# bravesoftdz/soundchunks

Measured on AMD Instinct MI355X. Metric: encoded Msamples/s @44.1kHz stereo ChunkSize=8 ChunkCount=4096; bit-exact .gsc, higher is better.
Workload: dtype f32; 1 GPU; 44.1 kHz stereo, ChunkSize=8 ChunkCount=4096 8-bit, 1024 s synthetic; frames=256, parallelism=frame-sharded x1

## Files before the change

soundchunks_amd/csrc/gsc_device.h:

```cpp
#pragma once
#include <stdint.h>

namespace gsc {

constexpr int kMaxK = 4096;
constexpr int kMaxInternal = 4095;
constexpr int kScanThreads = 512;
constexpr int kScanSlots = 8;
constexpr int kMaxScanIters = 100;
constexpr int kMaxChunkSize = 16;

__host__ __device__ constexpr int feature_stride(int cs) { return 2 * cs <= 8 ? 8 : (2 * cs <= 16 ? 16 : 32); }

__device__ inline float sqrt_rn(float x) { return __builtin_sqrtf(x); }

struct ReduceFrame {
    int64_t x_off;
    int64_t c_off;
    int64_t n_off;
    int64_t k_off;
    int64_t ka_off;
    int64_t t_off;
    int32_t N, K;
    int32_t iters;
    int32_t slow;
    double err;
    int32_t done;
    int32_t generic;
    int32_t restarts;
    int32_t loop_iters;
    int32_t tree_exact;
    int32_t dcol;
    uint64_t t_done;
    int32_t* cl_host;
    int32_t* notify;
    uint64_t stamps[128];
    uint64_t ystamps[16];
    uint64_t acounts[64];
    uint64_t xcounts[16];
    uint64_t xcounts2[16];
};

struct DspFrame {
    int64_t s_off;
    int64_t x_off;
    int64_t c_off;
    int32_t sc;
    int32_t n;
    int32_t atten_div;
    int32_t pad_;
};

struct ReconFrame {
    int64_t chunk_off;
    int64_t red_off;
    int64_t out_off;
    int32_t n, sc;
    double law;
};

struct FitFrame {
    int64_t cand_off;
    int64_t q_off;
    int64_t out_off;
    int32_t R, N;
    float eps;
    int32_t overflow;
};

struct PackFrame {
    int64_t out_off;
    int64_t r_off;
    int64_t w_off;
    int32_t N, R;
    int32_t nbits;
    int32_t cp_off;
};

inline int64_t pack_word_capacity(int64_t n) { return (n * 17 + 31) / 32 + 1; }

struct AnnTree {
    const float* pts;
    int n, dd;
    int* pidx;
    int* cd;
    float* cv;
    float* lo;
    float* hi;
    float* bnd;
    float* val;
    int ncap;
};

struct KnnOvJob {
    int tree;
    int q_off;
    int out;
    float eps;
};

}
```

soundchunks_amd/csrc/gsc_runtime.cpp:

```cpp
#include <cstddef>
#include <hip/hip_runtime.h>

#include <algorithm>
#include <atomic>
#include <chrono>
#include <cmath>
#include <cstdio>
#include <cstdlib>
#include <cstring>
#include <functional>
#include <new>
#include <string>
#include <strings.h>
#include <mutex>
#include <thread>
#include <vector>

#include "../../include/soundchunks.h"
#include "fpc_math.h"
#include "gsc_decode.h"
#include "gsc_device.h"
#include "gsc_encoder.h"

extern "C" hipError_t gsc_launch_yakmo(int D, const gsc::ReduceFrame* frames, int nframes, const float* X, float* C,
                                       float* fs, int* is, float* gsum, uint32_t* gbits, int max_n, hipStream_t st);
extern "C" size_t gsc_yakmo_big_floats(int64_t total_points, int nframes);
extern "C" size_t gsc_yakmo_big_words(int64_t total_points, int nframes);
extern "C" int gsc_yakmo_max_lds_points(void);
extern "C" hipError_t gsc_launch_scan_pass(int D, gsc::ReduceFrame* frames, int nframes, int K, const float* X,
                                           float* C, int* is, float* fs, const float* rate_tab, double tol, int max_passes,
                                           int only_flagged, hipStream_t st);
extern "C" hipError_t gsc_launch_scan_batch(int D, int logk, gsc::ReduceFrame* frames, int nframes, const float* X,
                                            float* C, int* is, const float* rate_tab, double tol, int max_passes,
                                            int opts, float* tails, hipStream_t st);
extern "C" size_t gsc_scan_tail_floats_per_frame(int D, int logk);
extern "C" hipError_t gsc_launch_atten(int cs, gsc::DspFrame* frames, int nframes, const double* samp, int64_t span,
                                       int ch, int obd, hipStream_t st);
extern "C" hipError_t gsc_launch_features(int cs, const gsc::DspFrame* frames, int nframes, int max_n,
                                          const double* samp, int64_t span, int ch, const double* trig, double s0,
                                          double scale, float* X, uint8_t* nr, float* Q, hipStream_t st);
extern "C" hipError_t gsc_launch_pcm(const int16_t* pcm, int64_t span, int ch, double* samp, hipStream_t st);
extern "C" hipError_t gsc_launch_knnfit(int CS, gsc::FitFrame* frames, int nframes, int max_n, int max_r,
                                        const float* cand, const float* q, int* out, hipStream_t st);
extern "C" hipError_t gsc_launch_recon(const gsc::ReconFrame* frames, int nframes, int max_n, int cs, int ch, int bd,
                                       const uint32_t* chunk, const int16_t* rdst, const uint8_t* ratten, int16_t* out,
                                       hipStream_t st);
extern "C" hipError_t gsc_launch_sqdiff(const int16_t* a, const int16_t* b, int64_t n, unsigned long long* acc,
                                        hipStream_t st);
extern "C" hipError_t gsc_launch_usecount(const gsc::PackFrame* frames, int nframes, const int* best, int* counts,
                                          hipStream_t st);
extern "C" hipError_t gsc_launch_pack(gsc::PackFrame* frames, int nframes, const int* best, const int* remap,
                                      uint32_t* words, uint32_t* codes, uint64_t* cps, hipStream_t st);
extern "C" hipError_t gsc_launch_ann_build_many(const void* trees, int ntrees, hipStream_t st);
extern "C" hipError_t gsc_launch_knnfit_ann(const void* trees, const void* jobs, int njobs, const float* q, int* out,
                                            float* pq_key, void* pq_node, int pq_cap, hipStream_t st);

namespace gsc {

void parallel_for(int n, int threads, const std::function<void(int)>& fn) {
    if (threads <= 1 || n <= 1) {
        for (int i = 0; i < n; ++i) fn(i);
        return;
    }
    std::atomic<int> next{0};
    std::vector<std::thread> pool;
    const int t = std::min(threads, n);
    pool.reserve(size_t(t));
    for (int k = 0; k < t; ++k)
        pool.emplace_back([&] {
            for (;;) {
                const int i = next.fetch_add(1);
                if (i >= n) break;
                fn(i);
            }
        });
    for (auto& th : pool) th.join();
}

int host_threads() {
    static int n = [] {
        const char* e = std::getenv("GSC_HOST_THREADS");
        if (e && std::atoi(e) > 0) return std::atoi(e);
        const unsigned hc = std::thread::hardware_concurrency();
        return int(std::min(16u, std::max(1u, hc)));
    }();
    return n;
}

namespace {

thread_local std::string t_err;
thread_local gsc_timing t_tim;

int fail(const std::string& m) {
    t_err = m;
    return -1;
}

#define HIP_TRY(expr)                                                                     \
    do {                                                                                  \
        hipError_t e_ = (expr);                                                           \
        if (e_ != hipSuccess) return fail(std::string(#expr) + ": " + hipGetErrorString(e_)); \
    } while (0)

double now_ms() {
    return std::chrono::duration<double, std::milli>(std::chrono::steady_clock::now().time_since_epoch()).count();
}

int ensure_device() {
    static int state = 0;
    static std::string why;
    if (state == 0) {
        int n = 0;
        if (hipGetDeviceCount(&n) != hipSuccess || n <= 0) {
            why = "no HIP device visible (the MI355X hot path has no CPU fallback)";
            state = -1;
        } else {
            hipDeviceProp_t p;
            int dev = 0;
            if (hipGetDevice(&dev) != hipSuccess || hipGetDeviceProperties(&p, dev) != hipSuccess) {
                why = "cannot query the HIP device";
                state = -1;
            } else if (std::strncmp(p.gcnArchName, "gfx950", 6) != 0) {
                why = std::string("device is ") + p.gcnArchName + ", kernels are built for gfx950 only";
                state = -1;
            } else {
                state = 1;
            }
        }
    }
    if (state < 0) return fail(why);
    (void)hipGetLastError();
    return 0;
}

std::atomic<int64_t> g_devbuf_ns{0};

template <typename T>
struct DevBuf {
    T* p = nullptr;
    size_t n = 0;
    ~DevBuf() {
        if (p) {
            const double t = now_ms();
            (void)hipFree(p);
            g_devbuf_ns.fetch_add(int64_t((now_ms() - t) * 1e6));
        }
    }
    hipError_t alloc(size_t count) {
        n = count;
        const double t = now_ms();
        const hipError_t e = hipMalloc(&p, sizeof(T) * std::max<size_t>(count, 1));
        g_devbuf_ns.fetch_add(int64_t((now_ms() - t) * 1e6));
        return e;
    }
};

struct DevArena {
    char* p = nullptr;
    size_t cap = 0, used = 0;
    std::vector<char*> retired;
    ~DevArena() {
        if (p) (void)hipFree(p);
        for (char* r : retired) (void)hipFree(r);
    }
    static size_t round_up(size_t b) { return (std::max<size_t>(b, 1) + 255) & ~size_t(255); }
    hipError_t reset(size_t bytes) {
        used = 0;
        if (bytes <= cap) return hipSuccess;
        if (p) retired.push_back(p);
        p = nullptr;
        cap = 0;
        const size_t want = std::max<size_t>(bytes + bytes / 4, size_t(1) << 20);
        const double t = now_ms();
        const hipError_t e = hipMalloc(reinterpret_cast<void**>(&p), want);
        g_devbuf_ns.fetch_add(int64_t((now_ms() - t) * 1e6));
        if (e == hipSuccess) cap = want;
        return e;
    }
    template <typename T>
    T* take(size_t count) {
        const size_t b = round_up(sizeof(T) * count);
        if (used + b > cap) return nullptr;
        T* r = reinterpret_cast<T*>(p + used);
        used += b;
        return r;
    }
};

double scan_tolerance(int precision) {
    if (precision <= 0) return 1.0;
    double p = 1.0, base = 10.0;
    int i = precision;
    while (i > 0) {
        while ((i & 1) == 0) {
            i >>= 1;
            base = base * base;
        }
        --i;
        p = p * base;
    }
    return 1.0 / p;
}

int padded_k(int K) {
    int k = 256;
    while (k < K) k <<= 1;
    return k;
}

bool batched_scan_shape(int D, int K) {
    if (std::getenv("GSC_SCAN_GENERIC")) return false;
    return (D == 8 || D == 16 || D == 32) && K >= 2 && K <= 4096;
}

int64_t tail_offset(int i) { return int64_t(i) * 4096 * 16; }

std::atomic<int> g_scan_rounds{0};

hipError_t launch_scan_passes(int D, ReduceFrame* dfr, int nf, int K, const float* X, float* C, int* is, float* fs,
                              const float* rate, int precision) {
    const double tol = scan_tolerance(precision);
    const bool batched = batched_scan_shape(D, K);
    int logk = 0;
    while ((1 << logk) < padded_k(K)) ++logk;
    DevBuf<float> tails;
    if (batched && gsc_scan_tail_floats_per_frame(D, logk) > 0) {
        const hipError_t e = tails.alloc(size_t(tail_offset(nf)));
        if (e != hipSuccess) return e;
    }
    int max_passes = kMaxScanIters;
    if (const char* e = std::getenv("GSC_SCAN_MAX_PASSES")) max_passes = std::max(1, std::min(kMaxScanIters, std::atoi(e)));
    std::vector<int32_t> flags(2 * static_cast<size_t>(nf));
    static_assert(offsetof(ReduceFrame, generic) == offsetof(ReduceFrame, done) + sizeof(int32_t), "adjacent flags");
    for (int round = 0; round < max_passes; ++round) {
        if (batched) {
            const int opts = (std::getenv("GSC_SCAN_FULL_A1") ? 1 : 0) | (std::getenv("GSC_SCAN_NO_PRUNE") ? 2 : 0) |
                             ((std::getenv("GSC_SCAN_KB") ? (std::atoi(std::getenv("GSC_SCAN_KB")) & 255) : 0) << 8);
            hipError_t e =
                gsc_launch_scan_batch(D, logk, dfr, nf, X, C, is, rate, tol, max_passes, opts, tails.p, nullptr);
            if (e != hipSuccess) return e;
            e = hipMemcpy2D(flags.data(), 2 * sizeof(int32_t), &dfr[0].done, sizeof(ReduceFrame), 2 * sizeof(int32_t),
                            size_t(nf), hipMemcpyDeviceToHost);
            if (e != hipSuccess) return e;
            g_scan_rounds.fetch_add(1);
            bool any_generic = false, all_done = true;
            for (int i = 0; i < nf; ++i) {
                all_done = all_done && flags[2 * size_t(i)] != 0;
                any_generic = any_generic || flags[2 * size_t(i) + 1] != 0;
            }
            if (all_done) break;
            if (!any_generic) continue;
        }
        const hipError_t e = gsc_launch_scan_pass(D, dfr, nf, K, X, C, is, fs, rate, tol, max_passes, batched ? 1 : 0, nullptr);
        if (e != hipSuccess) return e;
        if (!batched) g_scan_rounds.fetch_add(1);
    }
    return hipSuccess;
}

std::vector<float> rate_table(int n) {
    std::vector<float> t(size_t(n) + 2);
    t[0] = 0.0f;
    for (int c = 1; c < int(t.size()); ++c) t[c] = float(1.0 / std::sqrt(double(c)));
    return t;
}


int run_reduce_batch_dev(int D, int K, int precision, const std::vector<int>& Ns, const std::vector<int64_t>& xoff,
                         const float* dX, std::vector<float>* C, std::vector<int>* clusters, std::vector<int>* iters,
                         std::vector<int>* slow, long long* restarts, double* yakmo_ms, double* scan_ms,
                         int* cl_host = nullptr, int* notify = nullptr, int dcol = 0) {
    const int nf = int(Ns.size());
    if (nf == 0) return 0;
    if (D != 8 && D != 16 && D != 32) return fail("KNNScanReduce kernels support D = 8, 16 or 32 (ChunkSize 4, 8, 16)");
    std::vector<ReduceFrame> fr(static_cast<size_t>(nf));
    int64_t no = 0, maxN = 0;
    for (int i = 0; i < nf; ++i) {
        fr[i] = ReduceFrame{};
        fr[i].x_off = xoff[i];
        fr[i].c_off = int64_t(i) * K * D;
        fr[i].n_off = no;
        fr[i].k_off = 0;
        fr[i].N = Ns[i];
        fr[i].K = K;
        fr[i].dcol = dcol;
        no += Ns[i];
        maxN = std::max<int64_t>(maxN, Ns[i]);
    }
    const int Kp = padded_k(K);
    for (int i = 0; i < nf; ++i) {
        fr[i].k_off = no + int64_t(i) * K;
        fr[i].ka_off = no + int64_t(nf) * K + int64_t(i) * Kp;
        fr[i].t_off = tail_offset(i);
        if (cl_host && notify) {
            fr[i].cl_host = cl_host + fr[i].n_off;
            fr[i].notify = notify + i;
        }
    }
    DevBuf<float> dC, dF, dRate, dYSum;
    DevBuf<int> dI;
    DevBuf<uint32_t> dBits;
    DevBuf<ReduceFrame> dFr;
    HIP_TRY(dC.alloc(size_t(nf) * K * D));
    HIP_TRY(dF.alloc(size_t(no) * 4));
    HIP_TRY(dI.alloc(size_t(no) + size_t(nf) * (size_t(K) + size_t(Kp))));
    if (maxN > gsc_yakmo_max_lds_points()) {
        HIP_TRY(dBits.alloc(gsc_yakmo_big_words(no, nf)));
        HIP_TRY(dYSum.alloc(gsc_yakmo_big_floats(no, nf)));
    }
    HIP_TRY(dFr.alloc(size_t(nf)));
    const std::vector<float> rt = rate_table(int(maxN));
    HIP_TRY(dRate.alloc(rt.size()));
    HIP_TRY(hipMemcpy(dRate.p, rt.data(), sizeof(float) * rt.size(), hipMemcpyHostToDevice));
    HIP_TRY(hipMemcpy(dFr.p, fr.data(), sizeof(ReduceFrame) * size_t(nf), hipMemcpyHostToDevice));
    hipEvent_t e0, e1, e2;
    HIP_TRY(hipEventCreate(&e0));
    HIP_TRY(hipEventCreate(&e1));
    HIP_TRY(hipEventCreate(&e2));
    HIP_TRY(hipEventRecord(e0, nullptr));
    HIP_TRY(gsc_launch_yakmo(D, dFr.p, nf, dX, dC.p, dF.p, dI.p, dYSum.p, dBits.p, int(maxN), nullptr));
    HIP_TRY(hipEventRecord(e1, nullptr));
    HIP_TRY(launch_scan_passes(D, dFr.p, nf, K, dX, dC.p, dI.p, dF.p, dRate.p, precision));
    HIP_TRY(hipEventRecord(e2, nullptr));
    HIP_TRY(hipEventSynchronize(e2));
    float t1 = 0, t2 = 0;
    (void)hipEventElapsedTime(&t1, e0, e1);
    (void)hipEventElapsedTime(&t2, e1, e2);
    if (yakmo_ms) *yakmo_ms += t1;
    if (scan_ms) *scan_ms += t2;
    (void)hipEventDestroy(e0);
    (void)hipEventDestroy(e1);
    (void)hipEventDestroy(e2);
    C->resize(size_t(nf) * K * D);
    clusters->resize(size_t(no));
    HIP_TRY(hipMemcpy(C->data(), dC.p, sizeof(float) * C->size(), hipMemcpyDeviceToHost));
    HIP_TRY(hipMemcpy(clusters->data(), dI.p, sizeof(int) * size_t(no), hipMemcpyDeviceToHost));
    HIP_TRY(hipMemcpy(fr.data(), dFr.p, sizeof(ReduceFrame) * size_t(nf), hipMemcpyDeviceToHost));
    if (std::getenv("GSC_HOST_TIMING")) {
        std::vector<uint64_t> t;
        for (int i = 0; i < nf; ++i)
            if (fr[i].t_done) t.push_back(fr[i].t_done);
        if (!t.empty()) {
            std::sort(t.begin(), t.end());
            const double last = double(t.back());
            auto at = [&](double q) { return (last - double(t[size_t(q * double(t.size() - 1))])) / 1e5; };
            std::fprintf(stderr, "scan tail: frames finished [ms before the last] min %.1f p10 %.1f p50 %.1f p90 %.1f\n",
                         at(0.0), at(0.1), at(0.5), at(0.9));
        }
    }
    if (std::getenv("GSC_FRAME_STATS")) {
        uint64_t t0 = ~0ull;
        for (int i = 0; i < nf; ++i)
            if (fr[i].t_done) t0 = std::min<uint64_t>(t0, fr[i].t_done);
        for (int i = 0; i < nf; ++i)
            std::fprintf(stderr, "frame %d: N %d passes %d slow %d restarts %d done +%.1f ms\n", i, fr[i].N, fr[i].iters,
                         fr[i].slow, fr[i].restarts, fr[i].t_done ? double(fr[i].t_done - t0) / 1e5 : -1.0);
    }
    if (std::getenv("GSC_HOST_TIMING") && nf > 0 && fr[0].ystamps[6] + fr[0].ystamps[1] + fr[0].ystamps[2] != 0) {
        double m[16] = {};
        for (int i = 0; i < nf; ++i)
            for (int k = 0; k < 16; ++k) m[k] += double(fr[i].ystamps[k]) / double(nf) / double(K);
        std::fprintf(stderr,
                     "yakmo stamps [clk/pick]: chain pick %.0f fast %.0f slow %.0f wait %.0f (fast calls %.1f"
                     " slow blocks %.1f) | dist pick+sdlo %.0f compute %.0f wait %.0f | negative deltas dropped"
                     " per pick: chain %.3g dist %.3g\n",
                     m[0], m[1], m[2], m[3], m[4], m[5], m[8], m[9], m[10], m[6], m[14]);
    }
    iters->resize(size_t(nf));
    slow->resize(size_t(nf));
    for (int i = 0; i < nf; ++i) {
        (*iters)[i] = fr[i].iters;
        (*slow)[i] = fr[i].slow;
        if (restarts) *restarts += fr[i].restarts;
        if (fr[i].loop_iters < 0) return fail("KNNScanReduce: batched pipeline made no progress (guard tripped)");
    }
    return 0;
}

int run_reduce_batch(int D, int K, int precision, const std::vector<int>& Ns, const std::vector<float>& X,
                     std::vector<float>* C, std::vector<int>* clusters, std::vector<int>* iters, std::vector<int>* slow,
                     long long* restarts, double* yakmo_ms, double* scan_ms) {
    std::vector<int64_t> xoff(Ns.size());
    int64_t xo = 0;
    for (size_t i = 0; i < Ns.size(); ++i) {
        xoff[i] = xo;
        xo += int64_t(Ns[i]) * D;
    }
    DevBuf<float> dX;
    HIP_TRY(dX.alloc(size_t(xo)));
    HIP_TRY(hipMemcpy(dX.p, X.data(), sizeof(float) * size_t(xo), hipMemcpyHostToDevice));
    return run_reduce_batch_dev(D, K, precision, Ns, xoff, dX.p, C, clusters, iters, slow, restarts, yakmo_ms,
                                scan_ms);
}

int run_knnfit_overflow(int CS, const std::vector<FitFrame>& fr, const std::vector<int>& ov_frames,
                        const std::vector<float>& eps, const std::vector<float>& cand, const std::vector<float>& q,
                        std::vector<int>* best, hipStream_t st, DevArena* arena) {
    const int nt = int(ov_frames.size());
    const double t_begin = now_ms();
    std::vector<float> pts;
    std::vector<int64_t> pt_off(static_cast<size_t>(nt)), nd_off(static_cast<size_t>(nt));
    std::vector<int> caps(static_cast<size_t>(nt));
    int64_t nodes = 0;
    int max_n = 0;
    for (int t = 0; t < nt; ++t) {
        const FitFrame& f = fr[size_t(ov_frames[t])];
        const int n = 4 * f.R;
        pt_off[t] = int64_t(pts.size());
        pts.resize(pts.size() + size_t(n) * CS);
        float* o = pts.data() + pt_off[t];
        const float* c = cand.data() + f.cand_off;
        for (int r = 0; r < f.R; ++r) {
            const float* v = c + size_t(r) * CS;
            for (int j = 0; j < CS; ++j) {
                const float fw = v[j], rv = v[CS - 1 - j];
                o[(size_t(4 * r) + 0) * CS + j] = fw;
                o[(size_t(4 * r) + 1) * CS + j] = rv;
                o[(size_t(4 * r) + 2) * CS + j] = fw == 0.0f ? 0.0f : -fw;
                o[(size_t(4 * r) + 3) * CS + j] = rv == 0.0f ? 0.0f : -rv;
            }
        }
        int p2 = 1;
        while (p2 < n) p2 <<= 1;
        caps[t] = 2 * p2;
        nd_off[t] = nodes;
        nodes += caps[t];
        max_n = std::max(max_n, n);
    }
    std::vector<KnnOvJob> jobs;
    std::vector<int64_t> job_q;
    for (int t = 0; t < nt; ++t) {
        const FitFrame& f = fr[size_t(ov_frames[t])];
        for (int i = 0; i < f.N; ++i)
            if ((*best)[size_t(f.out_off + i)] == -1) {
                jobs.push_back(KnnOvJob{t, int(f.q_off + int64_t(i) * CS), int(f.out_off + i), eps[size_t(ov_frames[t])]});
            }
    }
    if (jobs.empty()) return 0;
    if (q.size() > size_t(INT32_MAX)) return fail("KNNFit overflow: query slab exceeds 2^31 floats");
    const int pq_cap = max_n + 2;
    const size_t per_job = size_t(pq_cap) * (sizeof(float) + sizeof(int4));
    const int chunk = int(std::max<size_t>(64, std::min<size_t>(jobs.size(), (size_t(2) << 30) / per_job)));
    const size_t npts = pts.size() / size_t(CS);
    const size_t R = DevArena::round_up(sizeof(float) * pts.size()) + 2 * DevArena::round_up(sizeof(float) * npts) +
                     2 * DevArena::round_up(sizeof(int) * size_t(nodes)) + 2 * DevArena::round_up(sizeof(float) * size_t(nodes)) +
                     DevArena::round_up(sizeof(int) * npts) + DevArena::round_up(sizeof(float) * size_t(2 * CS * nt)) +
                     DevArena::round_up(sizeof(AnnTree) * size_t(nt)) + DevArena::round_up(sizeof(float) * q.size()) +
                     DevArena::round_up(sizeof(int) * best->size()) + DevArena::round_up(sizeof(KnnOvJob) * jobs.size()) +
                     DevArena::round_up(sizeof(float) * size_t(chunk) * pq_cap) +
                     DevArena::round_up(sizeof(int4) * size_t(chunk) * pq_cap);
    HIP_TRY(arena->reset(R));
    float* dPts = arena->take<float>(pts.size());
    int* dPidx = arena->take<int>(npts);
    float* dVal = arena->take<float>(npts);
    int* dCd = arena->take<int>(size_t(nodes));
    float* dCv = arena->take<float>(size_t(nodes));
    float* dLo = arena->take<float>(size_t(nodes));
    float* dHi = arena->take<float>(size_t(nodes));
    float* dBnd = arena->take<float>(size_t(2 * CS * nt));
    AnnTree* dTrees = arena->take<AnnTree>(size_t(nt));
    float* dQ = arena->take<float>(q.size());
    int* dOut = arena->take<int>(best->size());
    KnnOvJob* dJobs = arena->take<KnnOvJob>(jobs.size());
    float* dPqk = arena->take<float>(size_t(chunk) * pq_cap);
    int4* dPqn = arena->take<int4>(size_t(chunk) * pq_cap);
    (void)dVal;
    if (!dPqn) return fail("KNNFit overflow: replay arena too small");
    HIP_TRY(hipMemsetAsync(arena->p, 0xff, arena->used, st));
    HIP_TRY(hipMemcpyAsync(dPts, pts.data(), sizeof(float) * pts.size(), hipMemcpyHostToDevice, st));
    HIP_TRY(hipMemcpyAsync(dQ, q.data(), sizeof(float) * q.size(), hipMemcpyHostToDevice, st));
    HIP_TRY(hipMemcpyAsync(dOut, best->data(), sizeof(int) * best->size(), hipMemcpyHostToDevice, st));
    std::vector<AnnTree> trees(static_cast<size_t>(nt));
    for (int t = 0; t < nt; ++t) {
        AnnTree& a = trees[size_t(t)];
        a.pts = dPts + pt_off[t];
        a.n = 4 * fr[size_t(ov_frames[t])].R;
        a.dd = CS;
        a.pidx = dPidx + pt_off[t] / CS;
        a.cd = dCd + nd_off[t];
        a.cv = dCv + nd_off[t];
        a.lo = dLo + nd_off[t];
        a.hi = dHi + nd_off[t];
        a.bnd = dBnd + size_t(2 * CS) * size_t(t);
        a.val = dVal + pt_off[t] / CS;
        a.ncap = caps[t];
    }
    HIP_TRY(hipMemcpyAsync(dTrees, trees.data(), sizeof(AnnTree) * size_t(nt), hipMemcpyHostToDevice, st));
    const bool timing = std::getenv("GSC_HOST_TIMING") != nullptr;
    struct EvPair {
        hipEvent_t a = nullptr, b = nullptr;
        ~EvPair() {
            if (a) (void)hipEventDestroy(a);
            if (b) (void)hipEventDestroy(b);
        }
    } ev;
    hipEvent_t& eb0 = ev.a;
    hipEvent_t& eb1 = ev.b;
    if (timing) {
        HIP_TRY(hipEventCreate(&eb0));
        HIP_TRY(hipEventCreate(&eb1));
        HIP_TRY(hipEventRecord(eb0, st));
    }
    HIP_TRY(gsc_launch_ann_build_many(dTrees, nt, st));
    if (timing) HIP_TRY(hipEventRecord(eb1, st));
    HIP_TRY(hipMemcpyAsync(dJobs, jobs.data(), sizeof(KnnOvJob) * jobs.size(), hipMemcpyHostToDevice, st));
    for (size_t j0 = 0; j0 < jobs.size(); j0 += size_t(chunk)) {
        const int nj = int(std::min<size_t>(size_t(chunk), jobs.size() - j0));
        HIP_TRY(gsc_launch_knnfit_ann(dTrees, dJobs + j0, nj, dQ, dOut, dPqk, dPqn, pq_cap, st));
    }
    HIP_TRY(hipMemcpyAsync(best->data(), dOut, sizeof(int) * best->size(), hipMemcpyDeviceToHost, st));
    HIP_TRY(hipStreamSynchronize(st));
    if (timing) {
        float bms = 0.0f;
        (void)hipEventElapsedTime(&bms, eb0, eb1);
        std::fprintf(stderr, "KNNFit overflow: %d trees (largest %d candidates), %zu queries, %.2f ms (tree builds %.2f ms)\n",
                     nt, max_n, jobs.size(), now_ms() - t_begin, double(bms));
    }
    for (const KnnOvJob& j : jobs) {
        const int b = (*best)[size_t(j.out)];
        if (b == -4) return fail("KNNFit overflow: a tree index left its frame's arrays (device bounds check)");
        if (b < 0) return fail("KNNFit: ANN priority search emulation failed");
    }
    return 0;
}

int run_knnfit_batch(int CS, const std::vector<int>& Rs, const std::vector<int>& Ns, const std::vector<float>& eps,
                     const std::vector<float>& cand, const std::vector<float>& q, std::vector<int>* best,
                     double* knn_ms, const float* qdev = nullptr) {
    const int nf = int(Ns.size());
    if (nf == 0) return 0;
    std::vector<FitFrame> fr(static_cast<size_t>(nf));
    int64_t co = 0, qo = 0;
    int maxN = 0, maxR = 0;
    for (int i = 0; i < nf; ++i) {
        fr[i] = FitFrame{};
        fr[i].cand_off = co;
        fr[i].q_off = qo;
        fr[i].out_off = qo / CS;
        fr[i].R = Rs[i];
        fr[i].N = Ns[i];
        fr[i].eps = eps[i];
        co += int64_t(Rs[i]) * CS;
        qo += int64_t(Ns[i]) * CS;
        maxN = std::max(maxN, Ns[i]);
        maxR = std::max(maxR, Rs[i]);
    }
    DevBuf<float> dCand, dQ;
    DevBuf<int> dOut;
    DevBuf<FitFrame> dFr;
    HIP_TRY(dCand.alloc(size_t(co)));
    if (!qdev) {
        HIP_TRY(dQ.alloc(size_t(qo)));
        HIP_TRY(hipMemcpy(dQ.p, q.data(), sizeof(float) * size_t(qo), hipMemcpyHostToDevice));
        qdev = dQ.p;
    }
    HIP_TRY(dOut.alloc(size_t(qo / CS)));
    HIP_TRY(dFr.alloc(size_t(nf)));
    HIP_TRY(hipMemcpy(dCand.p, cand.data(), sizeof(float) * size_t(co), hipMemcpyHostToDevice));
    HIP_TRY(hipMemcpy(dFr.p, fr.data(), sizeof(FitFrame) * size_t(nf), hipMemcpyHostToDevice));
    hipEvent_t e0, e1;
    HIP_TRY(hipEventCreate(&e0));
    HIP_TRY(hipEventCreate(&e1));
    HIP_TRY(hipEventRecord(e0, nullptr));
    HIP_TRY(gsc_launch_knnfit(CS, dFr.p, nf, maxN, maxR, dCand.p, qdev, dOut.p, nullptr));
    HIP_TRY(hipEventRecord(e1, nullptr));
    HIP_TRY(hipEventSynchronize(e1));
    float t = 0;
    (void)hipEventElapsedTime(&t, e0, e1);
    if (knn_ms) *knn_ms += t;
    (void)hipEventDestroy(e0);
    (void)hipEventDestroy(e1);
    best->resize(size_t(qo / CS));
    HIP_TRY(hipMemcpy(best->data(), dOut.p, sizeof(int) * best->size(), hipMemcpyDeviceToHost));
    HIP_TRY(hipMemcpy(fr.data(), dFr.p, sizeof(FitFrame) * size_t(nf), hipMemcpyDeviceToHost));
    std::vector<int> ov_frames;
    for (int i = 0; i < nf; ++i)
        if (fr[i].overflow > 0) ov_frames.push_back(i);
    if (!ov_frames.empty()) {
        const double t0 = now_ms();
        std::vector<float> qh;
        if (q.empty()) {
            qh.resize(size_t(qo));
            HIP_TRY(hipMemcpy(qh.data(), qdev, sizeof(float) * size_t(qo), hipMemcpyDeviceToHost));
        }
        DevArena arena;
        if (run_knnfit_overflow(CS, fr, ov_frames, eps, cand, q.empty() ? qh : q, best, nullptr, &arena) != 0) return -1;
        if (knn_ms) *knn_ms += now_ms() - t0;
    }
    return 0;
}

struct PinnedBuf {
    unsigned flags = hipHostMallocDefault;
    void* p = nullptr;
    size_t cap = 0;
    hipError_t reserve(size_t bytes) {
        if (bytes <= cap) return hipSuccess;
        if (p) (void)hipHostFree(p);
        p = nullptr;
        cap = 0;
        const size_t want = std::max<size_t>(bytes + bytes / 4, 4096);
        const hipError_t e = hipHostMalloc(&p, want, flags);
        if (e == hipSuccess) cap = want;
        return e;
    }
    template <typename T>
    T* as() const {
        return static_cast<T*>(p);
    }
};

struct PinnedArena {
    std::mutex m;
    PinnedBuf cand, cnt, remap, words, codes;
    PinnedBuf cl{hipHostMallocMapped | hipHostMallocCoherent}, notify{hipHostMallocMapped | hipHostMallocCoherent};
};

PinnedArena& pinned_arena() {
    static PinnedArena* a = new PinnedArena;
    return *a;
}

}

struct PostCtx {
    hipStream_t st = nullptr;
    bool recon = false;
    std::vector<int64_t> coff, roff, woff, noff;
    DevBuf<float> dCand;
    DevBuf<int> dBest, dCnt, dRemap;
    DevBuf<uint32_t> dWords, dCodes;
    DevBuf<FitFrame> dFit;
    DevBuf<PackFrame> dPack;
    bool table = false;
    std::vector<int64_t> cpoff;
    DevBuf<uint64_t> dCps;
    std::vector<uint64_t> hCps;
    DevArena ov_arena;
    const float* dQry = nullptr;
    float* hCand = nullptr;
    int *hCnt = nullptr, *hRemap = nullptr;
    uint32_t *hWords = nullptr, *hCodes = nullptr;
    int slot = 0;
    double knn_ms = 0;
    int groups = 0;
    long long ov_queries = 0;
    ~PostCtx() {
        if (st) {
            (void)hipStreamSynchronize(st);
            (void)hipStreamDestroy(st);
        }
    }
};

static void compact_rows(std::vector<float>* v, int n, int dp, int d) {
    if (dp == d) return;
    for (int i = 0; i < n; ++i)
        for (int k = 0; k < d; ++k) (*v)[size_t(i) * d + k] = (*v)[size_t(i) * dp + k];
    v->resize(size_t(n) * d);
}

int Encoder::device_dsp(int b, std::vector<FrameState>& frames, void* dXv, std::vector<int64_t>* xoff, double* ms,
                        std::string* err, void* dQv) {
    auto& dX = *static_cast<DevBuf<float>*>(dXv);
    const int cs = opt_.chunk_size, ch = channels_, nfr = int(frames.size());
    const int obd = (1 << (opt_.chunk_bit_depth - 1)) - 1;
    const int e = b + nfr;
    const int64_t s_first = fr_start_[b], span = int64_t(fr_end_[e - 1]) - s_first + 1;
    std::vector<DspFrame> df(static_cast<size_t>(nfr));
    xoff->assign(size_t(nfr), 0);
    int64_t xo = 0, co = 0;
    int max_n = 0;
    for (int i = 0; i < nfr; ++i) {
        const FrameState& f = frames[i];
        df[i] = DspFrame{};
        df[i].s_off = int64_t(f.start) - s_first;
        df[i].x_off = xo;
        df[i].c_off = co;
        df[i].sc = f.sample_count;
        df[i].n = f.n;
        (*xoff)[i] = xo;
        xo += int64_t(f.n) * feature_stride(cs);
        co += f.n;
        max_n = std::max(max_n, f.n);
    }
    std::vector<double> trig;
    double s0 = 0, scale = 0;
    trig_pack(cs, &trig, &s0, &scale);
    DevBuf<double> dS, dT;
    DevBuf<DspFrame> dF;
    DevBuf<uint8_t> dNR;
    DevBuf<int16_t> dP;
    float* dQ = nullptr;
    const double t0 = now_ms();
    if (dS.alloc(size_t(ch) * size_t(span)) != hipSuccess || dT.alloc(trig.size()) != hipSuccess ||
        dF.alloc(size_t(nfr)) != hipSuccess || dNR.alloc(size_t(co)) != hipSuccess || dX.alloc(size_t(xo)) != hipSuccess ||
        dP.alloc(size_t(ch) * size_t(span)) != hipSuccess) {
        *err = "device DSP: out of device memory";
        return -1;
    }
    if (dQv) {
        auto& q = *static_cast<DevBuf<float>*>(dQv);
        if (q.alloc(size_t(co) * size_t(cs)) != hipSuccess) {
            *err = "device DSP: out of device memory";
            return -1;
        }
        dQ = q.p;
    }
    auto chk = [&](hipError_t r, const char* what) {
        if (r == hipSuccess) return true;
        *err = std::string("device DSP: ") + what + ": " + hipGetErrorString(r);
        return false;
    };
    if (!chk(hipMemcpy(dP.p, pcm_.data() + size_t(s_first - pcm_off_) * ch, sizeof(int16_t) * size_t(ch) * size_t(span),
                       hipMemcpyHostToDevice),
             "sample upload") ||
        !chk(gsc_launch_pcm(dP.p, span, ch, dS.p, nullptr), "sample conversion"))
        return -1;
    if (!chk(hipMemcpy(dT.p, trig.data(), sizeof(double) * trig.size(), hipMemcpyHostToDevice), "trig upload") ||
        !chk(hipMemcpy(dF.p, df.data(), sizeof(DspFrame) * size_t(nfr), hipMemcpyHostToDevice), "frame upload") ||
        !chk(gsc_launch_atten(cs, dF.p, nfr, dS.p, span, ch, obd, nullptr), "atten launch") ||
        !chk(gsc_launch_features(cs, dF.p, nfr, max_n, dS.p, span, ch, dT.p, s0, scale, dX.p, dNR.p, dQ, nullptr),
             "features launch"))
        return -1;
    std::vector<uint8_t> nr(static_cast<size_t>(co));
    if (!chk(hipMemcpy(df.data(), dF.p, sizeof(DspFrame) * size_t(nfr), hipMemcpyDeviceToHost), "frame download") ||
        !chk(hipMemcpy(nr.data(), dNR.p, size_t(co), hipMemcpyDeviceToHost), "flag download"))
        return -1;
    for (int i = 0; i < nfr; ++i) {
        FrameState& f = frames[i];
        f.atten_div = df[i].atten_div;
        const uint8_t* q = nr.data() + df[i].c_off;
        for (int c = 0; c < f.n; ++c) {
            f.neg[c] = q[c] & 1;
            f.rev[c] = (q[c] >> 1) & 1;
        }
    }
    if (ms) *ms += now_ms() - t0;
    return 0;
}

int Encoder::device_recon(int b, const std::vector<FrameState>& frames, ReconOut* ro, std::string* err) {
    const int cs = opt_.chunk_size, ch = channels_, nfr = int(frames.size());
    if (nfr == 0) return 0;
    const double t0 = now_ms();
    const int64_t s_first = fr_start_[b], span = int64_t(fr_end_[b + nfr - 1]) - s_first + 1;
    std::vector<ReconFrame> rf(static_cast<size_t>(nfr));
    int64_t nchunk = 0, nred = 0;
    int max_n = 0;
    for (int i = 0; i < nfr; ++i) {
        const FrameState& f = frames[i];
        rf[i] = ReconFrame{nchunk, nred, int64_t(f.start) - s_first, f.n, f.sample_count, 1.0 / double(f.atten_div)};
        nchunk += f.n;
        nred += f.r;
        max_n = std::max(max_n, f.n);
    }
    std::vector<uint32_t> words(static_cast<size_t>(nchunk));
    std::vector<int16_t> rdst(static_cast<size_t>(std::max<int64_t>(nred, 1) * cs));
    std::vector<uint8_t> ratten(static_cast<size_t>(std::max<int64_t>(nred, 1)));
    parallel_for(nfr, host_threads(), [&](int i) {
        const FrameState& f = frames[i];
        uint32_t* w = words.data() + rf[i].chunk_off;
        for (int c = 0; c < f.n; ++c) w[c] = uint32_t(f.red[c]) << 2 | uint32_t(f.neg[c] & 1) << 1 | uint32_t(f.rev[c] & 1);
        std::copy(f.rdst.begin(), f.rdst.begin() + long(size_t(f.r) * cs), rdst.begin() + long(rf[i].red_off * cs));
        std::copy(f.ratten.begin(), f.ratten.begin() + f.r, ratten.begin() + long(rf[i].red_off));
    });
    const int64_t psc = ro->wav_len >= 44 ? int64_t((ro->wav_len - 44) / (2 * size_t(ch))) : 0;
    std::vector<int16_t> src(static_cast<size_t>(span * ch), 0);
    const int64_t avail = std::max<int64_t>(0, std::min(span, psc - s_first));
    if (avail > 0) std::memcpy(src.data(), ro->wav + 44 + size_t(s_first) * ch * 2, size_t(avail) * ch * 2);
    DevBuf<ReconFrame> dF;
    DevBuf<uint32_t> dW;
    DevBuf<int16_t> dR, dOut, dSrc;
    DevBuf<uint8_t> dA;
    DevBuf<unsigned long long> dAcc;
    auto chk = [&](hipError_t r, const char* what) {
        if (r == hipSuccess) return true;
        *err = std::string("reconstruction: ") + what + ": " + hipGetErrorString(r);
        return false;
    };
    const size_t nout = size_t(span) * ch;
    if (!chk(dF.alloc(size_t(nfr)), "alloc") || !chk(dW.alloc(words.size()), "alloc") ||
        !chk(dR.alloc(rdst.size()), "alloc") || !chk(dA.alloc(ratten.size()), "alloc") ||
        !chk(dOut.alloc(nout), "alloc") || !chk(dSrc.alloc(nout), "alloc") || !chk(dAcc.alloc(1), "alloc"))
        return -1;
    if (!chk(hipMemcpy(dF.p, rf.data(), sizeof(ReconFrame) * rf.size(), hipMemcpyHostToDevice), "upload") ||
        !chk(hipMemcpy(dW.p, words.data(), sizeof(uint32_t) * words.size(), hipMemcpyHostToDevice), "upload") ||
        !chk(hipMemcpy(dR.p, rdst.data(), sizeof(int16_t) * rdst.size(), hipMemcpyHostToDevice), "upload") ||
        !chk(hipMemcpy(dA.p, ratten.data(), ratten.size(), hipMemcpyHostToDevice), "upload") ||
        !chk(hipMemcpy(dSrc.p, src.data(), sizeof(int16_t) * nout, hipMemcpyHostToDevice), "upload") ||
        !chk(hipMemset(dOut.p, 0, sizeof(int16_t) * nout), "memset") ||
        !chk(hipMemset(dAcc.p, 0, sizeof(unsigned long long)), "memset") ||
        !chk(gsc_launch_recon(dF.p, nfr, max_n, cs, ch, opt_.chunk_bit_depth, dW.p, dR.p, dA.p, dOut.p, nullptr),
             "recon launch") ||
        !chk(gsc_launch_sqdiff(dSrc.p, dOut.p, int64_t(nout), dAcc.p, nullptr), "PsyADelta launch"))
        return -1;
    unsigned long long sq = 0;
    if (!chk(hipMemcpy(ro->pcm + size_t(s_first) * ch, dOut.p, sizeof(int16_t) * nout, hipMemcpyDeviceToHost),
             "download") ||
        !chk(hipMemcpy(&sq, dAcc.p, sizeof(sq), hipMemcpyDeviceToHost), "download"))
        return -1;
    ro->sq += sq;
    ro->ms += now_ms() - t0;
    return 0;
}

static bool inject_post_failure() {
    static std::atomic<int> used{0};
    return std::getenv("GSC_TEST_FAIL_POST") != nullptr && used.exchange(1) == 0;
}

int Encoder::post_group(std::vector<FrameState>& frames, const std::vector<int>& ids,
                        const std::vector<char>& reduced, PostCtx& c, std::string* err) {
    const int cs = opt_.chunk_size, bd = opt_.chunk_bit_depth, obd = (1 << (bd - 1)) - 1;
    const int g = int(ids.size());
    if (g == 0) return 0;
    if (inject_post_failure()) {
        *err = "injected post_group failure (GSC_TEST_FAIL_POST)";
        return -1;
    }
    auto chk = [&](hipError_t r, const char* what) {
        if (r == hipSuccess) return true;
        *err = std::string("KNNFit/pack pipeline: ") + what + ": " + hipGetErrorString(r);
        return false;
    };
    std::vector<float> eps(static_cast<size_t>(g));
    parallel_for(g, host_threads(), [&](int k) {
        FrameState& f = frames[size_t(ids[k])];
        frame_reduce_post(f, reduced[size_t(ids[k])] != 0);
        const double law = 1.0 / double(f.atten_div);
        float acc = 1.0f;
        for (int j = 0; j <= 15; ++j) acc = float(double(acc) + double(j) * law);
        const float e1 = 1.0f / (float(1 << bd) * acc);
        const float e2 = float(1.0 / 32767.0);
        eps[size_t(k)] = e1 > e2 ? e1 : e2;
        float* cp = c.hCand + c.coff[size_t(ids[k])];
        for (int r = 0; r < f.r; ++r) {
            double coeff = 1.0;
            for (int a = 0; a <= f.ratten[r]; ++a) coeff += double(a) * law;
            for (int j = 0; j < cs; ++j) {
                double v = double(f.rdst[size_t(r) * cs + j]) / (double(obd) * coeff);
                v = std::min(1.0, std::max(-1.0, v));
                *cp++ = float(v);
            }
        }
    });
    const int gb = c.slot;
    c.slot += g;
    std::vector<FitFrame> fit(static_cast<size_t>(g));
    std::vector<PackFrame> pk(static_cast<size_t>(g));
    int maxN = 0, maxR = 0;
    for (int k = 0; k < g; ++k) {
        const size_t i = size_t(ids[k]);
        const FrameState& f = frames[i];
        fit[size_t(k)] = FitFrame{c.coff[i], c.noff[i] * cs, c.noff[i], f.r, f.n, eps[size_t(k)], 0};
        pk[size_t(k)] = PackFrame{c.noff[i], c.roff[i], c.woff[i], f.n, f.r, 0, c.table ? int32_t(c.cpoff[i]) : 0};
        maxN = std::max(maxN, f.n);
        maxR = std::max(maxR, f.r);
    }
    hipEvent_t e0 = nullptr, e1 = nullptr;
    if (!chk(hipEventCreate(&e0), "event") || !chk(hipEventCreate(&e1), "event")) return -1;
    struct EvGuard {
        hipEvent_t a, b;
        ~EvGuard() {
            (void)hipEventDestroy(a);
            (void)hipEventDestroy(b);
        }
    } evg{e0, e1};
    const hipStream_t st = c.st;
    bool ok = chk(hipMemcpyAsync(c.dFit.p + gb, fit.data(), sizeof(FitFrame) * size_t(g), hipMemcpyHostToDevice, st),
                  "upload") &&
              chk(hipMemcpyAsync(c.dPack.p + gb, pk.data(), sizeof(PackFrame) * size_t(g), hipMemcpyHostToDevice, st),
                  "upload");
    for (int k = 0; ok && k < g; ++k) {
        const size_t i = size_t(ids[k]);
        ok = chk(hipMemcpyAsync(c.dCand.p + c.coff[i], c.hCand + c.coff[i], sizeof(float) * size_t(frames[i].r) * cs,
                                hipMemcpyHostToDevice, st),
                 "candidate upload");
    }
    ok = ok && chk(hipEventRecord(e0, st), "event") &&
         chk(gsc_launch_knnfit(cs, c.dFit.p + gb, g, maxN, maxR, c.dCand.p, c.dQry, c.dBest.p, st), "KNNFit launch") &&
         chk(hipEventRecord(e1, st), "event") &&
         chk(gsc_launch_usecount(c.dPack.p + gb, g, c.dBest.p, c.dCnt.p, st), "use count launch") &&
         chk(hipMemcpyAsync(fit.data(), c.dFit.p + gb, sizeof(FitFrame) * size_t(g), hipMemcpyDeviceToHost, st),
             "download");
    for (int k = 0; ok && k < g; ++k) {
        const size_t i = size_t(ids[k]);
        ok = chk(hipMemcpyAsync(c.hCnt + c.roff[i], c.dCnt.p + c.roff[i], sizeof(int) * size_t(frames[i].r),
                                hipMemcpyDeviceToHost, st),
                 "use count download");
    }
    if (!ok || !chk(hipStreamSynchronize(st), "KNNFit")) return -1;
    float t = 0;
    if (hipEventElapsedTime(&t, e0, e1) == hipSuccess) c.knn_ms += t;
    std::vector<int> ovk;
    for (int k = 0; k < g; ++k)
        if (fit[size_t(k)].overflow > 0) ovk.push_back(k);
    if (!ovk.empty()) {
        const double t0 = now_ms();
        std::vector<FitFrame> lf;
        std::vector<float> lcand, lq, leps;
        std::vector<int> lbest, lidx;
        for (int k : ovk) {
            const FrameState& f = frames[size_t(ids[k])];
            FitFrame x = fit[size_t(k)];
            x.cand_off = int64_t(lcand.size());
            x.q_off = int64_t(lq.size());
            x.out_off = int64_t(lbest.size());
            lcand.insert(lcand.end(), c.hCand + fit[size_t(k)].cand_off,
                         c.hCand + fit[size_t(k)].cand_off + size_t(f.r) * cs);
            lq.resize(lq.size() + size_t(f.n) * cs);
            lbest.resize(lbest.size() + size_t(f.n));
            if (!chk(hipMemcpyAsync(lq.data() + x.q_off, c.dQry + fit[size_t(k)].q_off, sizeof(float) * size_t(f.n) * cs,
                                    hipMemcpyDeviceToHost, st),
                     "query download") ||
                !chk(hipMemcpyAsync(lbest.data() + x.out_off, c.dBest.p + fit[size_t(k)].out_off,
                                    sizeof(int) * size_t(f.n), hipMemcpyDeviceToHost, st),
                     "download"))
                return -1;
            lidx.push_back(int(lf.size()));
            leps.push_back(x.eps);
            lf.push_back(x);
        }
        if (!chk(hipStreamSynchronize(st), "download")) return -1;
        c.ov_queries += std::count(lbest.begin(), lbest.end(), -1);
        if (run_knnfit_overflow(cs, lf, lidx, leps, lcand, lq, &lbest, st, &c.ov_arena) != 0) {
            *err = t_err;
            return -1;
        }
        for (size_t j = 0; j < ovk.size(); ++j)
            if (!chk(hipMemcpyAsync(c.dBest.p + fit[size_t(ovk[j])].out_off, lbest.data() + lf[j].out_off,
                                    sizeof(int) * size_t(lf[j].N), hipMemcpyHostToDevice, st),
                     "upload"))
                return -1;
        ok = chk(gsc_launch_usecount(c.dPack.p + gb, g, c.dBest.p, c.dCnt.p, st), "use count launch");
        for (int k = 0; ok && k < g; ++k) {
            const size_t i = size_t(ids[k]);
            ok = chk(hipMemcpyAsync(c.hCnt + c.roff[i], c.dCnt.p + c.roff[i], sizeof(int) * size_t(frames[i].r),
                                    hipMemcpyDeviceToHost, st),
                     "use count download");
        }
        if (!ok || !chk(hipStreamSynchronize(st), "use counts")) return -1;
        c.knn_ms += now_ms() - t0;
    }
    parallel_for(g, host_threads(), [&](int k) {
        const size_t i = size_t(ids[k]);
        frame_prune(frames[i], c.hCnt + c.roff[i], c.hRemap + c.roff[i]);
    });
    for (int k = 0; k < g; ++k) {
        const FrameState& f = frames[size_t(ids[k])];
        if (f.r > kMaxK) {
            *err = "SaveStream: Assert(reducedChunks.Count <= CMaxChunksPerFrame) failed: frame " +
                   std::to_string(f.index) + " keeps " + std::to_string(f.r) + " reduced chunks";
            return -1;
        }
    }
    ok = true;
    for (int k = 0; ok && k < g; ++k) {
        const size_t i = size_t(ids[k]);
        ok = chk(hipMemcpyAsync(c.dRemap.p + c.roff[i], c.hRemap + c.roff[i],
                                sizeof(int) * size_t(frames[i].r_before_prune), hipMemcpyHostToDevice, st),
                 "remap upload");
    }
    ok = ok && chk(gsc_launch_pack(c.dPack.p + gb, g, c.dBest.p, c.dRemap.p, c.dWords.p, c.recon ? c.dCodes.p : nullptr,
                                   c.table ? c.dCps.p : nullptr, st),
                   "pack launch") &&
         chk(hipMemcpyAsync(pk.data(), c.dPack.p + gb, sizeof(PackFrame) * size_t(g), hipMemcpyDeviceToHost, st),
             "download") &&
         chk(hipStreamSynchronize(st), "pack");
    for (int k = 0; ok && k < g; ++k) {
        const size_t i = size_t(ids[k]);
        const int64_t nw = (int64_t(pk[size_t(k)].nbits) + 31) / 32;
        if (pk[size_t(k)].nbits < 0 || nw > pack_word_capacity(frames[i].n)) {
            *err = "index packer overran its word slab";
            return -1;
        }
        ok = chk(hipMemcpyAsync(c.hWords + c.woff[i], c.dWords.p + c.woff[i], sizeof(uint32_t) * size_t(nw),
                                hipMemcpyDeviceToHost, st),
                 "stream download");
        if (ok && c.recon)
            ok = chk(hipMemcpyAsync(c.hCodes + c.noff[i], c.dCodes.p + c.noff[i], sizeof(uint32_t) * size_t(frames[i].n),
                                    hipMemcpyDeviceToHost, st),
                     "code download");
        const size_t ncp = c.table ? (size_t(frames[i].n) + kDecodeS - 1) / kDecodeS : 0;
        if (ok && ncp)
            ok = chk(hipMemcpyAsync(c.hCps.data() + c.cpoff[i], c.dCps.p + c.cpoff[i], sizeof(uint64_t) * ncp,
                                    hipMemcpyDeviceToHost, st),
                     "checkpoint download");
        frames[i].nbits = pk[size_t(k)].nbits;
    }
    if (!ok || !chk(hipStreamSynchronize(st), "stream download")) return -1;
    parallel_for(g, host_threads(), [&](int k) {
        const size_t i = size_t(ids[k]);
        FrameState& f = frames[i];
        frame_save_head(f);
        const size_t nbytes = size_t((pk[size_t(k)].nbits + 15) / 16) * 2;
        const uint8_t* wb = reinterpret_cast<const uint8_t*>(c.hWords + c.woff[i]);
        f.stream.insert(f.stream.end(), wb, wb + nbytes);
        if (c.recon) {
            f.red.resize(size_t(f.n));
            f.neg.resize(size_t(f.n));
            f.rev.resize(size_t(f.n));
            const uint32_t* cw = c.hCodes + c.noff[i];
            for (int j = 0; j < f.n; ++j) {
                f.red[size_t(j)] = int(cw[j] >> 2);
                f.neg[size_t(j)] = uint8_t((cw[j] >> 1) & 1);
                f.rev[size_t(j)] = uint8_t(cw[j] & 1);
            }
        }
    });
    c.groups += 1;
    return 0;
}

int Encoder::dsp_frame(int fi, int* atten_div, std::vector<float>* feat, std::string* err) {
    if (ensure_device() != 0) {
        *err = t_err;
        return -1;
    }
    if (fi < 0 || fi >= frame_count()) {
        *err = "frame index out of range";
        return -1;
    }
    warm_trig_tables(opt_.chunk_size);
    std::vector<FrameState> frames(1);
    frames[0].index = fi;
    frames[0].start = fr_start_[fi];
    frames[0].sample_count = fr_end_[fi] - fr_start_[fi] + 1;
    frame_host_src(frames[0]);
    DevBuf<float> dX;
    std::vector<int64_t> xoff;
    if (device_dsp(fi, frames, &dX, &xoff, nullptr, err) != 0) return -1;
    *atten_div = frames[0].atten_div;
    const int dp = feature_stride(opt_.chunk_size);
    feat->resize(size_t(frames[0].n) * dp);
    if (hipMemcpy(feat->data(), dX.p, sizeof(float) * feat->size(), hipMemcpyDeviceToHost) != hipSuccess) {
        *err = "feature download failed";
        return -1;
    }
    compact_rows(feat, frames[0].n, dp, 2 * opt_.chunk_size);
    return 0;
}

int Encoder::encode_range(int b, int e, std::vector<uint8_t>* out, std::string* err, gsc_timing* tim,
                          ReconOut* recon, std::vector<size_t>* frame_bytes, std::vector<uint8_t>* table) {
    if (ensure_device() != 0) {
        *err = t_err;
        return -1;
    }
    const int cs = opt_.chunk_size, D = 2 * cs, K = opt_.chunks_per_frame;
    const int DP = feature_stride(cs);
    const int nfr = e - b;
    std::vector<FrameState> frames(static_cast<size_t>(std::max(nfr, 0)));
    double t0 = now_ms();
    warm_trig_tables(cs);
    parallel_for(nfr, host_threads(), [&](int i) {
        FrameState& f = frames[i];
        f.index = b + i;
        f.start = fr_start_[b + i];
        f.sample_count = fr_end_[b + i] - fr_start_[b + i] + 1;
        frame_host_src(f);
    });
    double dsp_ms = 0;
    DevBuf<float> dFeat, dQry;
    std::vector<int64_t> feat_off;
    if (nfr > 0 && device_dsp(b, frames, &dFeat, &feat_off, &dsp_ms, err, &dQry) != 0) return -1;
    double t1 = now_ms();
    std::vector<int> red_idx, Ns;
    std::vector<int64_t> red_xoff;
    std::vector<char> is_red(size_t(nfr), 0);
    for (int i = 0; i < nfr; ++i)
        if (opt_.precision > 0 && frames[i].n > K) {
            red_idx.push_back(i);
            Ns.push_back(frames[i].n);
            red_xoff.push_back(feat_off[i]);
            is_red[size_t(i)] = 1;
        }
    const int nred = int(red_idx.size());
    double yak_ms = 0, scan_ms = 0;
    long long passes = 0, slow = 0, restarts = 0;
    PinnedArena& pa = pinned_arena();
    std::lock_guard<std::mutex> arena_lock(pa.m);
    struct DeviceDrain {
        ~DeviceDrain() { (void)hipDeviceSynchronize(); }
    } drain_before_unlock;
    PostCtx pc;
    pc.recon = recon != nullptr;
    pc.dQry = dQry.p;
    pc.coff.resize(size_t(nfr));
    pc.roff.resize(size_t(nfr));
    pc.woff.resize(size_t(nfr));
    pc.noff.resize(size_t(nfr));
    pc.table = table != nullptr;
    pc.cpoff.resize(size_t(nfr));
    int64_t nc = 0, nr = 0, nw = 0, nn = 0, ncp = 0;
    for (int i = 0; i < nfr; ++i) {
        const int rmax = is_red[size_t(i)] ? K : frames[i].n;
        pc.coff[size_t(i)] = nc;
        pc.roff[size_t(i)] = nr;
        pc.woff[size_t(i)] = nw;
        pc.noff[size_t(i)] = nn;
        nc += int64_t(rmax) * cs;
        nr += rmax;
        nw += pack_word_capacity(frames[i].n);
        nn += frames[i].n;
        pc.cpoff[size_t(i)] = ncp;
        ncp += (int64_t(frames[i].n) + kDecodeS - 1) / kDecodeS;
    }
    if (pc.table && ncp >= (int64_t(1) << 31)) {
        *err = "seek table: too many checkpoints for one call";
        return -1;
    }
    if (pc.table) pc.hCps.resize(size_t(ncp));
    int64_t nred_pts = 0;
    for (int n : Ns) nred_pts += n;
    {
        auto chk = [&](hipError_t r, const char* what) {
            if (r == hipSuccess) return true;
            *err = std::string("KNNFit/pack pipeline setup: ") + what + ": " + hipGetErrorString(r);
            return false;
        };
        if (!chk(hipStreamCreateWithFlags(&pc.st, hipStreamNonBlocking), "stream") ||
            !chk(pc.dCand.alloc(size_t(nc)), "alloc") || !chk(pc.dBest.alloc(size_t(nn)), "alloc") ||
            !chk(pc.dCnt.alloc(size_t(nr)), "alloc") || !chk(pc.dRemap.alloc(size_t(nr)), "alloc") ||
            !chk(pc.dWords.alloc(size_t(nw)), "alloc") || !chk(pc.dFit.alloc(size_t(std::max(nfr, 1))), "alloc") ||
            !chk(pc.dPack.alloc(size_t(std::max(nfr, 1))), "alloc") ||
            (pc.recon && !chk(pc.dCodes.alloc(size_t(nn)), "alloc")) ||
            (pc.table && !chk(pc.dCps.alloc(size_t(std::max<int64_t>(ncp, 1))), "alloc")) ||
            !chk(pa.cand.reserve(sizeof(float) * size_t(nc)), "pinned alloc") ||
            !chk(pa.cnt.reserve(sizeof(int) * size_t(nr)), "pinned alloc") ||
            !chk(pa.remap.reserve(sizeof(int) * size_t(nr)), "pinned alloc") ||
            !chk(pa.words.reserve(sizeof(uint32_t) * size_t(nw)), "pinned alloc") ||
            (pc.recon && !chk(pa.codes.reserve(sizeof(uint32_t) * size_t(nn)), "pinned alloc")) ||
            !chk(pa.cl.reserve(sizeof(int) * size_t(std::max<int64_t>(nred_pts, 1))), "pinned alloc") ||
            !chk(pa.notify.reserve(sizeof(int) * size_t(std::max(nred, 1))), "pinned alloc") ||
            !chk(hipMemsetAsync(pc.dWords.p, 0, sizeof(uint32_t) * size_t(nw), pc.st), "memset"))
            return -1;
    }
    pc.hCand = pa.cand.as<float>();
    pc.hCnt = pa.cnt.as<int>();
    pc.hRemap = pa.remap.as<int>();
    pc.hWords = pa.words.as<uint32_t>();
    pc.hCodes = pa.codes.as<uint32_t>();
    int* notify = pa.notify.as<int>();
    int* cl_host = pa.cl.as<int>();
    std::memset(notify, 0, sizeof(int) * size_t(std::max(nred, 1)));
    std::vector<int64_t> red_noff(size_t(nred) + 1, 0);
    std::vector<int> red_pos(size_t(nfr), -1);
    for (int j = 0; j < nred; ++j) {
        red_noff[size_t(j) + 1] = red_noff[size_t(j)] + Ns[size_t(j)];
        red_pos[size_t(red_idx[size_t(j)])] = j;
    }
    std::atomic<int> scan_state{0};
    std::vector<int> cl_final;
    std::string post_err;
    double t_scan_end = 0, overlap_ms = 0;
    const bool batched_scan = nred > 0 && !opt_.python_reduce;
    auto post_loop = [&]() -> int {
        std::vector<char> done(size_t(nfr), 0);
        int remaining = nfr;
        while (remaining > 0) {
            const int st = scan_state.load(std::memory_order_acquire);
            if (st < 0) return 0;
            std::vector<int> ids;
            for (int i = 0; i < nfr; ++i) {
                if (done[size_t(i)]) continue;
                const int j = red_pos[size_t(i)];
                const bool notified = j >= 0 && batched_scan && __atomic_load_n(&notify[j], __ATOMIC_ACQUIRE) != 0;
                if (j < 0 || notified || st == 1) ids.push_back(i);
            }
            if (ids.empty() || (st == 0 && int(ids.size()) < std::min(remaining, 8))) {
                std::this_thread::sleep_for(std::chrono::microseconds(500));
                continue;
            }
            for (int i : ids) {
                const int j = red_pos[size_t(i)];
                if (j < 0 || !batched_scan) continue;
                FrameState& f = frames[size_t(i)];
                if (__atomic_load_n(&notify[j], __ATOMIC_ACQUIRE) != 0)
                    f.clusters.assign(cl_host + red_noff[size_t(j)], cl_host + red_noff[size_t(j) + 1]);
                else
                    f.clusters.assign(cl_final.begin() + long(red_noff[size_t(j)]),
                                      cl_final.begin() + long(red_noff[size_t(j) + 1]));
            }
            const double tg = now_ms();
            if (post_group(frames, ids, is_red, pc, &post_err) != 0) return -1;
            if (st == 0) overlap_ms += now_ms() - tg;
            for (int i : ids) done[size_t(i)] = 1;
            remaining -= int(ids.size());
        }
        return 0;
    };
    if (nred > 0 && opt_.python_reduce) {
        const double tb = now_ms();
        for (size_t j = 0; j < red_idx.size(); ++j) {
            FrameState& f = frames[red_idx[j]];
            std::vector<float> x(size_t(f.n) * DP);
            if (hipMemcpy(x.data(), dFeat.p + red_xoff[j], sizeof(float) * x.size(), hipMemcpyDeviceToHost) !=
                hipSuccess) {
                *err = "-py: feature download failed";
                return -1;
            }
            compact_rows(&x, f.n, DP, D);
            f.clusters.resize(size_t(f.n));
            if (birch_reduce_labels(f.n, D, x.data(), K, f.clusters.data(), err) != 0) return -1;
            f.scan_iters = 0;
            f.scan_slow = 0;
        }
        scan_ms += now_ms() - tb;
    }
    int post_rc = 0;
    if (batched_scan) {
        int dev = 0;
        (void)hipGetDevice(&dev);
        std::thread worker([&] {
            if (hipSetDevice(dev) != hipSuccess) {
                post_err = "KNNFit/pack pipeline: hipSetDevice failed";
                post_rc = -1;
                return;
            }
            post_rc = post_loop();
        });
        std::vector<float> C;
        std::vector<int> it, sl;
        g_scan_rounds.store(0);
        int* cl_dev = nullptr;
        int* nt_dev = nullptr;
        int rr = 0;
        if (hipHostGetDevicePointer(reinterpret_cast<void**>(&cl_dev), cl_host, 0) != hipSuccess ||
            hipHostGetDevicePointer(reinterpret_cast<void**>(&nt_dev), notify, 0) != hipSuccess) {
            rr = fail("KNNScanReduce: no device address for the host-mapped cluster buffers");
        } else {
            rr = run_reduce_batch_dev(DP, K, opt_.precision, Ns, red_xoff, dFeat.p, &C, &cl_final, &it, &sl, &restarts,
                                      &yak_ms, &scan_ms, cl_dev, nt_dev, D);
        }
        t_scan_end = now_ms();
        if (rr != 0) *err = t_err;
        scan_state.store(rr != 0 ? -1 : 1, std::memory_order_release);
        worker.join();
        if (rr != 0) return -1;
        for (int j = 0; j < nred; ++j) {
            FrameState& f = frames[size_t(red_idx[size_t(j)])];
            f.scan_iters = it[size_t(j)];
            f.scan_slow = sl[size_t(j)];
            passes += it[size_t(j)];
            slow += sl[size_t(j)];
        }
    } else {
        t_scan_end = now_ms();
        scan_state.store(1, std::memory_order_release);
        post_rc = post_loop();
    }
    if (post_rc != 0) {
        *err = post_err;
        return -1;
    }
    const double t2 = t_scan_end;
    const double t3 = now_ms();
    if (recon && device_recon(b, frames, recon, err) != 0) return -1;
    const double recon_ms = now_ms() - t3;
    out->clear();
    size_t bytes = 0;
    for (auto& f : frames) bytes += f.stream.size();
    out->reserve(bytes);
    for (auto& f : frames) out->insert(out->end(), f.stream.begin(), f.stream.end());
    if (frame_bytes) {
        frame_bytes->clear();
        for (auto& f : frames) frame_bytes->push_back(f.stream.size());
    }
    if (table) {
        Index ix;
        ix.frames.resize(frames.size());
        size_t off = 0;
        for (size_t i = 0; i < frames.size(); ++i) {
            ix.frames[i].off = off;
            ix.frames[i].nbits = uint64_t(frames[i].nbits);
            off += frames[i].stream.size();
        }
        ix.len = off;
        ix.cps = std::move(pc.hCps);
        index_table_write(ix, table);
    }
    double t4 = now_ms();
    if (std::getenv("GSC_HOST_TIMING"))
        std::fprintf(stderr,
                     "host timing [ms]: frames+dsp %.1f (dsp %.1f) | reduce (yakmo %.1f scan %.1f) %.1f |"
                     " post after the scan %.1f (in the scan tail %.1f, KNNFit kernels %.1f, %d groups) | concat %.1f"
                     " | hipMalloc/hipFree so far %.1f\n",
                     t1 - t0, dsp_ms, yak_ms, scan_ms, t2 - t1, t3 - t2, overlap_ms, pc.knn_ms, pc.groups, t4 - t3,
                     double(g_devbuf_ns.exchange(0)) / 1e6);
    if (std::getenv("GSC_HOST_TIMING") && !red_idx.empty()) {
        std::vector<int> h(kMaxScanIters + 1, 0);
        for (int i : red_idx) h[std::min(kMaxScanIters, std::max(0, frames[i].scan_iters))]++;
        std::fprintf(stderr, "scan passes histogram:");
        for (int v = 0; v <= kMaxScanIters; ++v)
            if (h[v]) std::fprintf(stderr, " %d:%d", v, h[v]);
        std::fprintf(stderr, "\n");
    }
    if (tim) {
        tim->host_frames_ms = t1 - t0 - dsp_ms;
        tim->gpu_dsp_ms = dsp_ms;
        tim->gpu_yakmo_ms = yak_ms;
        tim->gpu_scan_ms = scan_ms;
        tim->gpu_knnfit_ms = pc.knn_ms;
        tim->host_post_ms = t4 - t2 - recon_ms;
        tim->gpu_recon_ms = recon_ms;
        tim->post_overlap_ms = overlap_ms;
        tim->post_groups = pc.groups;
        tim->knnfit_overflow = pc.ov_queries;
        tim->frames = nfr;
        tim->reduce_frames = int(red_idx.size());
        long long pts = 0;
        for (auto& f : frames) pts += f.n;
        tim->points = pts;
        tim->scan_passes = passes;
        tim->scan_slow = slow;
        tim->scan_restarts = restarts;
        long long pp = 0;
        for (auto& f : frames) pp += (long long)f.scan_iters * f.n;
        tim->scan_point_passes = pp;
        tim->scan_launches = g_scan_rounds.exchange(0);
        tim->knnfit_launches = pc.groups;
        long long cand = 0;
        for (auto& f : frames) cand += (long long)f.n * 4 * f.r_before_prune;
        tim->knnfit_pairs = cand;
    }
    return 0;
}

int set_last_error(const std::string& m) { return fail(m); }
int require_device() { return ensure_device(); }

}

using namespace gsc;

extern "C" {

void gsc_default_options(gsc_options* o) {
    std::memset(o, 0, sizeof(*o));
    o->bit_rate = -1;
    o->precision = 3;
    o->low_cut = 0.0;
    o->high_cut = 24000.0;
    o->chunk_bit_depth = 8;
    o->chunk_size = 4;
    o->chunks_per_frame = 4096;
    o->reduce_bass_band = 1;
    o->vfr = 1.0;
    o->chunk_blend = 0;
    o->frame_length = 4000.0;
}

static int opt_start(int argc, const char* const* argv, const char* pfx) {
    const size_t l = std::strlen(pfx);
    for (int i = 0; i < argc; ++i)
        if (std::strncmp(argv[i], pfx, l) == 0) return i;
    return -1;
}
static double opt_value(int argc, const char* const* argv, const char* pfx, double def) {
    const int i = opt_start(argc, argv, pfx);
    if (i < 0) return def;
    const char* s = argv[i] + std::strlen(pfx);
    if (!*s) return def;
    char* end = nullptr;
    const double v = std::strtod(s, &end);
    return (end && !*end) ? v : def;
}
static bool opt_has(int argc, const char* const* argv, const char* p) {
    for (int i = 0; i < argc; ++i)
        if (strcasecmp(argv[i], p) == 0) return true;
    return false;
}

void gsc_parse_options(gsc_options* o, int argc, const char* const* argv) {
    auto clampi = [](int64_t v, int64_t lo, int64_t hi) { return int(std::min(hi, std::max(lo, v))); };
    o->bit_rate = int(fpc::round(opt_value(argc, argv, "-br", o->bit_rate)));
    o->precision = int(fpc::round(opt_value(argc, argv, "-pr", o->precision)));
    o->low_cut = opt_value(argc, argv, "-lc", o->low_cut);
    o->high_cut = opt_value(argc, argv, "-hc", o->high_cut);
    o->vfr = std::min(1.0, std::max(0.0, opt_value(argc, argv, "-vfr", o->vfr)));
    o->frame_length = std::max(opt_value(argc, argv, "-fl", o->frame_length), 1.0);
    o->chunk_bit_depth = clampi(fpc::round(opt_value(argc, argv, "-cbd", o->chunk_bit_depth)), 1, 16);
    o->chunk_size = int(fpc::round(opt_value(argc, argv, "-cs", o->chunk_size)));
    o->chunks_per_frame = clampi(fpc::round(opt_value(argc, argv, "-cpf", o->chunks_per_frame)), 256, 4096);
    o->verbose = opt_has(argc, argv, "-v");
    o->reduce_bass_band = !opt_has(argc, argv, "-pbb");
    o->chunk_blend = clampi(fpc::round(opt_value(argc, argv, "-cb", o->chunk_blend)), 0, o->chunk_size / 2);
    o->python_reduce = opt_has(argc, argv, "-py");
}

int gsc_count_frames(const uint8_t* wav, size_t wav_len, const gsc_options* o, int* frame_count) {
    Encoder enc(*o);
    std::string err;
    if (enc.prepare(wav, wav_len, &err) != 0) return fail(err);
    *frame_count = enc.frame_count();
    return 0;
}

static int encode_prepared(Encoder& enc, int frame_begin, int frame_end, uint8_t** out, size_t* out_len,
                           size_t* file_bytes = nullptr, size_t* frame_bytes = nullptr,
                           std::vector<uint8_t>* table = nullptr) {
    const double t0 = now_ms();
    const int fc = enc.frame_count();
    frame_begin = std::max(0, frame_begin);
    frame_end = std::min(fc, frame_end < 0 ? fc : frame_end);
    std::vector<uint8_t> bytes;
    std::vector<size_t> fb;
    std::string err;
    if (frame_end > frame_begin) {
        if (enc.encode_range(frame_begin, frame_end, &bytes, &err, &t_tim, nullptr, &fb, table) != 0) return fail(err);
    }
    if (file_bytes) {
        const std::vector<int>& ff = enc.file_first();
        for (size_t f = 0; f + 1 < ff.size(); ++f) {
            size_t n = 0;
            for (int i = std::max(ff[f], frame_begin); i < std::min(ff[f + 1], frame_end); ++i)
                n += fb[size_t(i - frame_begin)];
            file_bytes[f] = n;
        }
    }
    if (frame_bytes)
        for (int i = frame_begin; i < frame_end; ++i) frame_bytes[i - frame_begin] = fb[size_t(i - frame_begin)];
    *out = static_cast<uint8_t*>(std::malloc(std::max<size_t>(bytes.size(), 1)));
    if (!*out) return fail("out of host memory");
    if (!bytes.empty()) std::memcpy(*out, bytes.data(), bytes.size());
    *out_len = bytes.size();
    t_tim.total_ms = now_ms() - t0;
    return 0;
}

int gsc_encode_wav_frames(const uint8_t* wav, size_t wav_len, const gsc_options* o, int frame_begin, int frame_end,
                          uint8_t** out, size_t* out_len, int* frame_count) {
    const double t0 = now_ms();
    t_tim = gsc_timing{};
    Encoder enc(*o);
    std::string err;
    if (enc.prepare(wav, wav_len, &err) != 0) return fail(err);
    const double t1 = now_ms();
    if (frame_count) *frame_count = enc.frame_count();
    if (encode_prepared(enc, frame_begin, frame_end, out, out_len) != 0) return -1;
    t_tim.host_prepare_ms = t1 - t0;
    t_tim.total_ms = now_ms() - t0;
    return 0;
}

}

struct gsc_prepared {
    Encoder enc;
    double prepare_ms = 0;
    int loaded_begin = 0, loaded_end = -1;
    explicit gsc_prepared(const gsc_options& o) : enc(o) {}
};

extern "C" {

gsc_prepared* gsc_prepare(const uint8_t* wav, size_t wav_len, const gsc_options* o) {
    if (!wav || !o) {
        fail("gsc_prepare: null argument");
        return nullptr;
    }
    const double t0 = now_ms();
    gsc_prepared* p = new (std::nothrow) gsc_prepared(*o);
    if (!p) {
        fail("gsc_prepare: out of host memory");
        return nullptr;
    }
    std::string err;
    if (p->enc.prepare(wav, wav_len, &err) != 0) {
        delete p;
        fail(err);
        return nullptr;
    }
    p->prepare_ms = now_ms() - t0;
    return p;
}

int gsc_prepared_frame_count(const gsc_prepared* p) { return p ? p->enc.frame_count() : -1; }

int gsc_prepared_frame_chunks(const gsc_prepared* p, int* chunks) {
    if (!p || !chunks) return fail("gsc_prepared_frame_chunks: null argument");
    for (int i = 0; i < p->enc.frame_count(); ++i) chunks[i] = p->enc.frame_chunks(i);
    return 0;
}

int gsc_prepared_frame_bounds(const gsc_prepared* p, int* starts, int* ends) {
    if (!p || !starts || !ends) return fail("gsc_prepared_frame_bounds: null argument");
    const auto& s = p->enc.frame_starts();
    const auto& e = p->enc.frame_ends();
    std::copy(s.begin(), s.end(), starts);
    std::copy(e.begin(), e.end(), ends);
    return 0;
}

gsc_prepared* gsc_prepare_frames(const uint8_t* wav, size_t wav_len, const gsc_options* o, const int* starts,
                                 const int* ends, int frame_count, int frame_begin, int frame_end) {
    if (!wav || !o || !starts || !ends) {
        fail("gsc_prepare_frames: null argument");
        return nullptr;
    }
    const double t0 = now_ms();
    gsc_prepared* p = new (std::nothrow) gsc_prepared(*o);
    if (!p) {
        fail("gsc_prepare_frames: out of host memory");
        return nullptr;
    }
    std::string err;
    if (frame_end < 0) frame_end = frame_count;
    if (p->enc.prepare_bounds(wav, wav_len, starts, ends, frame_count, frame_begin, frame_end, &err) != 0) {
        delete p;
        fail(err);
        return nullptr;
    }
    p->loaded_begin = frame_begin;
    p->loaded_end = frame_end;
    p->prepare_ms = now_ms() - t0;
    return p;
}

static int check_loaded(const gsc_prepared* p, int frame_begin, int frame_end, const char* who) {
    if (p->loaded_end < 0) return 0;
    const int fe = frame_end < 0 ? p->enc.frame_count() : std::min(frame_end, p->enc.frame_count());
    const int fb = std::max(0, frame_begin);
    if (fe > fb && (fb < p->loaded_begin || fe > p->loaded_end))
        return fail(std::string(who) + ": frames outside the range gsc_prepare_frames loaded");
    return 0;
}

int gsc_encode_prepared(gsc_prepared* p, int frame_begin, int frame_end, uint8_t** out, size_t* out_len) {
    return gsc_encode_prepared_frames(p, frame_begin, frame_end, out, out_len, nullptr);
}

int gsc_encode_prepared_frames(gsc_prepared* p, int frame_begin, int frame_end, uint8_t** out, size_t* out_len,
                               size_t* frame_bytes) {
    if (!p || !out || !out_len) return fail("gsc_encode_prepared: null argument");
    if (check_loaded(p, frame_begin, frame_end, "gsc_encode_prepared") != 0) return -1;
    t_tim = gsc_timing{};
    if (encode_prepared(p->enc, frame_begin, frame_end, out, out_len, nullptr, frame_bytes) != 0) return -1;
    t_tim.host_prepare_ms = 0;
    return 0;
}

int gsc_encode_prepared_with_table(gsc_prepared* p, int frame_begin, int frame_end, uint8_t** out, size_t* out_len,
                                   uint8_t** table, size_t* table_len) {
    if (!p || !out || !out_len || !table || !table_len) return fail("gsc_encode_prepared_with_table: null argument");
    if (p->enc.file_first().size() != 2)
        return fail("gsc_encode_prepared_with_table: a batch of files has no single table; index each file's bytes");
    if (check_loaded(p, frame_begin, frame_end, "gsc_encode_prepared_with_table") != 0) return -1;
    t_tim = gsc_timing{};
    std::vector<uint8_t> t;
    *table = static_cast<uint8_t*>(std::malloc(1));
    if (!*table) return fail("out of host memory");
    if (encode_prepared(p->enc, frame_begin, frame_end, out, out_len, nullptr, nullptr, &t) != 0) {
        std::free(*table);
        *table = nullptr;
        return -1;
    }
    t_tim.host_prepare_ms = 0;
    if (!t.empty()) {
        uint8_t* q = static_cast<uint8_t*>(std::realloc(*table, t.size()));
        if (!q) {
            std::free(*table);
            std::free(*out);
            *table = *out = nullptr;
            return fail("out of host memory");
        }
        std::memcpy(q, t.data(), t.size());
        *table = q;
    }
    *table_len = t.size();
    return 0;
}

int gsc_encode_prepared_files_with_tables(gsc_prepared* p, int frame_begin, int frame_end, uint8_t** out,
                                          size_t* out_len, size_t* file_bytes, uint8_t** tables, size_t* tables_len,
                                          size_t* table_bytes) {
    if (!p || !out || !out_len || !file_bytes || !tables || !tables_len || !table_bytes)
        return fail("gsc_encode_prepared_files_with_tables: null argument");
    if (check_loaded(p, frame_begin, frame_end, "gsc_encode_prepared_files_with_tables") != 0) return -1;
    t_tim = gsc_timing{};
    std::vector<uint8_t> t;
    if (encode_prepared(p->enc, frame_begin, frame_end, out, out_len, file_bytes, nullptr, &t) != 0) return -1;
    t_tim.host_prepare_ms = 0;
    const int nfiles = int(p->enc.file_first().size()) - 1;
    std::vector<std::vector<uint8_t>> per;
    std::string err;
    size_t total = 0;
    if (t.empty()) {
        per.assign(size_t(nfiles), std::vector<uint8_t>());
    } else if (index_table_split(*out, *out_len, t.data(), t.size(), file_bytes, nfiles, &per, &err) != 0) {
        std::free(*out);
        *out = nullptr;
        return fail(err);
    }
    for (const auto& v : per) total += v.size();
    *tables = static_cast<uint8_t*>(std::malloc(std::max<size_t>(total, 1)));
    if (!*tables) {
        std::free(*out);
        *out = nullptr;
        return fail("out of host memory");
    }
    size_t at = 0;
    for (int f = 0; f < nfiles; ++f) {
        if (!per[size_t(f)].empty()) std::memcpy(*tables + at, per[size_t(f)].data(), per[size_t(f)].size());
        table_bytes[f] = per[size_t(f)].size();
        at += per[size_t(f)].size();
    }
    *tables_len = total;
    return 0;
}

double gsc_prepared_prepare_ms(const gsc_prepared* p) { return p ? p->prepare_ms : 0.0; }

gsc_prepared* gsc_prepare_many(const uint8_t* const* wavs, const size_t* lens, int nfiles, const gsc_options* o) {
    if (!wavs || !lens || !o || nfiles <= 0) {
        fail("gsc_prepare_many: invalid argument");
        return nullptr;
    }
    const double t0 = now_ms();
    gsc_prepared* p = new (std::nothrow) gsc_prepared(*o);
    if (!p) {
        fail("gsc_prepare_many: out of host memory");
        return nullptr;
    }
    std::string err;
    if (p->enc.prepare_many(wavs, lens, nfiles, &err) != 0) {
        delete p;
        fail(err);
        return nullptr;
    }
    p->prepare_ms = now_ms() - t0;
    return p;
}

int gsc_prepared_file_count(const gsc_prepared* p) { return p ? int(p->enc.file_first().size()) - 1 : -1; }

int gsc_prepared_file_frames(const gsc_prepared* p, int* first_frame) {
    if (!p || !first_frame) return fail("gsc_prepared_file_frames: null argument");
    const auto& ff = p->enc.file_first();
    std::copy(ff.begin(), ff.end(), first_frame);
    return 0;
}

int gsc_encode_prepared_files(gsc_prepared* p, int frame_begin, int frame_end, uint8_t** out, size_t* out_len,
                              size_t* file_bytes) {
    if (!p || !out || !out_len || !file_bytes) return fail("gsc_encode_prepared_files: null argument");
    if (check_loaded(p, frame_begin, frame_end, "gsc_encode_prepared_files") != 0) return -1;
    t_tim = gsc_timing{};
    if (encode_prepared(p->enc, frame_begin, frame_end, out, out_len, file_bytes) != 0) return -1;
    return 0;
}

void gsc_prepared_free(gsc_prepared* p) { delete p; }

int gsc_frame_dsp(const uint8_t* wav, size_t wav_len, const gsc_options* o, int frame, int* atten_div, float** feat,
                  int* n_chunks) {
    Encoder enc(*o);
    std::string err;
    if (enc.prepare(wav, wav_len, &err) != 0) return fail(err);
    std::vector<float> f;
    if (enc.dsp_frame(frame, atten_div, &f, &err) != 0) return fail(err);
    *n_chunks = int(f.size() / size_t(2 * o->chunk_size));
    *feat = static_cast<float*>(std::malloc(std::max<size_t>(f.size(), 1) * sizeof(float)));
    if (!f.empty()) std::memcpy(*feat, f.data(), f.size() * sizeof(float));
    return 0;
}

int gsc_encode_wav(const uint8_t* wav, size_t wav_len, const gsc_options* o, uint8_t** out, size_t* out_len) {
    return gsc_encode_wav_frames(wav, wav_len, o, 0, -1, out, out_len, nullptr);
}

int gsc_encode_wav_recon(const uint8_t* wav, size_t wav_len, const gsc_options* o, uint8_t** out, size_t* out_len,
                         int16_t** recon, size_t* recon_len, double* psy_a_delta) {
    if (!wav || !o || !out || !out_len || !recon || !recon_len || !psy_a_delta)
        return fail("gsc_encode_wav_recon: null argument");
    *out = nullptr;
    *recon = nullptr;
    t_tim = gsc_timing{};
    const double t0 = now_ms();
    Encoder enc(*o);
    std::string err;
    if (enc.prepare(wav, wav_len, &err) != 0) return fail(err);
    t_tim.host_prepare_ms = now_ms() - t0;
    const int ch = enc.channels();
    const size_t n = size_t(enc.sample_count()) * size_t(ch);
    ReconOut ro;
    ro.pcm = static_cast<int16_t*>(std::calloc(std::max<size_t>(n, 1), sizeof(int16_t)));
    if (!ro.pcm) return fail("out of host memory");
    ro.wav = wav;
    ro.wav_len = wav_len;
    std::vector<uint8_t> bytes;
    const int fc = enc.frame_count();
    if (fc > 0 && enc.encode_range(0, fc, &bytes, &err, &t_tim, &ro) != 0) {
        std::free(ro.pcm);
        return fail(err);
    }
    *out = static_cast<uint8_t*>(std::malloc(std::max<size_t>(bytes.size(), 1)));
    if (!*out) {
        std::free(ro.pcm);
        return fail("out of host memory");
    }
    if (!bytes.empty()) std::memcpy(*out, bytes.data(), bytes.size());
    *out_len = bytes.size();
    double acc = 0.0;
    if (ro.sq < (1ull << 53)) {
        acc = double(ro.sq);
    } else {
        const size_t psc = wav_len >= 44 ? (wav_len - 44) / (2 * size_t(ch)) : 0;
        for (int j = 0; j < ch; ++j)
            for (size_t i = 0; i < size_t(enc.sample_count()); ++i) {
                int16_t sv = 0;
                if (i < psc) std::memcpy(&sv, wav + 44 + (i * ch + j) * 2, 2);
                const double d = double(sv) - double(ro.pcm[i * ch + j]);
                acc += d * d;
            }
    }
    *psy_a_delta = n ? std::sqrt(acc / double(n)) : 0.0;
    *recon = ro.pcm;
    *recon_len = n;
    t_tim.total_ms = now_ms() - t0;
    return 0;
}

static std::vector<float> pad_rows(const float* x, int n, int d, int dp) {
    std::vector<float> v(size_t(n) * dp, 0.0f);
    for (int i = 0; i < n; ++i) std::memcpy(&v[size_t(i) * dp], x + size_t(i) * d, sizeof(float) * size_t(d));
    return v;
}

extern "C" hipError_t gsc_launch_yakmo_chain_test(int ppl, const float* pts, int nbk, float run, int* k_out,
                                                  float* out);

int gsc_yakmo_chain_test(int ppl, const float* pts, int nbk, float run, int* accepted, float* run_out, float* ck,
                         float* bmn, float* bmx) {
    if (ensure_device() != 0) return -1;
    if ((ppl != 8 && ppl != 16) || nbk < 1 || nbk > ppl) return fail("gsc_yakmo_chain_test: ppl 8 / 16, 1 <= nbk <= ppl");
    DevBuf<float> dP, dO;
    DevBuf<int> dK;
    HIP_TRY(dP.alloc(size_t(64) * nbk));
    HIP_TRY(dO.alloc(1 + 3 * 64));
    HIP_TRY(dK.alloc(1));
    HIP_TRY(hipMemcpy(dP.p, pts, sizeof(float) * 64 * size_t(nbk), hipMemcpyHostToDevice));
    HIP_TRY(gsc_launch_yakmo_chain_test(ppl, dP.p, nbk, run, dK.p, dO.p));
    HIP_TRY(hipDeviceSynchronize());
    float o[1 + 3 * 64];
    HIP_TRY(hipMemcpy(o, dO.p, sizeof(o), hipMemcpyDeviceToHost));
    HIP_TRY(hipMemcpy(accepted, dK.p, sizeof(int), hipMemcpyDeviceToHost));
    *run_out = o[0];
    for (int b = 0; b < nbk; ++b) {
        ck[b] = o[1 + b];
        bmn[b] = o[1 + 64 + b];
        bmx[b] = o[1 + 128 + b];
    }
    return 0;
}

int gsc_yakmo_seed_means(int n, int d0, const float* x, int k, float* centroids) {
    if (ensure_device() != 0) return -1;
    if (k >= n || k <= 0 || k > kMaxK) return fail("yakmo needs 0 < k < n, k <= 4096");
    if (d0 <= 0 || d0 > 32) return fail("yakmo: 1 <= d <= 32 features");
    const int d = feature_stride((d0 + 1) / 2);
    std::vector<float> X = pad_rows(x, n, d0, d), C;
    std::vector<int> cl, it, sl;
    const int nf = 1;
    std::vector<ReduceFrame> fr(1);
    fr[0] = ReduceFrame{};
    fr[0].N = n;
    fr[0].K = k;
    fr[0].k_off = n;
    DevBuf<float> dX, dC, dF, dYSum;
    DevBuf<int> dI;
    DevBuf<uint32_t> dBits;
    DevBuf<ReduceFrame> dFr;
    HIP_TRY(dX.alloc(X.size()));
    HIP_TRY(dC.alloc(size_t(k) * d));
    HIP_TRY(dF.alloc(size_t(n) * 4));
    HIP_TRY(dI.alloc(size_t(n) + size_t(k)));
    HIP_TRY(dBits.alloc(gsc_yakmo_big_words(n, 1)));
    HIP_TRY(dYSum.alloc(gsc_yakmo_big_floats(n, 1)));
    HIP_TRY(dFr.alloc(1));
    HIP_TRY(hipMemcpy(dX.p, X.data(), sizeof(float) * X.size(), hipMemcpyHostToDevice));
    HIP_TRY(hipMemcpy(dFr.p, fr.data(), sizeof(ReduceFrame), hipMemcpyHostToDevice));
    HIP_TRY(gsc_launch_yakmo(d, dFr.p, nf, dX.p, dC.p, dF.p, dI.p, dYSum.p, dBits.p, n, nullptr));
    HIP_TRY(hipDeviceSynchronize());
    C.resize(size_t(k) * d);
    HIP_TRY(hipMemcpy(C.data(), dC.p, sizeof(float) * size_t(k) * d, hipMemcpyDeviceToHost));
    compact_rows(&C, k, d, d0);
    std::memcpy(centroids, C.data(), sizeof(float) * size_t(k) * d0);
    (void)cl;
    (void)it;
    (void)sl;
    return 0;
}

int gsc_scan_reduce(int n, int d0, const float* x, int k, float* centroids, int* clusters, int precision, int* iters) {
    if (ensure_device() != 0) return -1;
    if (d0 <= 0 || d0 > 32) return fail("KNNScanReduce kernels support 1 <= d <= 32 features");
    const int d = feature_stride((d0 + 1) / 2);
    const std::vector<float> xp = pad_rows(x, n, d0, d);
    std::vector<float> cp = pad_rows(centroids, k, d0, d);
    x = xp.data();
    std::vector<ReduceFrame> fr(1);
    fr[0] = ReduceFrame{};
    fr[0].N = n;
    fr[0].K = k;
    fr[0].dcol = d0;
    fr[0].k_off = n;
    fr[0].ka_off = n + k;
    DevBuf<float> dX, dC, dRate, dF;
    DevBuf<int> dI;
    DevBuf<ReduceFrame> dFr;
    HIP_TRY(dF.alloc(size_t(n) * 4));
    HIP_TRY(dX.alloc(size_t(n) * d));
    HIP_TRY(dC.alloc(size_t(k) * d));
    HIP_TRY(dI.alloc(size_t(n) + size_t(k) + size_t(padded_k(k))));
    HIP_TRY(dFr.alloc(1));
    const std::vector<float> rt = rate_table(n);
    HIP_TRY(dRate.alloc(rt.size()));
    HIP_TRY(hipMemcpy(dX.p, x, sizeof(float) * size_t(n) * d, hipMemcpyHostToDevice));
    HIP_TRY(hipMemcpy(dC.p, cp.data(), sizeof(float) * size_t(k) * d, hipMemcpyHostToDevice));
    HIP_TRY(hipMemcpy(dRate.p, rt.data(), sizeof(float) * rt.size(), hipMemcpyHostToDevice));
    HIP_TRY(hipMemcpy(dFr.p, fr.data(), sizeof(ReduceFrame), hipMemcpyHostToDevice));
    HIP_TRY(launch_scan_passes(d, dFr.p, 1, k, dX.p, dC.p, dI.p, dF.p, dRate.p, precision));
    HIP_TRY(hipDeviceSynchronize());
    HIP_TRY(hipMemcpy(cp.data(), dC.p, sizeof(float) * size_t(k) * d, hipMemcpyDeviceToHost));
    compact_rows(&cp, k, d, d0);
    std::memcpy(centroids, cp.data(), sizeof(float) * size_t(k) * d0);
    HIP_TRY(hipMemcpy(clusters, dI.p, sizeof(int) * size_t(n), hipMemcpyDeviceToHost));
    HIP_TRY(hipMemcpy(fr.data(), dFr.p, sizeof(ReduceFrame), hipMemcpyDeviceToHost));
    if (iters) *iters = fr[0].iters;
    if (fr[0].loop_iters < 0) return fail("KNNScanReduce: batched pipeline made no progress (guard tripped)");
    if (std::getenv("GSC_SCAN_DEBUG"))
    {
        std::fprintf(stderr, "scan: passes %d slow %d restarts %d loop_iters(last pass) %d err %.9g tree_exact %d\n",
                     fr[0].iters, fr[0].slow, fr[0].restarts, fr[0].loop_iters, fr[0].err, fr[0].tree_exact);
        std::fprintf(stderr, "stamps [prep A1 A2 B2 part3 part4 B1 vcheck won setup soloA soloDFS a2win a2far a2box a2out]");
        for (int w = 0; w < 8; ++w) {
            std::fprintf(stderr, "\n  w%d:", w);
            for (int k = 0; k < 16; ++k) std::fprintf(stderr, " %.3g", double(fr[0].stamps[w * 16 + k]));
        }
        std::fprintf(stderr, "\nA1 queries [home pruned evaluated | iterations fixups pending | clk: box+home midbarrier]"
                             "\n  (one-CU frames: stamps slot 'vcheck' = A1 after the mid barrier + vp_end, slot 'A1' = the V check)");
        for (int w = 0; w < 8; ++w) {
            std::fprintf(stderr, "\n  w%d:", w);
            for (int k = 0; k < 8; ++k) std::fprintf(stderr, " %.4g", double(fr[0].acounts[w * 8 + k]));
        }
        const uint64_t* x = fr[0].xcounts;
        std::fprintf(stderr,
                     "\niterations [kind: count, cycles]: bubble %llu %.4g | with new queries %llu %.4g (new queries %llu)"
                     " | with fixups %llu %.4g | with a solo %llu %.4g | A2 queries on per-wave bounds %llu",
                     (unsigned long long)x[0], double(x[1]), (unsigned long long)x[2], double(x[3]),
                     (unsigned long long)x[8], (unsigned long long)x[4], double(x[5]), (unsigned long long)x[6],
                     double(x[7]), (unsigned long long)x[9]);
        std::fprintf(stderr, "\napproximate certificates failed: no unique minimum %llu, a far step not provable %llu",
                     (unsigned long long)x[10], (unsigned long long)x[11]);
        std::fprintf(stderr, "\nfailed queries by cause: snapshot uncertified %llu, c* moved past m2 %llu, V check %llu"
                     " (V check only %llu)", (unsigned long long)x[12], (unsigned long long)x[13],
                     (unsigned long long)x[14], (unsigned long long)x[15]);
        const uint64_t* x2 = fr[0].xcounts2;
        std::fprintf(stderr, "\nsolo answer = speculative c*: by cause uncertified %llu, m2 %llu, V %llu | solos with a remainder"
                             " %llu, of them same answer %llu (remainder queries valid to the next failure %llu, whole"
                             " remainder valid %llu)", (unsigned long long)x2[0], (unsigned long long)x2[1],
                     (unsigned long long)x2[2], (unsigned long long)x2[3], (unsigned long long)x2[4],
                     (unsigned long long)x2[5], (unsigned long long)x2[6]);
        std::fprintf(stderr, "\nin-batch DFS answers %llu, of them failing at commit %llu", (unsigned long long)x2[8],
                     (unsigned long long)x2[9]);
        std::fprintf(stderr, "\n");
    }
    return 0;
}

int gsc_birch_labels(int n, int d, const float* x, int k, int* labels) {
    if (!x || !labels || n <= 0 || d <= 0 || k <= 0) return fail("gsc_birch_labels: invalid argument");
    if (ensure_device() != 0) return -1;
    std::string err;
    if (birch_reduce_labels(n, d, x, k, labels, &err) != 0) return fail(err);
    return 0;
}

int gsc_knnfit_assign(int r, int cs, const float* cand_fwd, int n, const float* q, float eps, int* best) {
    if (ensure_device() != 0) return -1;
    std::vector<int> Rs{r}, Ns{n}, out;
    std::vector<float> E{eps}, C(cand_fwd, cand_fwd + size_t(r) * cs), Q(q, q + size_t(n) * cs);
    double ms = 0;
    if (run_knnfit_batch(cs, Rs, Ns, E, C, Q, &out, &ms) != 0) return -1;
    std::memcpy(best, out.data(), sizeof(int) * size_t(n));
    return 0;
}

void gsc_last_timing(gsc_timing* t) { *t = t_tim; }

int gsc_set_device(int device) {
    HIP_TRY(hipSetDevice(device));
    return 0;
}

int gsc_device_count(void) {
    int n = 0;
    if (hipGetDeviceCount(&n) != hipSuccess) return 0;
    return n;
}

const char* gsc_last_error(void) { return t_err.c_str(); }

void gsc_free(void* p) { std::free(p); }

}
```

soundchunks_amd/csrc/gsc_scan.hip:

```cpp
#include "gsc_tree.h"

namespace gsc {

#ifndef GSC_DFS_CALL_D
#define GSC_DFS_CALL_D 8
#endif
#ifndef GSC_VP_EARLY_D
#define GSC_VP_EARLY_D 32
#endif
#ifndef GSC_INBATCH_DFS_D
#define GSC_INBATCH_DFS_D 16
#endif
#ifndef GSC_EPSF8
#define GSC_EPSF8 0x1p-18f
#endif

template <int D_, int LOGK_, int SL_, int DR_ = D_>
struct ScanCfg {
    static constexpr int D = D_, LOGK = LOGK_, SL = SL_;
    static constexpr int DR = DR_, TL = D_ - DR_;
    static constexpr bool SPLIT = TL > 0;
    static constexpr int K = 1 << LOGK;
    static constexpr int LS = SL == 8 ? 3 : (SL == 4 ? 2 : (SL == 2 ? 1 : 0));
    static constexpr int LPW = 64 * SL;
    static constexpr bool FULL = K >= LPW;
    static constexpr int NWL = FULL ? K / LPW : 1;
    static constexpr int NWV = NWL;
    static constexpr int NT = 64 * NWL;
    static constexpr int KW = LOGK - 6 - LS >= 0 ? LOGK - 6 - LS : 0;
    static constexpr int KB = D > 16 ? 16 : 32;
    static constexpr int KVER = 64 + KB;
    static constexpr int QD = D < 16 ? 16 : D + 4;
    static constexpr int H = D / 2;
    static constexpr int ROW = D + 4;
    static constexpr float EPSF = D > 16 ? 0x1p-16f : (D > 8 ? 0x1p-17f : GSC_EPSF8);
    static_assert(NWV <= 16, "A2 evaluates up to 16 wave records per query (one per lane of a 16-lane group)");
    static_assert(KB <= 32 && 64 % KB == 0, "batch size");
    static_assert(!SPLIT || DR == H, "split layout: the DCT half in registers");
};

__device__ __forceinline__ uint32_t fminb(uint32_t a, uint32_t b) {
    return __float_as_uint(fminf(__uint_as_float(a), __uint_as_float(b)));
}
constexpr uint32_t kInfBits = 0x7F800000u;
__device__ __forceinline__ int ordkey(uint32_t b) { return (int)(b ^ ((uint32_t)((int32_t)b >> 31) >> 1)); }
__device__ __forceinline__ uint32_t keybits(int k) { return (uint32_t)ordkey((uint32_t)k); }

template <int SL>
struct WaveRecT {
    uint32_t minbits;
    int lanebits;
    uint32_t sl[6];
    uint32_t b[SL];
};

template <int SL>
__device__ __forceinline__ int rec_slot(const WaveRecT<SL>& r, bool* tie2) {
    int ls = SL - 1, lc = 0;
#pragma unroll
    for (int s = SL - 1; s >= 0; --s) {
        const bool e = r.b[s] == r.minbits;
        lc += e ? 1 : 0;
        ls = e ? s : ls;
    }
    *tie2 = lc > 1 || (r.lanebits >> 8) != 0;
    return ls;
}

template <int SL>
__device__ __forceinline__ uint32_t rec_sib(const WaveRecT<SL>& r, int ls, int idx) {
    if (idx < 6) return keybits((int)r.sl[idx]);
    if constexpr (SL >= 2) {
        if (idx == 6) return r.b[ls ^ 1];
    }
    if constexpr (SL >= 4) {
        if (SL == 4 || idx == 7) {
            const int pb = (ls & (SL - 4)) | ((ls & 2) ^ 2);
            return fminb(r.b[pb], r.b[pb + 1]);
        }
        const int qb = (ls & 4) ^ 4;
        return fminb(fminb(r.b[qb], r.b[qb + 1]), fminb(r.b[qb + 2], r.b[qb + 3]));
    }
    return kInfBits;
}

#ifndef GSC_MAX_IMP
#define GSC_MAX_IMP 8
#endif
constexpr int kMaxImp = GSC_MAX_IMP;

template <int D>
struct QRecT {
    int valid;
    int cstar;
    int id;
    float g;
    float m2;
    float rate;
    uint32_t farmask;
    int pad_;
    float B[16];
    float o[D];
    int nimp;
    int ir[kMaxImp];
};

template <class C>
struct Scan2Shared {
    KdTree t;
    union {
        float dist[kMaxK];
        WaveRecT<C::SL> wrec[C::NWV][C::KB + 1];
    };
    float rate[kMaxK];
    float dfs_inc[kMaxK];
    uint32_t dfs_near[kMaxK / 32];
    alignas(16) float q[2][C::KB][C::QD];
    alignas(16) float qm[2][C::KB][C::QD];
    float cnmax[C::NWV];
    float cnmax_h[C::NWV], cnmax_f[C::NWV];
    float ptlo[C::NWV][C::D], pthi[C::NWV][C::D];
    int xtlo[C::D], xthi[C::D];
    float wlo[C::NWV][C::D], whi[C::NWV][C::D];
    uint32_t ub[C::KB];
    int fxl[C::KB];
    alignas(16) float qslow[C::QD];
    alignas(16) QRecT<C::D> qrec[2][C::KB];
    QRecT<C::D> qsolo;
    alignas(16) float lg_c[64][C::ROW];
    int pub_pos[64];
    alignas(16) float solo_c[C::ROW];
    double err_out;
    int vcs[C::KB];
    alignas(16) int4 vmeta[C::KVER];
    alignas(16) float newc[2][C::KB][C::ROW];
    float gp[C::KB];
    int inval[C::KB];
    int nxt[2][C::KB];
    int ient[C::KB];
    int vie[C::KB];
    int freel[64];
    int asg[64];
    int slow_pos;
    float slow_key;
    int vc_next;
    int vp_ready;
    int any_nan;
    int nan_rows;
    uint32_t nanid[kMaxK / 32];
    int pass_done;
    uint32_t wkey[2][C::NWL];
    alignas(16) float a2s[C::NWL][C::D > 16 ? 2 : 1][64];
    alignas(16) float a2i[C::NWL][64];
};

#ifdef GSC_STAMPS
__device__ __forceinline__ uint64_t stamp() {
    uint64_t t;
    __builtin_amdgcn_sched_barrier(0);
    asm volatile("s_memtime %0\n\ts_waitcnt lgkmcnt(0)" : "=s"(t)::"memory");
    __builtin_amdgcn_sched_barrier(0);
    return t;
}
#define STAMP(k)                     \
    {                                \
        const uint64_t t_ = stamp(); \
        acc[k] += t_ - tlast;        \
        tlast = t_;                  \
    }
#else
#define STAMP(k)
#endif

template <int B>
__device__ __forceinline__ uint32_t partner(uint32_t v) {
    if constexpr (B == 0) return (uint32_t)__builtin_amdgcn_mov_dpp((int)v, 0xB1, 0xF, 0xF, true);
    if constexpr (B == 1) return (uint32_t)__builtin_amdgcn_mov_dpp((int)v, 0x4E, 0xF, 0xF, true);
    if constexpr (B == 2) return (uint32_t)__builtin_amdgcn_mov_dpp((int)v, 0x141, 0xF, 0xF, true);
    if constexpr (B == 3) return (uint32_t)__builtin_amdgcn_mov_dpp((int)v, 0x140, 0xF, 0xF, true);
    if constexpr (B == 4) return (uint32_t)__builtin_amdgcn_ds_swizzle((int)v, 0x401F);
    return 0u;
}
__device__ __forceinline__ uint32_t min16(uint32_t v) {
    v = min(v, partner<0>(v));
    v = min(v, partner<1>(v));
    v = min(v, partner<2>(v));
    return min(v, partner<3>(v));
}
__device__ __forceinline__ uint32_t fmin16(uint32_t v) {
    v = fminb(v, partner<0>(v));
    v = fminb(v, partner<1>(v));
    v = fminb(v, partner<2>(v));
    return fminb(v, partner<3>(v));
}
__device__ __forceinline__ uint32_t sum16(uint32_t v) {
    v += partner<0>(v);
    v += partner<1>(v);
    v += partner<2>(v);
    return v + partner<3>(v);
}

__device__ __forceinline__ int wave_of_lane() { return __builtin_amdgcn_readfirstlane(threadIdx.x >> 6); }

__device__ __forceinline__ int opaque_v(int v) {
    asm volatile("" : "+v"(v));
    return v;
}

__device__ __forceinline__ void wave_lds_sync() {
    __builtin_amdgcn_fence(__ATOMIC_SEQ_CST, "wavefront");
    __builtin_amdgcn_wave_barrier();
}

__device__ __forceinline__ void lds_barrier() {
    __builtin_amdgcn_fence(__ATOMIC_RELEASE, "workgroup", "local");
    __builtin_amdgcn_s_barrier();
    __builtin_amdgcn_fence(__ATOMIC_ACQUIRE, "workgroup", "local");
}

template <int D>
__device__ __forceinline__ float seqdist(const float* __restrict__ a, const float* __restrict__ b) {
    float s = 0.0f;
#pragma unroll
    for (int d = 0; d < D; ++d) {
        const float t = fsub(a[d], b[d]);
        s = fadd(s, fmul(t, t));
    }
    return s;
}

__device__ __forceinline__ int wave_min_i(int v) {
    v = min(v, (int)partner<0>((uint32_t)v));
    v = min(v, (int)partner<1>((uint32_t)v));
    v = min(v, (int)partner<2>((uint32_t)v));
    v = min(v, (int)partner<3>((uint32_t)v));
    v = min(v, (int)partner<4>((uint32_t)v));
    return min(__builtin_amdgcn_readlane(v, 0), __builtin_amdgcn_readlane(v, 32));
}
__device__ __forceinline__ int wave_max_i(int v) {
    v = max(v, (int)partner<0>((uint32_t)v));
    v = max(v, (int)partner<1>((uint32_t)v));
    v = max(v, (int)partner<2>((uint32_t)v));
    v = max(v, (int)partner<3>((uint32_t)v));
    v = max(v, (int)partner<4>((uint32_t)v));
    return max(__builtin_amdgcn_readlane(v, 0), __builtin_amdgcn_readlane(v, 32));
}

template <class C>
__device__ __forceinline__ void wave_box_init(Scan2Shared<C>& sh, const float (&creg)[C::SL][C::DR], int vwave, int lane,
                                              int p0, uint32_t dmask) {
    if constexpr (C::SPLIT) {
        if (lane == 0)
            for (int d = C::DR; d < C::D; ++d) {
                sh.wlo[vwave][d] = sh.ptlo[vwave][d];
                sh.whi[vwave][d] = sh.pthi[vwave][d];
            }
    }
#pragma unroll
    for (int d = 0; d < C::DR; ++d) {
        float lo = __builtin_inff(), hi = -__builtin_inff();
#pragma unroll
        for (int s = 0; s < C::SL; ++s)
            if (!((dmask >> s) & 1u)) {
                lo = fminf(lo, creg[s][d]);
                hi = fmaxf(hi, creg[s][d]);
            }
        const int klo = wave_min_i(ordkey(__float_as_uint(lo)));
        const int khi = wave_max_i(ordkey(__float_as_uint(hi)));
        if (lane == 0) {
            sh.wlo[vwave][d] = __uint_as_float(keybits(klo));
            sh.whi[vwave][d] = __uint_as_float(keybits(khi));
        }
    }
}

template <class C>
__device__ __forceinline__ float wave_box_lb(const Scan2Shared<C>& sh, const float* __restrict__ q, int w) {
    float lb = 0.0f;
#pragma unroll
    for (int d = 0; d < C::D; ++d) {
        const float qd = q[d], lo = sh.wlo[w][d], hi = sh.whi[w][d];
        const float t = fmaxf(fmaxf(fsub(lo, qd), fsub(qd, hi)), 0.0f);
        lb = fadd(lb, fmul(t, t));
    }
    return fmul(lb, 1.0f - 0x1p-17f);
}

template <int D, int SL>
__device__ __forceinline__ void a1_dist(const float (&creg)[SL][D], const float* __restrict__ qv, float (&dv)[SL]) {
#pragma unroll
    for (int s = 0; s < SL; ++s) dv[s] = 0.0f;
#pragma unroll
    for (int d = 0; d < D; ++d) {
        const float qd = qv[d];
#pragma unroll
        for (int s = 0; s < SL; ++s) {
            const float t = fsub(qd, creg[s][d]);
            dv[s] = fadd(dv[s], fmul(t, t));
        }
    }
}

template <int SL>
struct A1Tree {
    uint32_t b[SL];
    uint32_t lmin;
    int sl[6];
    uint64_t m;
};

template <class C>
__device__ __forceinline__ A1Tree<C::SL> a1_tree(const float (&dv)[C::SL], int vwave, int lane) {
    constexpr int SL = C::SL;
    const int p0 = (vwave * 64 + lane) * SL;
    A1Tree<SL> t;
    const bool has = C::FULL || p0 < C::K;
#pragma unroll
    for (int s = 0; s < SL; ++s) t.b[s] = has ? __float_as_uint(dv[s]) : kInfBits;
    if constexpr (SL == 1) {
        t.lmin = t.b[0];
    } else {
        uint32_t mm[SL / 2];
#pragma unroll
        for (int s = 0; s < SL / 2; ++s) mm[s] = fminb(t.b[2 * s], t.b[2 * s + 1]);
        if constexpr (SL == 8) {
            t.lmin = fminb(fminb(mm[0], mm[1]), fminb(mm[2], mm[3]));
        } else if constexpr (SL == 4) {
            t.lmin = fminb(mm[0], mm[1]);
        } else {
            t.lmin = mm[0];
        }
    }
    const int key = ordkey(t.lmin);
    int v = key;
    t.sl[0] = (int)partner<0>((uint32_t)v);
    v = min(v, t.sl[0]);
    t.sl[1] = (int)partner<1>((uint32_t)v);
    v = min(v, t.sl[1]);
    t.sl[2] = (int)partner<2>((uint32_t)v);
    v = min(v, t.sl[2]);
    t.sl[3] = (int)partner<3>((uint32_t)v);
    v = min(v, t.sl[3]);
    const auto p16 = __builtin_amdgcn_permlane16_swap((uint32_t)v, (uint32_t)v, false, false);
    t.sl[4] = (int)((lane & 16) ? p16[0] : p16[1]);
    v = min((int)p16[0], (int)p16[1]);
    const auto p32 = __builtin_amdgcn_permlane32_swap((uint32_t)v, (uint32_t)v, false, false);
    t.sl[5] = (int)((lane & 32) ? p32[0] : p32[1]);
    const int wmin = min((int)p32[0], (int)p32[1]);
    t.m = __ballot(key == wmin);
    return t;
}

template <int SL>
__device__ __forceinline__ void a1_store(const A1Tree<SL>& t, WaveRecT<SL>& rec, int lane) {
    const int L = __ffsll((long long)t.m) - 1;
    if (lane == L) {
        rec.minbits = t.lmin;
        rec.lanebits = L | (__popcll(t.m) > 1 ? 256 : 0);
#pragma unroll
        for (int i = 0; i < 6; ++i) rec.sl[i] = (uint32_t)t.sl[i];
#pragma unroll
        for (int s = 0; s < SL; ++s) rec.b[s] = t.b[s];
    }
}

template <class C>
__device__ __forceinline__ void a1_reduce(const float (&dv)[C::SL], WaveRecT<C::SL>& rec, int vwave, int lane) {
    a1_store<C::SL>(a1_tree<C>(dv, vwave, lane), rec, lane);
}

template <class C>
__device__ __forceinline__ void a1_reduce2(const float (&dv0)[C::SL], const float (&dv1)[C::SL], WaveRecT<C::SL>& rec0,
                                           WaveRecT<C::SL>& rec1, int vwave, int lane) {
    const A1Tree<C::SL> t0 = a1_tree<C>(dv0, vwave, lane);
    const A1Tree<C::SL> t1 = a1_tree<C>(dv1, vwave, lane);
    a1_store<C::SL>(t0, rec0, lane);
    a1_store<C::SL>(t1, rec1, lane);
}

__device__ __forceinline__ float wave_max_nonneg(float x) {
    uint32_t k = __float_as_uint(x);
    k = max(k, partner<0>(k));
    k = max(k, partner<1>(k));
    k = max(k, partner<2>(k));
    k = max(k, partner<3>(k));
    k = max(k, partner<4>(k));
    k = max((uint32_t)__builtin_amdgcn_readlane((int)k, 0), (uint32_t)__builtin_amdgcn_readlane((int)k, 32));
    return __uint_as_float(k);
}

__device__ __forceinline__ float wave_min_nonneg(float x) {
    uint32_t k = __float_as_uint(x);
    k = min(k, partner<0>(k));
    k = min(k, partner<1>(k));
    k = min(k, partner<2>(k));
    k = min(k, partner<3>(k));
    k = min(k, partner<4>(k));
    k = min((uint32_t)__builtin_amdgcn_readlane((int)k, 0), (uint32_t)__builtin_amdgcn_readlane((int)k, 32));
    return __uint_as_float(k);
}

template <class C>
__device__ __forceinline__ void a1_query(const float (&creg)[C::SL][C::DR], const float* __restrict__ qv,
                                         WaveRecT<C::SL>& rec, int vwave, int lane, uint32_t dmask,
                                         const float* __restrict__ trow = nullptr, int p0 = 0, float tw = 0.0f) {
    float dv[C::SL];
    a1_dist<C::DR, C::SL>(creg, qv, dv);
    if constexpr (C::SPLIT) {
        float ml = __builtin_inff();
#pragma unroll
        for (int s = 0; s < C::SL; ++s) ml = ((dmask >> s) & 1u) ? ml : fminf(ml, dv[s]);
        const float U = fmul(fadd(wave_min_nonneg(ml), tw), 1.0f + 0x1p-18f);
#pragma unroll
        for (int s = 0; s < C::SL; ++s)
            if (!((dmask >> s) & 1u) && dv[s] <= U) {
                const float* tr = trow + (int64_t)(p0 + s) * C::TL;
                float a = dv[s];
#pragma unroll
                for (int d = 0; d < C::TL; ++d) {
                    const float t = fsub(qv[C::DR + d], tr[d]);
                    a = fadd(a, fmul(t, t));
                }
                dv[s] = a;
            }
    }
#pragma unroll
    for (int s = 0; s < C::SL; ++s) dv[s] = ((dmask >> s) & 1u) ? __builtin_inff() : dv[s];
    a1_reduce<C>(dv, rec, vwave, lane);
}

template <int DD, int D, int SL>
__device__ __forceinline__ void a1_dist_x2(const float (&creg)[SL][D], const float (&cn)[SL],
                                           const float* __restrict__ qm0, const float* __restrict__ qm1,
                                           float (&dv0)[SL], float (&dv1)[SL]) {
#pragma unroll
    for (int s = 0; s < SL; ++s) {
        dv0[s] = cn[s];
        dv1[s] = cn[s];
    }
#pragma unroll
    for (int d = 0; d < DD; ++d) {
        const float m0 = qm0[d], m1 = qm1[d];
#pragma unroll
        for (int s = 0; s < SL; ++s) {
            dv0[s] = __builtin_fmaf(m0, creg[s][d], dv0[s]);
            dv1[s] = __builtin_fmaf(m1, creg[s][d], dv1[s]);
        }
    }
}

template <int D>
__device__ __forceinline__ float norm2_x(const float* __restrict__ v) {
    float n = 0.0f;
#pragma unroll
    for (int d = 0; d < D; ++d) n = __builtin_fmaf(v[d], v[d], n);
    return n;
}

__device__ __forceinline__ float fsum16(float v) {
    v = fadd(v, __uint_as_float(partner<0>(__float_as_uint(v))));
    v = fadd(v, __uint_as_float(partner<1>(__float_as_uint(v))));
    v = fadd(v, __uint_as_float(partner<2>(__float_as_uint(v))));
    return fadd(v, __uint_as_float(partner<3>(__float_as_uint(v))));
}

template <class C, bool APPROX>
__device__ __forceinline__ void a2_group(Scan2Shared<C>& sh, int j0, int nq, const float (*qrows)[C::QD],
                                         QRecT<C::D>* recs, int wcol0, const int* jlist, int lane,
                                         bool half = false, float twh = 0.0f, float te = 0.0f, bool nanpass = false
#ifdef GSC_STAMPS
                                         , uint64_t* acc = nullptr, uint64_t* tl = nullptr, uint64_t* xc = nullptr
#endif
) {
#ifdef GSC_STAMPS
#define ASTAMP(k)                          \
    if (acc) {                             \
        const uint64_t t_ = stamp();       \
        acc[k] += t_ - *tl;                \
        *tl = t_;                          \
    }
#else
#define ASTAMP(k)
#endif
    constexpr int D = C::D, LOGK = C::LOGK, NW = C::NWV, SL = C::SL, LS = C::LS;
    constexpr int KW = C::KW;
    const int l = lane & 15, gbase = lane & ~15;
    const int t = j0 + (lane >> 4);
    const bool qa = t < nq;
    const int tr = qa ? t : j0;
    const int jr = jlist ? jlist[tr] : tr;
    const int jj = jr;
    const int wc = wcol0 + jr;
    const uint32_t mw = (l < NW) ? sh.wrec[l][wc].minbits : kInfBits;
    const uint32_t gmin = fmin16(mw);
    const uint32_t nmin = sum16((mw == gmin && l < NW) ? 1u : 0u);
    const int W = (int)min16((mw == gmin && l < NW) ? (uint32_t)l : 99u);
    const int Wv = W < NW ? W : 0;
    const WaveRecT<SL>& r = sh.wrec[Wv][wc];
    bool tie2;
    const int ls = rec_slot<SL>(r, &tie2);
    const int cstar = (Wv * 64 + (r.lanebits & 255)) * SL + ls;
    const bool tie = nmin > 1 || tie2;
    const float* q = qrows[jr];
    ASTAMP(12)
    uint32_t sib = kInfBits;
    if (l < KW) {
        const int sh_ = KW - 1 - l;
        const int want = (W >> sh_) ^ 1;
#pragma unroll
        for (int w = 0; w < NW; ++w)
            if ((w >> sh_) == want) sib = fminb(sib, sh.wrec[w][wc].minbits);
    } else if (l < LOGK) {
        const int idx = l < LOGK - LS ? (LOGK - LS - 1 - l) : (6 + (LOGK - 1 - l));
        sib = rec_sib<SL>(r, ls, idx);
    }
    bool far = false;
    float inc = 0.0f;
    if (l < LOGK) {
        const int h = (1 << l) - 1 + (cstar >> (LOGK - l));
        const bool golo = ((cstar >> (LOGK - 1 - l)) & 1) == 0;
        const int cdim = sh.t.cd[h];
        const float qc = q[cdim];
        const float cut = fsub(qc, sh.t.cv[h]);
        const bool nearlo = cut < 0.0f;
        if (golo != nearlo) {
            float bd = nearlo ? fsub(sh.t.lo[h], qc) : fsub(qc, sh.t.hi[h]);
            if (bd < 0.0f) bd = 0.0f;
            far = true;
            inc = fsub(fmul(cut, cut), fmul(bd, bd));
        }
    }
    const uint32_t farmask = (uint32_t)(__ballot(far) >> gbase) & 0xFFFFu;
    ASTAMP(13)
    constexpr int NH = D > 16 ? 2 : 1;
    {
#pragma unroll
        for (int hh = 0; hh < NH; ++hh) {
            const int dd = l + 16 * hh;
            float term = -1.0f;
            if (dd < D) {
                const float qd = q[dd], blo = sh.t.bnd_lo[dd], bhi = sh.t.bnd_hi[dd];
                const bool below = blo > qd, above = qd > bhi;
                const float tt = below ? fsub(blo, qd) : fsub(qd, bhi);
                term = (below || above) ? fmul(tt, tt) : -1.0f;
            }
            sh.a2s[wave_of_lane()][hh][lane] = term;
        }
        sh.a2i[wave_of_lane()][lane] = inc;
    }
    wave_lds_sync();
    float box = 0.0f;
    {
#pragma unroll
        for (int d = 0; d < D; ++d) {
            const float v = sh.a2s[wave_of_lane()][d >> 4][gbase + (d & 15)];
            box = v >= 0.0f ? fadd(box, v) : box;
        }
    }
    float incs[LOGK];
#pragma unroll
    for (int k = 0; k < LOGK; ++k) incs[k] = sh.a2i[wave_of_lane()][gbase + k];
    wave_lds_sync();
    float bp[LOGK];
#pragma unroll
    for (int k = 0; k < LOGK; ++k) {
        bp[k] = -__builtin_inff();
        if ((farmask >> k) & 1u) {
            box = fadd(box, incs[k]);
            bp[k] = box;
        }
    }
    float Bv = -__builtin_inff(), run = -__builtin_inff();
#pragma unroll
    for (int k = LOGK - 1; k >= 0; --k) {
        run = fmaxf(run, bp[k]);
        Bv = (l == k) ? run : Bv;
    }
    ASTAMP(14)
    const uint32_t m2 = fmin16(sib);
    bool ok, unique;
    float m2lo;
    if constexpr (APPROX) {
        const int dn = half ? C::H : D;
        const float qs = l < dn ? q[l] : 0.0f;
        const float qs2 = (D > 16 && l + 16 < dn) ? q[l + 16] : 0.0f;
        const float qn0 = fsum16(__builtin_fmaf(qs2, qs2, __builtin_fmaf(qs, qs, 0.0f)));
        float M = 0.0f;
#pragma unroll
        for (int w = 0; w < NW; ++w) M = fmaxf(M, sh.cnmax[w]);
        const float eps = fadd(fadd(fmul(fadd(qn0, M), C::EPSF), 1e-37f), te);
        const float qn = fadd(qn0, twh);
#ifndef GSC_NO_LEAF_EPS
        const float eg = fmul(fadd(qn0, M), C::EPSF);
        auto epsv = [&](uint32_t vb) {
            const float v = __uint_as_float(vb);
            const float dq = fmaxf(fadd(fadd(qn0, v), fadd(eg, eg)), 0.0f);
            const float cb = fmul(fadd(fadd(qn0, qn0), fadd(dq, dq)), 1.0f + 0x1p-20f);
            return fadd(fadd(fmul(fadd(qn0, fminf(cb, M)), C::EPSF), 1e-37f), te);
        };
        const float es = epsv(gmin), e2 = epsv(m2), eb = epsv(sib);
        ok = !far || (fsub(fadd(qn, __uint_as_float(sib)), eb) > Bv);
        unique = fsub(__uint_as_float(m2), __uint_as_float(gmin)) > fadd(es, e2);
        m2lo = fsub(fadd(qn, __uint_as_float(m2)), e2);
#else
        ok = !far || (fsub(fadd(qn, __uint_as_float(sib)), eps) > Bv);
        unique = fsub(__uint_as_float(m2), __uint_as_float(gmin)) > fadd(eps, eps);
        m2lo = fsub(fadd(qn, __uint_as_float(m2)), eps);
#endif
        const bool gfail = !unique || ((__ballot(!ok) >> gbase) & 0xFFFFull) != 0;
#ifdef GSC_STAMPS
        if (xc) xc[9] += __popcll(__ballot(gfail && l == 0 && qa));
#endif
        if (__ballot(gfail) != 0) {
            auto epsw = [&](int w) { return fadd(fadd(fmul(fadd(qn0, sh.cnmax[w]), C::EPSF), 1e-37f), te); };
            const float eW = epsw(Wv);
            float eS = eW;
            if (l < KW) {
                const int sh_ = KW - 1 - l;
                const int want = (W >> sh_) ^ 1;
                eS = 0.0f;
#pragma unroll
                for (int w = 0; w < NW; ++w)
                    if ((w >> sh_) == want) eS = fmaxf(eS, epsw(w));
            }
            ok = !far || (fsub(fadd(qn, __uint_as_float(sib)), eS) > Bv);
            const float gm = __uint_as_float(gmin);
            const float m2W = __uint_as_float(fmin16((l >= KW && l < LOGK) ? sib : kInfBits));
            const bool ow = l < NW && l != Wv;
            const float el = ow ? epsw(l) : 0.0f;
            const bool uw = !ow || fsub(__uint_as_float(mw), gm) > fadd(eW, el);
            unique = fsub(m2W, gm) > fadd(eW, eW) && ((__ballot(!uw) >> gbase) & 0xFFFFull) == 0;
            const float lo_l = ow ? fsub(fadd(qn, __uint_as_float(mw)), el) : __builtin_inff();
            m2lo = fminf(fsub(fadd(qn, m2W), eW), __uint_as_float(fmin16(__float_as_uint(lo_l))));
        }
    } else {
        ok = !far || (__uint_as_float(sib) > Bv);
        unique = !tie;
        m2lo = __uint_as_float(m2);
    }
    if (far && inc != inc) ok = false;
    const bool gok = ((__ballot(!ok) >> gbase) & 0xFFFFull) == 0;
    const bool valid = unique && __uint_as_float(gmin) <= FLT_MAX && gok;
#ifdef GSC_STAMPS
    if (xc && APPROX) {
        xc[10] += __popcll(__ballot(qa && l == 0 && !unique));
        xc[11] += __popcll(__ballot(qa && l == 0 && unique && !gok));
    }
#endif
    int nanf = -1;
    if (APPROX && nanpass && qa && l == 0 && farmask != 0) {
        int h = 0, pos = 0;
#pragma unroll 1
        for (int lv = 0; lv < LOGK; ++lv) {
            const int bit = fsub(q[sh.t.cd[h]], sh.t.cv[h]) < 0.0f ? 0 : 1;
            pos = 2 * pos + bit;
            h = 2 * h + 1 + bit;
        }
        const int id = sh.t.pidx[pos];
        if (id != 0xFFFF && ((sh.nanid[id >> 5] >> (id & 31)) & 1u)) nanf = pos;
    }
    if (qa) {
        QRecT<D>& R = recs[jj];
        if (l < LOGK) R.B[l] = Bv;
        if (l == 0) {
            const int cs = nanf >= 0 ? nanf : cstar;
            R.valid = (valid || nanf >= 0) ? 1 : 0;
            R.cstar = cs;
            R.id = sh.t.pidx[cs];
            R.g = nanf >= 0 ? __builtin_nanf("") : __uint_as_float(gmin);
            R.m2 = m2lo;
            R.rate = sh.rate[cs];
            R.farmask = farmask;
            R.pad_ = nanf >= 0 ? 1 : 0;
        }
    }
    ASTAMP(15)
    (void)LS;
}
#undef ASTAMP

struct VPState {
    int cs, pred, nxt, first, ie;
};

template <class C>
__device__ __forceinline__ void vp_begin(Scan2Shared<C>& sh, int qb, int off, int pn, int a1, int lane, int& lg_pos,
                                         int lg_tag, VPState& st) {
    if (lg_pos >= 0 && lg_tag < a1) lg_pos = -1;
    st.cs = lane < pn ? (sh.qrec[qb][off + lane].pad_ ? -100 - lane : sh.qrec[qb][off + lane].cstar) : -2;
    sh.vmeta[lane].x = lg_pos;
    sh.vmeta[lane].y = 0;
    if (lane < C::KB) sh.vcs[lane] = st.cs;
    uint32_t* qm = reinterpret_cast<uint32_t*>(sh.dfs_inc);
    const int cs = st.cs;
    const bool qv = lane < C::KB && cs >= 0;
    if (qv) qm[cs] = 0u;
    if (lg_pos >= 0) qm[lg_pos] = 0u;
    if (lane < C::KB) sh.vie[lane] = 64;
    wave_lds_sync();
    if (qv) atomicOr(&qm[cs], 1u << lane);
    wave_lds_sync();
    const uint32_t mq = qv ? qm[cs] : 0u;
    const uint32_t me = lg_pos >= 0 ? qm[lg_pos] : 0u;
    const uint32_t below = lane < 32 ? (1u << lane) - 1u : ~0u;
    const uint32_t above = lane < 31 ? ~((2u << lane) - 1u) : 0u;
    const uint32_t mb = mq & below, ma = mq & above;
    st.pred = mb ? 64 + (31 - __clz(mb)) : -1;
    st.nxt = ma ? __ffs(ma) - 1 : C::KB;
    st.first = me ? __ffs(me) - 1 : C::KB;
    for (uint32_t m = me; m; m &= m - 1u) atomicMin(&sh.vie[__ffs(m) - 1], lane);
    wave_lds_sync();
    st.ie = lane < C::KB ? sh.vie[lane] : 64;
}

template <class C>
__device__ __forceinline__ void vp_end(Scan2Shared<C>& sh, int qb, int off, int pn, int lane, int lg_pos,
                                       const VPState& st, bool half, int par) {
    constexpr int D = C::D, KB = C::KB;
    const int j = lane;
    const bool act = j < pn;
    const QRecT<D>& R = sh.qrec[qb][off + (act ? j : 0)];
    const int cs = st.cs, nxt = st.nxt;
    const int ie = st.ie < 64 ? st.ie : -1;
    const int pred = st.pred >= 0 ? st.pred : ie;
    sh.vmeta[lane].z = lg_pos >= 0 ? st.first : -1;
    if (lane < KB) {
        sh.vmeta[64 + lane] = make_int4(act ? cs : -1, j + 1, act ? nxt : -1, 0);
        sh.nxt[par][lane] = nxt;
        sh.ient[lane] = ie;
        sh.inval[lane] = 0;
    }
    uint64_t done = ~__ballot(act);
    for (;;) {
        const bool ready = act && !((done >> j) & 1ull) && (pred < 64 || ((done >> (pred - 64)) & 1ull));
        const uint64_t rm = __ballot(ready);
        if (!rm) break;
        if (ready) {
            const float* qv = sh.q[qb][off + j];
            const float* o = pred < 0 ? R.o : (pred < 64 ? sh.lg_c[pred] : sh.newc[par][pred - 64]);
            float oc[D];
#pragma unroll
            for (int d = 0; d < D; ++d) oc[d] = o[d];
            const bool nanq = R.pad_ != 0;
            const float gpj = nanq ? __builtin_nanf("") : seqdist<D>(qv, oc);
            const bool okc = nanq || (R.valid != 0 && (pred < 0 || gpj < R.m2));
            const float rate = R.rate;
            float nrm = 0.0f;
#pragma unroll
            for (int d = 0; d < D; ++d) {
                const float nc = fadd(oc[d], fmul(fsub(qv[d], oc[d]), rate));
                sh.newc[par][j][d] = nc;
                if (d < C::H || !half) nrm = __builtin_fmaf(nc, nc, nrm);
            }
            sh.newc[par][j][C::ROW - 1] = nrm;
            sh.gp[j] = gpj;
#ifdef GSC_STAMPS
            if (!okc) sh.inval[j] = R.valid == 0 ? 1 : (R.valid == 2 ? 8 : 2);
#else
            if (!okc) sh.inval[j] = 1;
#endif
        }
        wave_lds_sync();
        done |= rm;
    }
}

template <int LOGK, int D>
__device__ __forceinline__ bool dfs_keeps(const QRecT<D>& R, float du, int vp, float g) {
    const int n = R.nimp;
#pragma unroll 1
    for (int i = n - 1; i >= 0; --i) {
        const int x = R.ir[i];
        const int pos = x & 4095, rk = x >> 12;
        if (vp == pos) return false;
        const int l = __clz((uint32_t)(vp ^ pos)) - (32 - LOGK);
        if (((rk >> (LOGK - 1 - l)) & 1) == 0) return !(du < (i == n - 1 ? g : R.B[i]));
    }
    return false;
}

template <class C>
__device__ __forceinline__ void v_check_grab(Scan2Shared<C>& sh, int qb, int off, int pn, int lane, int par) {
    constexpr int D = C::D, KB = C::KB, QPL = 64 / KB, LOGK = C::LOGK;
    constexpr int VPT = 2 * QPL;
    constexpr int NTRIP = (C::KVER + VPT - 1) / VPT;
    int t = 0;
    if (lane == 0) t = atomicAdd(&sh.vc_next, 1);
    t = __builtin_amdgcn_readfirstlane(t);
    if (t >= NTRIP) return;
    const int j = lane % KB, grp = lane / KB;
    const int jr = j < pn ? j : 0;
    const QRecT<D>& R = sh.qrec[qb][off + jr];
    const bool act = j < pn && R.pad_ == 0;
    const bool dfsa = R.valid == 2;
    const int cs = R.cstar;
    const uint32_t fm = R.farmask;
    const float g = sh.gp[jr];
    float q[D];
#pragma unroll
    for (int d = 0; d < D; ++d) q[d] = sh.q[qb][off + jr][d];
    bool bad = false;
#pragma unroll 1
    while (t < NTRIP) {
        int tn = 0;
        if (lane == 0) tn = atomicAdd(&sh.vc_next, 1);
        const int v0 = t * VPT + 2 * grp;
        const bool h0 = v0 < C::KVER, h1 = v0 + 1 < C::KVER;
        const int v0s = h0 ? v0 : 0, v1 = h1 ? v0 + 1 : v0s;
        const int4 m0 = sh.vmeta[v0s], m1 = sh.vmeta[v1];
        const int vp0 = h0 ? m0.x : -1, vp1 = h1 ? m1.x : -1;
        const bool u0 = (vp0 >= 0) & act & (j >= m0.y) & (j <= m0.z) & (vp0 != cs);
        const bool u1 = (vp1 >= 0) & act & (j >= m1.y) & (j <= m1.z) & (vp1 != cs);
        if (u0 || u1) {
            const float* c0 = v0s < 64 ? sh.lg_c[v0s] : sh.newc[par][v0s - 64];
            const float* c1 = v1 < 64 ? sh.lg_c[v1] : sh.newc[par][v1 - 64];
            const int lca0 = __clz(vp0 ^ cs) - (32 - LOGK), lca1 = __clz(vp1 ^ cs) - (32 - LOGK);
            const float b0 = R.B[lca0 & 15], b1 = R.B[lca1 & 15];
            float du0 = 0.0f, du1 = 0.0f;
#pragma unroll
            for (int d = 0; d < D; ++d) {
                const float t0 = fsub(q[d], c0[d]), t1 = fsub(q[d], c1[d]);
                du0 = fadd(du0, fmul(t0, t0));
                du1 = fadd(du1, fmul(t1, t1));
            }
            const bool far0 = (fm >> (lca0 & 31)) & 1u, far1 = (fm >> (lca1 & 31)) & 1u;
            if (!dfsa) {
                if (u0 && !(du0 > g && (!far0 || du0 > b0))) bad = true;
                if (u1 && !(du1 > g && (!far1 || du1 > b1))) bad = true;
            } else {
                if (u0 && !dfs_keeps<LOGK, D>(R, du0, vp0, g)) bad = true;
                if (u1 && !dfs_keeps<LOGK, D>(R, du1, vp1, g)) bad = true;
            }
        }
        t = __builtin_amdgcn_readfirstlane(tn);
    }
#ifdef GSC_STAMPS
    if (bad) atomicOr(&sh.inval[j], 4);
#else
    if (bad) sh.inval[j] = 1;
#endif
}

template <class C>
__device__ __forceinline__ void dfs_parallel(Scan2Shared<C>& sh, const float* __restrict__ q, int tid, int lane,
                                             int wave, int& out_pos, float& out_key, QRecT<C::D>* rec = nullptr) {
    constexpr int D = C::D, LOGK = C::LOGK, NW = C::NWL;
    constexpr int K = 1 << LOGK;
    constexpr int nthreads = 64 * NW;
    for (int h = tid; h < K - 1; h += nthreads) {
        const int cdim = sh.t.cd[h];
        const float qc = q[cdim];
        const float cut = fsub(qc, sh.t.cv[h]);
        const bool nearlo = cut < 0.0f;
        float bd = nearlo ? fsub(sh.t.lo[h], qc) : fsub(qc, sh.t.hi[h]);
        if (bd < 0.0f) bd = 0.0f;
        const float inc = fsub(fmul(cut, cut), fmul(bd, bd));
        sh.dfs_inc[h] = nearlo ? inc : -inc;
    }
    float rootbox = 0.0f;
#pragma unroll
    for (int d = 0; d < D; ++d) {
        const float qd = q[d];
        if (sh.t.bnd_lo[d] > qd) {
            const float t = fsub(sh.t.bnd_lo[d], qd);
            rootbox = fadd(rootbox, fmul(t, t));
        } else if (qd > sh.t.bnd_hi[d]) {
            const float t = fsub(qd, sh.t.bnd_hi[d]);
            rootbox = fadd(rootbox, fmul(t, t));
        }
    }
    lds_barrier();
    const int p0 = tid * 8;
    int rs[8];
    float bxs[8];
    {
        float box = rootbox, bF = 0.0f;
        int pref = 0, sF = -1, h = 0;
        for (int l = 0; l < LOGK - 3; ++l) {
            const int bit = (p0 >> (LOGK - 1 - l)) & 1;
            const float v = sh.dfs_inc[h];
            if (bit != (int)(__float_as_uint(v) >> 31)) {
                box = fadd(box, fabsf(v));
                sF = pref + (1 << (LOGK - 1 - l));
                bF = box;
                pref += 1 << (LOGK - 1 - l);
            }
            h = 2 * h + 1 + bit;
        }
#pragma unroll
        for (int s = 0; s < 8; ++s) {
            float box2 = box, bF2 = bF;
            int pref2 = pref, sF2 = sF, h2 = h;
#pragma unroll
            for (int l = LOGK - 3; l < LOGK; ++l) {
                const int bit = ((p0 + s) >> (LOGK - 1 - l)) & 1;
                const float v = sh.dfs_inc[h2];
                if (bit != (int)(__float_as_uint(v) >> 31)) {
                    box2 = fadd(box2, fabsf(v));
                    sF2 = pref2 + (1 << (LOGK - 1 - l));
                    bF2 = box2;
                    pref2 += 1 << (LOGK - 1 - l);
                }
                h2 = 2 * h2 + 1 + bit;
            }
            rs[s] = (pref2 << 13) | (sF2 + 1);
            bxs[s] = bF2;
        }
    }
    int pos = -1, bp = -1, par = 0, nimp = 0;
    float b = FLT_MAX;
    for (;;) {
        uint32_t key = 0xFFFFFFFFu;
#pragma unroll
        for (int s = 0; s < 8; ++s) {
            const int rk = rs[s] >> 13, st = (rs[s] & 8191) - 1;
            const bool reach = st <= pos || bxs[s] < b;
            if (p0 + s < K && rk > pos && reach && sh.dist[p0 + s] < b)
                key = min(key, ((uint32_t)rk << 12) | (uint32_t)(p0 + s));
        }
        key = min(key, partner<0>(key));
        key = min(key, partner<1>(key));
        key = min(key, partner<2>(key));
        key = min(key, partner<3>(key));
        key = min(key, partner<4>(key));
        key = min((uint32_t)__builtin_amdgcn_readlane((int)key, 0), (uint32_t)__builtin_amdgcn_readlane((int)key, 32));
        if (lane == 0) sh.wkey[par][wave] = key;
        lds_barrier();
        uint32_t g = 0xFFFFFFFFu;
#pragma unroll
        for (int w = 0; w < NW; ++w) g = min(g, sh.wkey[par][w]);
        par ^= 1;
        if (g == 0xFFFFFFFFu) break;
        pos = (int)(g >> 12);
        bp = (int)(g & 4095u);
        b = sh.dist[bp];
        if (rec && tid == 0 && nimp < kMaxImp) {
            rec->ir[nimp] = (int)g;
            rec->B[nimp] = b;
        }
        ++nimp;
    }
    if (rec && tid == 0) rec->nimp = nimp;
    out_pos = bp;
    out_key = b;
}

template <class C>
__device__ __noinline__ void dfs_parallel_call(Scan2Shared<C>& sh, const float* __restrict__ q, int tid, int lane,
                                               int wave, int& out_pos, float& out_key, QRecT<C::D>* rec) {
    dfs_parallel<C>(sh, q, tid, lane, wave, out_pos, out_key, rec);
}

template <class C>
__device__ __noinline__ void dfs_parallel_nan(Scan2Shared<C>& sh, const float* __restrict__ q, int tid, int lane,
                                                 int wave, int& out_pos, float& out_key, QRecT<C::D>* rec) {
    constexpr int D = C::D, LOGK = C::LOGK, NW = C::NWL;
    constexpr int K = 1 << LOGK;
    constexpr int nthreads = 64 * NW;
    for (int h0 = 0; h0 < K; h0 += nthreads) {
        const int h = h0 + tid;
        bool nearlo = false;
        if (h < K - 1) {
            const float qc = q[sh.t.cd[h]];
            const float cut = fsub(qc, sh.t.cv[h]);
            nearlo = cut < 0.0f;
            float bd = nearlo ? fsub(sh.t.lo[h], qc) : fsub(qc, sh.t.hi[h]);
            if (bd < 0.0f) bd = 0.0f;
            sh.dfs_inc[h] = fsub(fmul(cut, cut), fmul(bd, bd));
        }
        const uint64_t m = __ballot(nearlo);
        if (lane == 0) {
            sh.dfs_near[(h0 + wave * 64) >> 5] = (uint32_t)m;
            sh.dfs_near[((h0 + wave * 64) >> 5) + 1] = (uint32_t)(m >> 32);
        }
    }
    float rootbox = 0.0f;
#pragma unroll
    for (int d = 0; d < D; ++d) {
        const float qd = q[d];
        if (sh.t.bnd_lo[d] > qd) {
            const float t = fsub(sh.t.bnd_lo[d], qd);
            rootbox = fadd(rootbox, fmul(t, t));
        } else if (qd > sh.t.bnd_hi[d]) {
            const float t = fsub(qd, sh.t.bnd_hi[d]);
            rootbox = fadd(rootbox, fmul(t, t));
        }
    }
    lds_barrier();
    const int p0 = tid * 8;
    constexpr int LT = LOGK - 3;
    float smt[LT + 1];
    int preft = 0;
    float boxt = rootbox;
    int ht = 0;
    {
        float fb[LT];
#pragma unroll
        for (int l = 0; l < LT; ++l) {
            const int bit = (p0 >> (LOGK - 1 - l)) & 1;
            const int nearbit = ((sh.dfs_near[ht >> 5] >> (ht & 31)) & 1u) ? 0 : 1;
            fb[l] = -__builtin_inff();
            if (bit != nearbit) {
                boxt = fadd(boxt, sh.dfs_inc[ht]);
                preft += 1 << (LOGK - 1 - l);
                fb[l] = boxt != boxt ? __builtin_inff() : boxt;
            }
            ht = 2 * ht + 1 + bit;
        }
        smt[LT] = -__builtin_inff();
#pragma unroll
        for (int l = LT - 1; l >= 0; --l) smt[l] = fmaxf(fb[l], smt[l + 1]);
    }
    int rk[8];
    float sb[8][3];
#pragma unroll
    for (int s8 = 0; s8 < 8; ++s8) {
        float box = boxt, fb[3];
        int pref = preft, h = ht;
#pragma unroll
        for (int j = 0; j < 3; ++j) {
            const int l = LT + j;
            const int bit = ((p0 + s8) >> (LOGK - 1 - l)) & 1;
            const int nearbit = ((sh.dfs_near[h >> 5] >> (h & 31)) & 1u) ? 0 : 1;
            fb[j] = -__builtin_inff();
            if (bit != nearbit) {
                box = fadd(box, sh.dfs_inc[h]);
                pref += 1 << (LOGK - 1 - l);
                fb[j] = box != box ? __builtin_inff() : box;
            }
            h = 2 * h + 1 + bit;
        }
        rk[s8] = pref;
        sb[s8][2] = fb[2];
        sb[s8][1] = fmaxf(fb[1], fb[2]);
        sb[s8][0] = fmaxf(fb[0], sb[s8][1]);
    }
    int pos = -1, bp = -1, par = 0, nimp = 0;
    float b = FLT_MAX;
    for (;;) {
        uint32_t key = 0xFFFFFFFFu;
        const int gt = preft >> 3, gp = pos >> 3;
        if (gt > gp) {
            const int t = 31 - __builtin_clz((uint32_t)(preft ^ pos));
            const int lt = max(0, LOGK - 1 - t);
            float mt = smt[0];
#pragma unroll
            for (int l = 1; l < LT; ++l) mt = l == lt ? smt[l] : mt;
#pragma unroll
            for (int s8 = 0; s8 < 8; ++s8) {
                const float M = fmaxf(mt, sb[s8][0]);
                if (p0 + s8 < K && M < b && sh.dist[p0 + s8] < b)
                    key = min(key, ((uint32_t)rk[s8] << 12) | (uint32_t)(p0 + s8));
            }
        } else if (gt == gp) {
#pragma unroll
            for (int s8 = 0; s8 < 8; ++s8) {
                const int x = (rk[s8] ^ pos) & 7;
                if (rk[s8] > pos && x != 0) {
                    const int t = 31 - __builtin_clz((uint32_t)x);
                    const float M = t == 2 ? sb[s8][0] : (t == 1 ? sb[s8][1] : sb[s8][2]);
                    if (p0 + s8 < K && M < b && sh.dist[p0 + s8] < b)
                        key = min(key, ((uint32_t)rk[s8] << 12) | (uint32_t)(p0 + s8));
                }
            }
        }
        key = min(key, partner<0>(key));
        key = min(key, partner<1>(key));
        key = min(key, partner<2>(key));
        key = min(key, partner<3>(key));
        key = min(key, partner<4>(key));
        key = min((uint32_t)__builtin_amdgcn_readlane((int)key, 0), (uint32_t)__builtin_amdgcn_readlane((int)key, 32));
        if (lane == 0) sh.wkey[par][wave] = key;
        lds_barrier();
        uint32_t g = 0xFFFFFFFFu;
#pragma unroll
        for (int w = 0; w < NW; ++w) g = min(g, sh.wkey[par][w]);
        par ^= 1;
        if (g == 0xFFFFFFFFu) break;
        pos = (int)(g >> 12);
        bp = (int)(g & 4095u);
        b = sh.dist[bp];
        if (rec && tid == 0 && nimp < kMaxImp) {
            rec->ir[nimp] = (int)g;
            rec->B[nimp] = b;
        }
        ++nimp;
    }
    if (rec && tid == 0) rec->nimp = nimp;
    out_pos = bp;
    out_key = b;
}

template <class C>
__device__ __forceinline__ void refresh(Scan2Shared<C>& sh, float (&creg)[C::SL][C::DR], float (&cn)[C::SL],
                                        float& cnmax, int vwave, int lane, float* __restrict__ trow = nullptr) {
    constexpr int SL = C::SL, LS = C::LS, D = C::D, DR = C::DR;
    const int pp = sh.pub_pos[lane];
    uint64_t m = __ballot(pp >= 0 && (pp >> (6 + LS)) == vwave);
    if (!m) return;
    float blo = __builtin_inff(), bhi = -__builtin_inff();
    auto apply = [&](int e, int p, const float* r, float nv) {
        const int owner = (p >> LS) & 63, slot = p & (SL - 1);
#pragma unroll
        for (int s = 0; s < SL; ++s) {
            if (s == slot) {
#pragma unroll
                for (int d = 0; d < DR; ++d) creg[s][d] = lane == owner ? r[d] : creg[s][d];
                cn[s] = lane == owner ? nv : cn[s];
            }
        }
        if constexpr (C::SPLIT) {
            if (lane == owner)
                for (int d = DR; d < D; ++d) trow[(int64_t)p * C::TL + (d - DR)] = sh.lg_c[e][d];
        }
    };
    constexpr bool PAIR = DR <= 8;
    while (m) {
        const int e0 = __ffsll((long long)m) - 1;
        m &= m - 1;
        const bool two = PAIR && m != 0;
        const int e1 = two ? __ffsll((long long)m) - 1 : e0;
        if (two) m &= m - 1;
        const int p0 = __builtin_amdgcn_readlane(pp, e0), p1 = __builtin_amdgcn_readlane(pp, e1);
        float r0[DR], r1[PAIR ? DR : 1];
#pragma unroll
        for (int d = 0; d < DR; ++d) {
            r0[d] = sh.lg_c[e0][d];
            if constexpr (PAIR) r1[d] = sh.lg_c[e1][d];
        }
        const float nv0 = sh.lg_c[e0][C::ROW - 1], nv1 = sh.lg_c[e1][C::ROW - 1];
        if (lane < D) {
            const float v0 = sh.lg_c[e0][lane], v1 = sh.lg_c[e1][lane];
            blo = fminf(blo, fminf(v0, v1));
            bhi = fmaxf(bhi, fmaxf(v0, v1));
        }
        cnmax = fmaxf(cnmax, fmaxf(nv0, nv1));
        apply(e0, p0, r0, nv0);
        if constexpr (PAIR) {
            if (two) apply(e1, p1, r1, nv1);
        }
    }
    if (lane < D) {
        sh.wlo[vwave][lane] = fminf(sh.wlo[vwave][lane], blo);
        sh.whi[vwave][lane] = fmaxf(sh.whi[vwave][lane], bhi);
    }
    if (lane == 0) sh.cnmax[vwave] = cnmax;
}

template <class C>
__device__ __forceinline__ void fold_commits(Scan2Shared<C>& sh, float (&creg)[C::SL][C::DR], float (&cn)[C::SL],
                                             float& cnmax, int vwave, int lane, int qb, int off, int kc, int par,
                                             float* __restrict__ trow = nullptr) {
    constexpr int SL = C::SL, LS = C::LS, D = C::D, DR = C::DR;
    int pp = 0;
    bool mine = false;
    if (lane < kc) {
        const QRecT<D>& R = sh.qrec[qb][off + lane];
        pp = R.cstar;
        mine = sh.nxt[par][lane] >= kc && R.pad_ == 0 && (pp >> (6 + LS)) == vwave;
    }
    uint64_t m = __ballot(mine);
    if (!m) return;
    float blo = __builtin_inff(), bhi = -__builtin_inff();
    auto apply = [&](int e, int p, const float* r, float nv) {
        const int owner = (p >> LS) & 63, slot = p & (SL - 1);
#pragma unroll
        for (int s = 0; s < SL; ++s) {
            if (s == slot) {
#pragma unroll
                for (int d = 0; d < DR; ++d) creg[s][d] = lane == owner ? r[d] : creg[s][d];
                cn[s] = lane == owner ? nv : cn[s];
            }
        }
        if constexpr (C::SPLIT) {
            if (lane == owner)
                for (int d = DR; d < D; ++d) trow[(int64_t)p * C::TL + (d - DR)] = sh.newc[par][e][d];
        }
    };
    constexpr bool PAIR = DR <= 8;
    while (m) {
        const int e0 = __ffsll((long long)m) - 1;
        m &= m - 1;
        const bool two = PAIR && m != 0;
        const int e1 = two ? __ffsll((long long)m) - 1 : e0;
        if (two) m &= m - 1;
        const int p0 = __builtin_amdgcn_readlane(pp, e0), p1 = __builtin_amdgcn_readlane(pp, e1);
        float r0[DR], r1[PAIR ? DR : 1];
#pragma unroll
        for (int d = 0; d < DR; ++d) {
            r0[d] = sh.newc[par][e0][d];
            if constexpr (PAIR) r1[d] = sh.newc[par][e1][d];
        }
        const float nv0 = sh.newc[par][e0][C::ROW - 1], nv1 = sh.newc[par][e1][C::ROW - 1];
        if (lane < D) {
            const float v0 = sh.newc[par][e0][lane], v1 = sh.newc[par][e1][lane];
            blo = fminf(blo, fminf(v0, v1));
            bhi = fmaxf(bhi, fmaxf(v0, v1));
        }
        cnmax = fmaxf(cnmax, fmaxf(nv0, nv1));
        apply(e0, p0, r0, nv0);
        if constexpr (PAIR) {
            if (two) apply(e1, p1, r1, nv1);
        }
    }
    if (lane < D) {
        sh.wlo[vwave][lane] = fminf(sh.wlo[vwave][lane], blo);
        sh.whi[vwave][lane] = fmaxf(sh.whi[vwave][lane], bhi);
    }
    if (lane == 0) sh.cnmax[vwave] = cnmax;
}

template <class C>
__device__ __forceinline__ void write_cstar(Scan2Shared<C>& sh, const float (&creg)[C::SL][C::DR], QRecT<C::D>* recs,
                                            uint64_t qmask, int col0, int wave, int lane,
                                            const float* __restrict__ trow = nullptr) {
    constexpr int SL = C::SL, D = C::D, NWL = C::NWL;
    uint64_t won;
    int ol = 0;
    {
        const bool act = (qmask >> lane) & 1ull;
        const int jq = act ? lane : 0;
        float gm = __builtin_inff();
        int W = 0;
#pragma unroll
        for (int w = 0; w < NWL; ++w) {
            const float m = __uint_as_float(sh.wrec[w][col0 + jq].minbits);
            if (m < gm) {
                gm = m;
                W = w;
            }
        }
        won = __ballot(act && W == wave);
        if (act && W == wave) {
            const WaveRecT<SL>& r = sh.wrec[wave][col0 + jq];
            bool tie2;
            const int slot = rec_slot<SL>(r, &tie2);
            ol = ((r.lanebits & 255) << 8) | slot;
        }
    }
    while (won) {
        const int jj = __ffsll((long long)won) - 1;
        won &= won - 1;
        const int o = __builtin_amdgcn_readlane(ol, jj);
        const int owner = o >> 8, slot = o & 255;
        float* dst = recs[jj].o;
#pragma unroll
        for (int s = 0; s < SL; ++s)
            if (s == slot && lane == owner) {
#pragma unroll
                for (int d = 0; d < C::DR; ++d) dst[d] = creg[s][d];
                if constexpr (C::SPLIT) {
                    const float* tr = trow + (int64_t)((wave * 64 + owner) * SL + s) * C::TL;
                    for (int d = C::DR; d < D; ++d) dst[d] = tr[d - C::DR];
                }
            }
    }
}

template <class C>
__global__ __launch_bounds__(C::NT) void scan_batch_kernel(ReduceFrame* __restrict__ frames, int nframes,
                                                           const float* __restrict__ Xall, float* __restrict__ Call,
                                                           int* __restrict__ i_scratch,
                                                           const float* __restrict__ rate_tab, double tol,
                                                           int max_passes, int opts,
                                                           float* __restrict__ Tall) {
    constexpr int D = C::D, K = C::K, SL = C::SL, LS = C::LS, NWL = C::NWL, KB = C::KB;
    constexpr int kErrWave = NWL > 1 ? 1 : 0;
    constexpr bool PRUNE = true;
    constexpr bool kInBatchDfs = D <= GSC_INBATCH_DFS_D;
    const bool no_half = (opts & 1) != 0;
    const bool no_prune = (opts & 2) != 0;
    const int kbe = ((opts >> 8) & 255) > 0 && ((opts >> 8) & 255) < KB ? ((opts >> 8) & 255) : KB;
    extern __shared__ __attribute__((aligned(16))) unsigned char smem[];
    Scan2Shared<C>& sh = *reinterpret_cast<Scan2Shared<C>*>(smem);
    const int tid = threadIdx.x, lane = tid & 63, wave = tid >> 6;
    constexpr int nthreads = C::NT;
    const int vwave = wave;
    const int fi0 = blockIdx.x, fstep = nframes;
    for (int fi = fi0; fi < nframes; fi += fstep) {
    ReduceFrame* frp = frames + fi;
    if (uniform_int(frp->done) || uniform_int(frp->generic)) continue;
    const int N = uniform_int(frp->N);
    const int dcol_i = uniform_int(frp->dcol) > 0 ? uniform_int(frp->dcol) : D;
    auto per_col = [dcol_i](float v) { return dcol_i == D ? v / (float)D : v / (float)dcol_i; };
    const int Kr = uniform_int(frp->K);
    const bool padded = Kr != K;
    const float* __restrict__ X = Xall + uniform_i64(frp->x_off);
    float* C_ = Call + uniform_i64(frp->c_off);
    int* clusters = i_scratch + uniform_i64(frp->n_off);
    int* prev_cnt = i_scratch + uniform_i64(frp->k_off);
    int* cnta = i_scratch + uniform_i64(frp->ka_off);
    float* trow = C::SPLIT ? Tall + uniform_i64(frp->t_off) : nullptr;
    double prev_err = uniform_int(frp->iters) == 0 ? 3.4028234663852886e+38 : frp->err;
    if constexpr (PRUNE) {
        constexpr int NT_ = D - C::H;
        static_assert(nthreads % NT_ == 0, "each thread keeps one tail feature");
        __syncthreads();
        if (tid < D) {
            sh.xtlo[tid] = 0x7FFFFFFF;
            sh.xthi[tid] = (int)0x80000000;
        }
        __syncthreads();
        int klo = 0x7FFFFFFF, khi = (int)0x80000000;
        const int d = C::H + tid % NT_;
        for (int64_t r = tid / NT_; r < N; r += nthreads / NT_) {
            const int k = ordkey(__float_as_uint(X[r * D + d]));
            klo = min(klo, k);
            khi = max(khi, k);
        }
        atomicMin(&sh.xtlo[d], klo);
        atomicMax(&sh.xthi[d], khi);
        __syncthreads();
    }

    for (int pass = uniform_int(frp->iters); pass < max_passes; ++pass) {
#ifdef GSC_STAMPS
    const uint64_t t_kernel0 = stamp();
#endif
    if (pass == 0)
        for (int k = tid; k < Kr; k += nthreads) prev_cnt[k] = 1;
    if (tid == 0) sh.any_nan = 0;
    for (int w = tid; w < kMaxK / 32; w += nthreads) sh.nanid[w] = 0u;
    __syncthreads();
    int nan_rows = 0;
    for (int k = tid; k < Kr; k += nthreads) {
        bool nn = false;
#pragma unroll
        for (int d = 0; d < D; ++d) nn |= C_[(int64_t)k * D + d] != C_[(int64_t)k * D + d];
        if (nn) {
            atomicOr(&sh.nanid[k >> 5], 1u << (k & 31));
            nan_rows = 1;
        }
    }
    nan_rows = __syncthreads_or(nan_rows);
    if (padded) {
        build_tree<D>(sh.t, sh.dist, C_, Kr);
        pad_tree<C::LOGK>(sh.t, reinterpret_cast<int*>(sh.dist), Kr, tid, nthreads);
    } else if (nan_rows) {
        if constexpr (K / nthreads >= 4)
            build_tree_nan<D, C::LOGK, nthreads>(sh.t, sh.dist, sh.dfs_inc, C_);
        else
            build_tree<D>(sh.t, sh.dist, C_, K);
    } else if constexpr (K / nthreads < 4) {
        build_tree<D>(sh.t, sh.dist, C_, K);
    } else if (!build_tree_fast<D, C::LOGK, nthreads>(sh.t, sh.dist, sh.dfs_inc, C_, &sh.slow_pos)) {
        build_tree<D>(sh.t, sh.dist, C_, K);
        if (tid == 0) frp->tree_exact += 1;
    }

    float creg[SL][C::DR];
    float cn[SL];
    const int p0 = (vwave * 64 + lane) * SL;
    bool nan_here = false;
    uint32_t dmask = 0;
    constexpr int TLA = C::TL > 0 ? C::TL : 1;
    float tlo[TLA], thi[TLA];
#pragma unroll
    for (int d = 0; d < TLA; ++d) {
        tlo[d] = __builtin_inff();
        thi[d] = -__builtin_inff();
    }
#pragma unroll
    for (int s = 0; s < SL; ++s) {
        const int p = p0 + s;
        const int id = p < K ? (int)sh.t.pidx[p] : 0xFFFF;
        bool dead = false;
        if (nan_rows && p < K) {
#pragma unroll 1
            for (int l = 0, h = 0; l < C::LOGK; ++l) {
                const int bit = (p >> (C::LOGK - 1 - l)) & 1;
                dead |= bit == 0 && sh.t.cv[h] != sh.t.cv[h];
                h = 2 * h + 1 + bit;
            }
        }
        if (id != 0xFFFF && !dead && !((sh.nanid[id >> 5] >> (id & 31)) & 1u)) {
#pragma unroll
            for (int d = 0; d < C::DR; ++d) {
                creg[s][d] = C_[(int64_t)id * D + d];
                nan_here |= creg[s][d] != creg[s][d];
            }
            if constexpr (C::SPLIT) {
#pragma unroll
                for (int d = 0; d < C::TL; ++d) {
                    const float v = C_[(int64_t)id * D + C::DR + d];
                    trow[(int64_t)p * C::TL + d] = v;
                    nan_here |= v != v;
                    tlo[d] = fminf(tlo[d], v);
                    thi[d] = fmaxf(thi[d], v);
                }
            }
        } else {
            dmask |= 1u << s;
#pragma unroll
            for (int d = 0; d < C::DR; ++d) creg[s][d] = 0.0f;
        }
        cn[s] = (dmask >> s) & 1u ? __builtin_inff() : norm2_x<C::DR>(creg[s]);
    }
    if constexpr (PRUNE) {
        float mh = 0.0f;
#pragma unroll
        for (int s = 0; s < SL; ++s) mh = fmaxf(mh, (dmask >> s) & 1u ? 0.0f : norm2_x<C::H>(creg[s]));
        mh = wave_max_nonneg(nan_here ? 0.0f : mh);
        if (lane == 0) sh.cnmax_h[vwave] = mh;
#pragma unroll
        for (int d = C::H; d < D; ++d) {
            float lo = __builtin_inff(), hi = -__builtin_inff();
            if constexpr (C::SPLIT) {
                lo = tlo[d - C::H];
                hi = thi[d - C::H];
            } else {
#pragma unroll
                for (int s = 0; s < SL; ++s)
                    if (!((dmask >> s) & 1u)) {
                        lo = fminf(lo, creg[s][d < C::DR ? d : 0]);
                        hi = fmaxf(hi, creg[s][d < C::DR ? d : 0]);
                    }
            }
            const int klo = wave_min_i(ordkey(__float_as_uint(lo)));
            const int khi = wave_max_i(ordkey(__float_as_uint(hi)));
            if (lane == 0) {
                sh.ptlo[vwave][d] = __uint_as_float(keybits(klo));
                sh.pthi[vwave][d] = __uint_as_float(keybits(khi));
            }
        }
    }
    for (int p = tid; p < K; p += nthreads) {
        const int id = sh.t.pidx[p];
        sh.rate[p] = id != 0xFFFF ? rate_tab[prev_cnt[id]] : 0.0f;
        cnta[p] = 1;
    }
    if (nan_here) sh.any_nan = 1;
    float cnmax;
    {
        float mx = 0.0f;
#pragma unroll
        for (int s = 0; s < SL; ++s) mx = fmaxf(mx, (dmask >> s) & 1u ? 0.0f : cn[s]);
        cnmax = wave_max_nonneg(nan_here ? 0.0f : mx);
        if (lane == 0) {
            sh.cnmax[vwave] = cnmax;
            sh.cnmax_f[vwave] = cnmax;
        }
    }
    if constexpr (PRUNE) {
        wave_box_init<C>(sh, creg, vwave, lane, p0, dmask);
        if (tid < KB) sh.ub[tid] = kInfBits;
    }
    if (tid == 0) {
        sh.vc_next = 0;
        sh.vp_ready = 0;
    }
    const int n0 = min(kbe, N);
    for (int k = tid; k < n0 * D; k += nthreads) {
        const float x = X[k];
        sh.q[0][k / D][k % D] = x;
        sh.qm[0][k / D][k % D] = -2.0f * x;
    }
    __syncthreads();
    bool half = false;
    float twh = 0.0f, te = 0.0f, tw_pass = 0.0f;
    if constexpr (PRUNE) {
        float tw = 0.0f, tn = 0.0f;
#pragma unroll
        for (int d = C::H; d < D; ++d) {
            float lo = __uint_as_float(keybits(sh.xtlo[d])), hi = __uint_as_float(keybits(sh.xthi[d]));
#pragma unroll
            for (int w = 0; w < C::NWV; ++w) {
                lo = fminf(lo, sh.ptlo[w][d]);
                hi = fmaxf(hi, sh.pthi[w][d]);
            }
            const float mag = fmaxf(fabsf(lo), fabsf(hi));
            const float wd = fadd(fsub(hi, lo), fadd(fmul(mag, 0x1p-20f), 1e-30f));
            tw = fadd(tw, fmul(wd, wd));
            tn = fadd(tn, fmul(mag, mag));
        }
        tw = fmul(tw, 1.0f + 0x1p-10f);
        tw_pass = tw;
        float mh = 0.0f;
#pragma unroll
        for (int w = 0; w < C::NWV; ++w) mh = fmaxf(mh, sh.cnmax_h[w]);
        twh = fmul(tw, 0.5f);
        te = fadd(twh, fmul(fmul(fmul(tn, 2.0f), C::EPSF), 1.0f + 0x1p-10f));
        half = !(tw != tw) && te <= fmul(fmul(mh, C::EPSF), 0.25f) && !uniform_int(sh.any_nan) && !no_half;
    }
    if (uniform_int(sh.any_nan) || (C::SPLIT && !half)) {
        if (tid == 0) frp->generic = 1;
        break;
    }
    if (half) {
#pragma unroll
        for (int s = 0; s < SL; ++s) cn[s] = (dmask >> s) & 1u ? __builtin_inff() : norm2_x<C::H>(creg[s]);
        cnmax = sh.cnmax_h[vwave];
        __syncthreads();
        if (lane == 0) sh.cnmax[vwave] = cnmax;
        __syncthreads();
    }

    int lg_pos = -1, lg_tag = 0;
    double err = 0.0;
    int slow_total = 0, restarts = 0;
    int ib_try = 0, ib_fail = 0;
    bool guard = false;
#ifdef GSC_STAMPS
    uint64_t acc[16] = {0, 0, 0, 0, 0, 0, 0, 0, 0, 0, 0, 0, 0, 0, 0, 0};
    uint64_t acn[8] = {0, 0, 0, 0, 0, 0, 0, 0};
    uint64_t xc[16] = {0, 0, 0, 0, 0, 0, 0, 0, 0, 0, 0, 0, 0, 0, 0, 0};
    uint64_t xc2[16] = {0, 0, 0, 0, 0, 0, 0, 0, 0, 0, 0, 0, 0, 0, 0, 0};
    uint64_t tlast = stamp();
    acc[9] = tlast - t_kernel0;
#endif
    int vq_buf0 = 0, vq_s0 = 0, vq_off0 = 0, vq_n0 = 0, vq_a10 = 0;
    int vq_buf1 = 0, vq_s1 = 0, vq_off1 = 0, vq_n1 = 0, vq_a11 = 0;
    int nvq = 0;
    int cur_buf = 0, cur_s = 0, cur_n = n0;
    auto exact_dists = [&](const float* __restrict__ qe) {
        float dv[SL];
#pragma unroll
        for (int s = 0; s < SL; ++s) dv[s] = 0.0f;
#pragma unroll
        for (int d = 0; d < C::DR; ++d) {
            const float qd = qe[d];
#pragma unroll
            for (int s = 0; s < SL; ++s) {
                const float t = fsub(qd, creg[s][d]);
                dv[s] = fadd(dv[s], fmul(t, t));
            }
        }
        if constexpr (C::SPLIT) {
#pragma unroll
            for (int s = 0; s < SL; ++s) {
                const float* tr = trow + (int64_t)(p0 + s) * C::TL;
                if (!((dmask >> s) & 1u))
                    for (int d = 0; d < C::TL; ++d) {
                        const float t = fsub(qe[C::DR + d], tr[d]);
                        dv[s] = fadd(dv[s], fmul(t, t));
                    }
            }
        }
#pragma unroll
        for (int s = 0; s < SL; ++s)
            if (p0 + s < K) sh.dist[p0 + s] = ((dmask >> s) & 1u) ? __builtin_inff() : dv[s];
    };
    int next_load = n0;
    for (int it = 0;; ++it) {
        int ln = opaque_v(lane);
#ifdef GSC_STAMPS
        const uint64_t t_it0 = stamp();
        const bool it_bubble = cur_n == 0;
        bool it_fix = false;
#endif
        const bool has_p = nvq > 0;
        const int P_buf = vq_buf0, P_s = vq_s0, P_off = vq_off0, P_n = has_p ? vq_n0 : 0;
        VPState vst;
#ifdef GSC_STAMPS_PREP
        STAMP(14)
#endif
        if (wave == 0 && has_p) vp_begin<C>(sh, P_buf, P_off, P_n, vq_a10, ln, lg_pos, lg_tag, vst);
        constexpr bool kVpEarly = D <= GSC_VP_EARLY_D;
        if constexpr (kVpEarly) {
            if (wave == 0 && has_p) {
                vp_end<C>(sh, P_buf, P_off, P_n, ln, lg_pos, vst, half, it & 1);
                wave_lds_sync();
                if (ln == 0) __hip_atomic_store(&sh.vp_ready, it + 1, __ATOMIC_RELEASE, __HIP_MEMORY_SCOPE_WORKGROUP);
            }
        }
        constexpr int PE = (KB * D + nthreads - 1) / nthreads;
        float pre[PE];
#pragma unroll
        for (int e = 0; e < PE; ++e) {
            const int k = tid + e * nthreads;
            pre[e] = (k < KB * D && next_load + k / D < N) ? X[(int64_t)next_load * D + k] : 0.0f;
        }
        STAMP(0)
        auto a1_mask = [&](uint64_t m) {
#pragma unroll 1
            while (m) {
                const int j0 = __ffsll((long long)m) - 1;
                m &= m - 1;
                const int j1 = m ? __ffsll((long long)m) - 1 : j0;
                if (m) m &= m - 1;
                float dv0[SL], dv1[SL];
                if (C::SPLIT || half)
                    a1_dist_x2<C::H, C::DR, SL>(creg, cn, sh.qm[cur_buf][j0], sh.qm[cur_buf][j1], dv0, dv1);
                else if constexpr (!C::SPLIT)
                    a1_dist_x2<D, D, SL>(creg, cn, sh.qm[cur_buf][j0], sh.qm[cur_buf][j1], dv0, dv1);
                a1_reduce2<C>(dv0, dv1, sh.wrec[vwave][j0], sh.wrec[vwave][j1], vwave, ln);
            }
        };
        const uint64_t curm = cur_n > 0 ? (cur_n >= 64 ? ~0ull : (1ull << cur_n) - 1ull) : 0ull;
#ifdef GSC_STAMPS
        const int cur_n_it = cur_n;
#endif
        uint64_t prunedm = 0;
        float lbp = 0.0f, qn_j = 0.0f, eps_j = 0.0f;
        if constexpr (PRUNE) {
            if (no_prune) {
                a1_mask(curm);
            } else if (cur_n > 0) {
                const int jr = ln < cur_n ? ln : 0;
                const float* qv = sh.q[cur_buf][jr];
                lbp = wave_box_lb<C>(sh, qv, vwave);
                qn_j = half ? norm2_x<C::H>(qv) : norm2_x<D>(qv);
                float M = 0.0f;
#pragma unroll
                for (int w = 0; w < C::NWV; ++w) M = fmaxf(M, sh.cnmax[w]);
                eps_j = fadd(fadd(fmul(fadd(qn_j, M), C::EPSF), 1e-37f), te);
                qn_j = fadd(qn_j, twh);
                const uint64_t home = __ballot(lbp == 0.0f) & curm;
                a1_mask(home);
                wave_lds_sync();
                if ((home >> ln) & 1ull) {
                    const float m = __uint_as_float(sh.wrec[vwave][ln].minbits);
                    const float ubd = fmul(fadd(fadd(qn_j, m), eps_j), 1.0f + 0x1p-20f);
                    atomicMin(&sh.ub[ln], __float_as_uint(fmaxf(ubd, 0.0f)));
                }
#ifdef GSC_STAMPS
                const uint64_t tm0_ = stamp();
                acn[6] += tm0_ - tlast;
#endif
                lds_barrier();
#ifdef GSC_STAMPS
                {
                    const uint64_t tm1_ = stamp();
                    acn[7] += tm1_ - tm0_;
                    tlast = tm1_;
                }
#endif
                const float ubj = __uint_as_float(sh.ub[jr]);
                const float thr = fmul(fadd(ubj, fmul(4.0f, eps_j)), 1.0f + 0x1p-20f);
                prunedm = __ballot(lbp > thr) & curm & ~home;
#ifdef GSC_STAMPS
                acn[0] += __popcll(home);
                acn[1] += __popcll(prunedm);
                acn[2] += __popcll(curm & ~home & ~prunedm);
#endif
                if ((prunedm >> ln) & 1ull)
                    sh.wrec[vwave][ln].minbits = __float_as_uint(fsub(fsub(lbp, fmul(3.0f, eps_j)), qn_j));
                a1_mask(curm & ~home & ~prunedm);
            }
        } else {
            a1_mask(curm);
        }
        if constexpr (!kVpEarly) {
            if (wave == 0 && has_p) vp_end<C>(sh, P_buf, P_off, P_n, ln, lg_pos, vst, half, it & 1);
        }
        {
            STAMP(7)
            if (has_p) {
                if (wave == 0) {
                    if constexpr (!kVpEarly) {
                        wave_lds_sync();
                        if (ln == 0)
                            __hip_atomic_store(&sh.vp_ready, it + 1, __ATOMIC_RELEASE, __HIP_MEMORY_SCOPE_WORKGROUP);
                    }
                } else {
                    while (__hip_atomic_load(&sh.vp_ready, __ATOMIC_ACQUIRE, __HIP_MEMORY_SCOPE_WORKGROUP) != it + 1)
                        __builtin_amdgcn_s_sleep(1);
                }
                v_check_grab<C>(sh, P_buf, P_off, P_n, ln, it & 1);
            }
        }
#ifdef GSC_STAMPS
        acn[3] += 1;
        acn[5] += P_n;
#endif
        STAMP(1)
        lds_barrier();
        STAMP(6)
        ln = opaque_v(ln);
        int fj = -1;
        if (has_p) {
            const uint64_t bad = __ballot(ln < P_n && sh.inval[ln] != 0);
            fj = bad ? __ffsll((long long)bad) - 1 : -1;
        }
        const int kc = has_p ? (fj >= 0 ? fj : P_n) : 0;
        if (kInBatchDfs && fj >= 0) ib_fail += uniform_int(sh.qrec[P_buf][P_off + fj].valid) == 2 ? 1 : 0;
#ifdef GSC_STAMPS
        int fj_cause = 0;
        if (fj >= 0) {
            const int cause = sh.inval[fj];
            fj_cause = cause;
            xc2[9] += sh.qrec[P_buf][P_off + fj].valid == 2 ? 1 : 0;
            xc[12] += (cause & 1) ? 1 : 0;
            xc[13] += (cause & 2) ? 1 : 0;
            xc[14] += (cause & 4) ? 1 : 0;
            xc[15] += (cause & 4) && (cause & 3) == 0 ? 1 : 0;
        }
#endif
        if (wave == 0 && fj >= 0 && ln < D) sh.qslow[ln] = sh.q[P_buf][P_off + fj][ln];
        const int A_buf = cur_buf, A_n = cur_n;
        const int solo_j = fj >= 0 ? P_s + P_off + fj : -1;
        if (has_p) {
            if (fj >= 0 && fj + 1 < P_n) {
                vq_off0 = P_off + fj + 1;
                vq_n0 = P_n - fj - 1;
            } else {
                vq_buf0 = vq_buf1;
                vq_s0 = vq_s1;
                vq_off0 = vq_off1;
                vq_n0 = vq_n1;
                vq_a10 = vq_a11;
                --nvq;
            }
        }
        if (cur_n > 0) {
            if (nvq == 0) {
                vq_buf0 = cur_buf;
                vq_s0 = cur_s;
                vq_off0 = 0;
                vq_n0 = cur_n;
                vq_a10 = it;
            } else {
                vq_buf1 = cur_buf;
                vq_s1 = cur_s;
                vq_off1 = 0;
                vq_n1 = cur_n;
                vq_a11 = it;
            }
            ++nvq;
        }
        cur_n = 0;
        const int freeb = nvq == 0 ? (fj >= 0 ? P_buf ^ 1 : 0) : (nvq == 1 ? vq_buf0 ^ 1 : -1);
        if (freeb >= 0 && !(fj >= 0 && freeb == P_buf) && !(A_n > 0 && freeb == A_buf) && next_load < N) {
            cur_buf = freeb;
            cur_s = next_load;
            cur_n = min(kbe, N - next_load);
            next_load += cur_n;
#pragma unroll
            for (int e = 0; e < PE; ++e) {
                const int k = tid + e * nthreads;
                if (k < cur_n * D) {
                    sh.q[cur_buf][k / D][k % D] = pre[e];
                    sh.qm[cur_buf][k / D][k % D] = -2.0f * pre[e];
                }
            }
        }
        if (tid == 0) sh.vc_next = 0;
        if (PRUNE && wave == 0 && ln < KB) sh.ub[ln] = kInfBits;
        STAMP(4)
        if (A_n > 0) {
            write_cstar<C>(sh, creg, sh.qrec[A_buf], (1ull << A_n) - 1ull, 0, wave, ln, trow);
            STAMP(8)
#pragma unroll 1
            for (int j0 = wave * 4; j0 < A_n; j0 += 4 * NWL)
                a2_group<C, true>(sh, j0, A_n, sh.q[A_buf], sh.qrec[A_buf], 0, nullptr, ln, half, twh, te,
                                  nan_rows != 0
#ifdef GSC_STAMPS
                                  , acc, &tlast, xc
#endif
                );
        }
        float err_sq = 0.0f;
        if (wave == kErrWave && ln < kc) err_sq = sqrt_rn(per_col(sh.gp[ln]));
        STAMP(2)
        lds_barrier();
        if (A_n > 0) {
            const uint64_t fx = __ballot(ln < A_n && sh.qrec[A_buf][ln].valid == 0);
            if (fx) {
                const int nfx = __popcll(fx);
#ifdef GSC_STAMPS
                it_fix = true;
                acn[4] += nfx;
#endif
                if (wave == 0 && ((fx >> ln) & 1ull)) sh.fxl[__popcll(fx & ((1ull << ln) - 1ull))] = ln;
                uint64_t m = fx;
                while (m) {
                    const int jj = __ffsll((long long)m) - 1;
                    m &= m - 1;
                    if ((prunedm >> jj) & 1ull) {
                        const float lb = __int_as_float(__builtin_amdgcn_readlane(__float_as_int(lbp), jj));
                        if (ln == 0) sh.wrec[vwave][jj].minbits = __float_as_uint(lb);
                    } else {
                        a1_query<C>(creg, sh.q[A_buf][jj], sh.wrec[vwave][jj], vwave, ln, dmask, trow, p0,
                                    tw_pass);
                    }
                }
                lds_barrier();
                write_cstar<C>(sh, creg, sh.qrec[A_buf], fx, 0, wave, ln, trow);
#pragma unroll 1
                for (int j0 = wave * 4; j0 < nfx; j0 += 4 * NWL)
                    a2_group<C, false>(sh, j0, nfx, sh.q[A_buf], sh.qrec[A_buf], 0, sh.fxl, ln);
                lds_barrier();
                if (kInBatchDfs && 3 * ib_fail <= ib_try + 8) {
                    uint64_t ux = __ballot(((fx >> ln) & 1ull) && sh.qrec[A_buf][ln].valid == 0);
                    const bool any_ux = ux != 0;
                    ib_try += __popcll(ux);
#pragma unroll 1
                    while (ux) {
                        const int jj = __ffsll((long long)ux) - 1;
                        ux &= ux - 1;
                        QRecT<D>& R = sh.qrec[A_buf][jj];
                        exact_dists(sh.q[A_buf][jj]);
                        lds_barrier();
                        int bpos;
                        float key;
                        if (nan_rows)
                            dfs_parallel_nan<C>(sh, sh.q[A_buf][jj], tid, ln, wave, bpos, key, &R);
                        else
                            dfs_parallel_call<C>(sh, sh.q[A_buf][jj], tid, ln, wave, bpos, key, &R);
                        bpos = uniform_int(bpos);
                        const int owner_t = bpos >> LS, slot = bpos & (SL - 1);
#pragma unroll
                        for (int s = 0; s < SL; ++s)
                            if (s == slot && tid == owner_t) {
#pragma unroll
                                for (int d = 0; d < C::DR; ++d) R.o[d] = creg[s][d];
                                if constexpr (C::SPLIT)
                                    for (int d = C::DR; d < D; ++d) R.o[d] = trow[(int64_t)bpos * C::TL + (d - C::DR)];
                            }
                        if (tid == 0) {
                            R.cstar = bpos;
                            R.id = sh.t.pidx[bpos];
                            R.g = key;
                            R.m2 = __uint_as_float(__float_as_uint(key) + 1u);
                            R.rate = sh.rate[bpos];
                            R.valid = (R.nimp <= kMaxImp && key <= FLT_MAX) ? 2 : 0;
                        }
#ifdef GSC_STAMPS
                        xc2[8] += 1;
#endif
                    }
                    if (any_ux) lds_barrier();
                }
            }
        }
        if (kc > 0) fold_commits<C>(sh, creg, cn, cnmax, vwave, ln, P_buf, P_off, kc, it & 1, trow);
#ifdef GSC_BOX_SHRINK
        if constexpr (!C::SPLIT) {
            if ((it % GSC_BOX_SHRINK) == GSC_BOX_SHRINK - 1) wave_box_init<C>(sh, creg, vwave, ln, p0, dmask);
        }
#endif
        STAMP(3)
        ln = opaque_v(ln);
        if (wave == kErrWave && has_p) {
            const int j = ln;
            const bool cj = j < kc;
            const QRecT<D>& R = sh.qrec[P_buf][P_off + (cj ? j : 0)];
            if (cj) {
                clusters[P_s + P_off + j] = R.id;
                atomicAdd(&cnta[R.cstar], 1);
            }
#pragma unroll
            for (int jj = 0; jj < KB; ++jj) {
                const double t = (double)__int_as_float(__builtin_amdgcn_readlane(__float_as_int(err_sq), jj));
                err = jj < kc ? err + t : err;
            }
        }
        if (wave == 0 && has_p) {
            const int j = ln;
            const bool cj = j < kc;
            const QRecT<D>& R = sh.qrec[P_buf][P_off + (cj ? j : 0)];
            const bool lastc = cj && sh.nxt[it & 1][j] >= kc && R.pad_ == 0;
            int tgt = lastc ? sh.ient[j] : -1;
            const uint64_t need = __ballot(lastc && tgt < 0);
            const uint64_t freem = __ballot(lg_pos < 0);
            const uint64_t below = (1ull << ln) - 1ull;
            sh.asg[ln] = -1;
            if (lg_pos < 0) sh.freel[__popcll(freem & below)] = ln;
            wave_lds_sync();
            if (lastc && tgt < 0) tgt = sh.freel[__popcll(need & below)];
            if (lastc) {
#pragma unroll
                for (int d = 0; d < D; ++d) sh.lg_c[tgt][d] = sh.newc[it & 1][j][d];
                sh.lg_c[tgt][C::ROW - 1] = sh.newc[it & 1][j][C::ROW - 1];
                sh.asg[tgt] = R.cstar;
            }
            wave_lds_sync();
            const int a = sh.asg[ln];
            if (a >= 0) {
                lg_pos = a;
                lg_tag = it;
            }
        }
        if (solo_j >= 0) {
            ++restarts;
            const bool snap_failed = uniform_int(sh.qrec[P_buf][P_off + fj].valid) != 1;
            if (!snap_failed) {
                a1_query<C>(creg, sh.qslow, sh.wrec[vwave][KB], vwave, ln, dmask, trow, p0, tw_pass);
                lds_barrier();
                if (wave == 0)
                    a2_group<C, false>(sh, 0, 1, reinterpret_cast<const float(*)[C::QD]>(sh.qslow), &sh.qsolo, KB,
                                       nullptr, ln);
                lds_barrier();
            }
            int bpos;
            float key;
            STAMP(10)
            if (!snap_failed && uniform_int(sh.qsolo.valid)) {
                bpos = uniform_int(sh.qsolo.cstar);
                key = sh.qsolo.g;
            } else {
                exact_dists(sh.qslow);
                lds_barrier();
                if (nan_rows) {
                    dfs_parallel_nan<C>(sh, sh.qslow, tid, ln, wave, bpos, key, nullptr);
                } else if constexpr (D <= GSC_DFS_CALL_D) {
                    dfs_parallel_call<C>(sh, sh.qslow, tid, ln, wave, bpos, key, nullptr);
                } else {
                    dfs_parallel<C>(sh, sh.qslow, tid, ln, wave, bpos, key);
                }
                bpos = uniform_int(bpos);
                ++slow_total;
                STAMP(11)
            }
#ifdef GSC_STAMPS
            {
                const bool same = bpos == sh.vcs[fj];
                const bool rem = fj + 1 < P_n;
                const uint64_t badm = __ballot(ln > fj && ln < P_n && sh.inval[ln] != 0);
                const int nb = badm ? __ffsll((long long)badm) - 1 : P_n;
                if (same) {
                    xc2[(fj_cause & 1) ? 0 : ((fj_cause & 2) ? 1 : 2)] += 1;
                    if (rem) {
                        xc2[4] += 1;
                        xc2[5] += (uint64_t)(nb - fj - 1);
                        xc2[6] += nb == P_n ? 1 : 0;
                    }
                }
                xc2[3] += rem ? 1 : 0;
            }
#endif
            const int owner_t = bpos >> LS, slot = bpos & (SL - 1);
#pragma unroll
            for (int s = 0; s < SL; ++s)
                if (s == slot && tid == owner_t) {
#pragma unroll
                    for (int d = 0; d < C::DR; ++d) sh.solo_c[d] = creg[s][d];
                    if constexpr (C::SPLIT)
                        for (int d = C::DR; d < D; ++d) sh.solo_c[d] = trow[(int64_t)bpos * C::TL + (d - C::DR)];
                }
            lds_barrier();
            if (wave == kErrWave && ln == 0) err += (double)sqrt_rn(per_col(key));
            if (wave == 0) {
                if (ln == 0) {
                    const float rate = sh.rate[bpos];
                    for (int d = 0; d < D; ++d) {
                        const float o = sh.solo_c[d];
                        sh.solo_c[d] = fadd(o, fmul(fsub(sh.qslow[d], o), rate));
                    }
                    atomicAdd(&cnta[bpos], 1);
                    clusters[solo_j] = sh.t.pidx[bpos];
                }
                wave_lds_sync();
                const uint64_t hit = __ballot(lg_pos == bpos);
                const int e = hit ? __ffsll((long long)hit) - 1 : __ffsll((long long)__ballot(lg_pos < 0)) - 1;
                if (ln == e) {
                    lg_pos = bpos;
                    lg_tag = it;
#pragma unroll
                    for (int d = 0; d < D; ++d) sh.lg_c[e][d] = sh.solo_c[d];
                    sh.lg_c[e][C::ROW - 1] = half ? norm2_x<C::H>(sh.solo_c) : norm2_x<D>(sh.solo_c);
                }
                sh.pub_pos[ln] = ln == e ? bpos : -1;
            }
            lds_barrier();
            refresh<C>(sh, creg, cn, cnmax, vwave, ln, trow);
        }
        STAMP(5)
#ifdef GSC_STAMPS
        {
            const uint64_t dt_ = stamp() - t_it0;
            xc[it_bubble ? 0 : 2] += 1;
            xc[it_bubble ? 1 : 3] += dt_;
            if (it_fix) {
                xc[4] += 1;
                xc[5] += dt_;
            }
            if (solo_j >= 0) {
                xc[6] += 1;
                xc[7] += dt_;
            }
            xc[8] += (uint64_t)cur_n_it;
        }
#endif
        if (nvq == 0 && cur_n == 0) {
            if (tid == 0) frp->loop_iters = it + 1;
            break;
        }
        if (it > 4 * N + 64) {
            if (tid == 0) frp->loop_iters = -1;
            guard = true;
            break;
        }
    }
    if (wave == kErrWave && lane == 0) sh.err_out = err;
    __syncthreads();
    err = sh.err_out;
#pragma unroll
    for (int s = 0; s < SL; ++s) {
        const int p = p0 + s;
        if (!((dmask >> s) & 1u)) {
            const int id = sh.t.pidx[p];
#pragma unroll
            for (int d = 0; d < C::DR; ++d) C_[(int64_t)id * D + d] = creg[s][d];
            if constexpr (C::SPLIT)
                for (int d = C::DR; d < D; ++d) C_[(int64_t)id * D + d] = trow[(int64_t)p * C::TL + (d - C::DR)];
        }
    }
    for (int p = tid; p < K; p += nthreads) {
        const int id = sh.t.pidx[p];
        if (id != 0xFFFF) prev_cnt[id] = __hip_atomic_load(&cnta[p], __ATOMIC_RELAXED, __HIP_MEMORY_SCOPE_AGENT);
    }
#ifdef GSC_STAMPS
    if (lane == 0)
        for (int k = 0; k < 16; ++k) frp->stamps[wave * 16 + k] += acc[k];
    if (lane == 0)
        for (int k = 0; k < 8; ++k) frp->acounts[wave * 8 + k] += acn[k];
    if (tid == 0)
        for (int k = 0; k < 16; ++k) frp->xcounts[k] += xc[k];
    if (tid == 0)
        for (int k = 0; k < 16; ++k) frp->xcounts2[k] += xc2[k];
#endif
    const double diff = err > prev_err ? err - prev_err : prev_err - err;
    const bool done = diff <= tol || pass + 1 >= kMaxScanIters || guard;
    prev_err = err;
    if (tid == 0) {
        frp->iters = pass + 1;
        frp->slow += slow_total;
        frp->restarts += restarts;
        frp->err = err;
        frp->done = done ? 1 : 0;
        if (done) frp->t_done = __builtin_amdgcn_s_memrealtime();
    }
    __threadfence();
    __syncthreads();
    if (done) {
        int* clh = uniform_ptr(frp->cl_host);
        if (clh) {
            for (int j = tid; j < N; j += nthreads)
                clh[j] = __hip_atomic_load(&clusters[j], __ATOMIC_RELAXED, __HIP_MEMORY_SCOPE_AGENT);
            __threadfence_system();
            __syncthreads();
            if (tid == 0) __hip_atomic_store(uniform_ptr(frp->notify), 1, __ATOMIC_RELEASE, __HIP_MEMORY_SCOPE_SYSTEM);
        }
        break;
    }
    }
    }
}

}

using namespace gsc;

template <class C>
static hipError_t launch_scan(ReduceFrame* frames, int nframes, const float* X, float* Cc, int* is,
                              const float* rate_tab, double tol, int max_passes, int opts, float* tails,
                              hipStream_t st) {
    const size_t shm = sizeof(Scan2Shared<C>);
    static_assert(sizeof(Scan2Shared<C>) <= 160 * 1024, "LDS budget (160 KB per CU)");
    hipError_t e = hipFuncSetAttribute((const void*)scan_batch_kernel<C>, hipFuncAttributeMaxDynamicSharedMemorySize,
                                       (int)shm);
    if (e != hipSuccess) return e;
    hipLaunchKernelGGL(scan_batch_kernel<C>, dim3(nframes), dim3(C::NT), shm, st, frames, nframes, X, Cc, is, rate_tab,
                       tol, max_passes, opts, tails);
    return hipGetLastError();
}

extern "C" hipError_t gsc_launch_scan_batch(int D, int logk, ReduceFrame* frames, int nframes, const float* X,
                                            float* Cc, int* is, const float* rate_tab, double tol, int max_passes,
                                            int opts, float* tails, hipStream_t st) {
#define SB(DV, LK, SLV)                                                                                           \
    if (D == DV && logk == LK)                                                                                    \
        return launch_scan<ScanCfg<DV, LK, SLV>>(frames, nframes, X, Cc, is, rate_tab, tol, max_passes, opts, tails, \
                                                 st);
    SB(8, 8, 1) SB(8, 9, 1) SB(8, 10, 2) SB(8, 11, 4) SB(8, 12, 8)
    SB(16, 8, 1) SB(16, 9, 1) SB(16, 10, 2) SB(16, 11, 4) SB(16, 12, 8)
    SB(32, 8, 1) SB(32, 9, 1) SB(32, 10, 2) SB(32, 11, 4)
    if (D == 32 && logk == 12)
        return launch_scan<ScanCfg<32, 12, 8, 16>>(frames, nframes, X, Cc, is, rate_tab, tol, max_passes, opts, tails,
                                                   st);
#undef SB
    return hipErrorInvalidValue;
}

extern "C" size_t gsc_scan_tail_floats_per_frame(int D, int logk) {
    return logk == 12 && D == 32 ? 4096 * size_t(D / 2) : 0;
}
```

Measured before the change: 23.93 Msamples/s.

## Specialize scan kernel for NaN-free frames and run general variant on side stream

```diff
diff --git a/soundchunks_amd/csrc/gsc_device.h b/soundchunks_amd/csrc/gsc_device.h
--- a/soundchunks_amd/csrc/gsc_device.h
+++ b/soundchunks_amd/csrc/gsc_device.h
@@ -31,6 +31,8 @@
     int32_t loop_iters;
     int32_t tree_exact;
     int32_t dcol;
+    int32_t plain;
+    int32_t plain_passes;
     uint64_t t_done;
     int32_t* cl_host;
     int32_t* notify;
diff --git a/soundchunks_amd/csrc/gsc_runtime.cpp b/soundchunks_amd/csrc/gsc_runtime.cpp
--- a/soundchunks_amd/csrc/gsc_runtime.cpp
+++ b/soundchunks_amd/csrc/gsc_runtime.cpp
@@ -32,7 +32,12 @@
                                            int only_flagged, hipStream_t st);
 extern "C" hipError_t gsc_launch_scan_batch(int D, int logk, gsc::ReduceFrame* frames, int nframes, const float* X,
                                             float* C, int* is, const float* rate_tab, double tol, int max_passes,
-                                            int opts, float* tails, hipStream_t st);
+                                            int opts, float* tails, int kinds, hipStream_t st,
+                                            hipStream_t st_general, hipEvent_t fork, hipEvent_t join);
+extern "C" int gsc_scan_has_experiments(void);
+extern "C" int gsc_scan_has_plain(int D, int logk);
+extern "C" hipError_t gsc_launch_scan_classify(int D, int logk, gsc::ReduceFrame* frames, int nframes, const float* C,
+                                               hipStream_t st);
 extern "C" size_t gsc_scan_tail_floats_per_frame(int D, int logk);
 extern "C" hipError_t gsc_launch_atten(int cs, gsc::DspFrame* frames, int nframes, const double* samp, int64_t span,
                                        int ch, int obd, hipStream_t st);
@@ -218,6 +223,48 @@
 
 std::atomic<int> g_scan_rounds{0};
 
+int scan_experiment_opts() {
+    const char* full = std::getenv("GSC_SCAN_FULL_A1");
+    const char* nopr = std::getenv("GSC_SCAN_NO_PRUNE");
+    const char* kb = std::getenv("GSC_SCAN_KB");
+    if (!full && !nopr && !kb) return 0;
+    if (!gsc_scan_has_experiments()) {
+        static std::atomic<bool> said{false};
+        if (!said.exchange(true))
+            std::fprintf(stderr,
+                         "soundchunks:%s%s%s set, but the scan experiments are not compiled into this build "
+                         "(tools/build_variant.sh NAME -DGSC_SCAN_EXPERIMENTS): ignored\n",
+                         full ? " GSC_SCAN_FULL_A1" : "", nopr ? " GSC_SCAN_NO_PRUNE" : "", kb ? " GSC_SCAN_KB" : "");
+        return 0;
+    }
+    return (full ? 1 : 0) | (nopr ? 2 : 0) | ((kb ? (std::atoi(kb) & 255) : 0) << 8);
+}
+
+struct ScanFork {
+    hipStream_t side = nullptr;
+    hipEvent_t fork = nullptr, join = nullptr;
+    std::mutex mu;
+    hipError_t err = hipSuccess;
+    bool made = false;
+};
+
+ScanFork* scan_fork() {
+    constexpr int kMaxDev = 64;
+    static ScanFork forks[kMaxDev];
+    static std::mutex mu;
+    int dev = 0;
+    if (hipGetDevice(&dev) != hipSuccess || dev < 0 || dev >= kMaxDev) return nullptr;
+    std::lock_guard<std::mutex> lk(mu);
+    ScanFork& f = forks[dev];
+    if (!f.made) {
+        f.made = true;
+        f.err = hipStreamCreateWithFlags(&f.side, hipStreamNonBlocking);
+        if (f.err == hipSuccess) f.err = hipEventCreateWithFlags(&f.fork, hipEventDisableTiming);
+        if (f.err == hipSuccess) f.err = hipEventCreateWithFlags(&f.join, hipEventDisableTiming);
+    }
+    return f.err == hipSuccess ? &f : nullptr;
+}
+
 hipError_t launch_scan_passes(int D, ReduceFrame* dfr, int nf, int K, const float* X, float* C, int* is, float* fs,
                               const float* rate, int precision) {
     const double tol = scan_tolerance(precision);
@@ -229,16 +276,29 @@
         const hipError_t e = tails.alloc(size_t(tail_offset(nf)));
         if (e != hipSuccess) return e;
     }
+    const int kinds = batched && K == (1 << logk) && gsc_scan_has_plain(D, logk) ? 3 : 2;
+    ScanFork* sf = kinds == 3 ? scan_fork() : nullptr;
+    if (kinds == 3) {
+        if (!sf) return hipErrorUnknown;
+        const hipError_t e = gsc_launch_scan_classify(D, logk, dfr, nf, C, nullptr);
+        if (e != hipSuccess) return e;
+    }
+    const int opts = batched ? scan_experiment_opts() : 0;
     int max_passes = kMaxScanIters;
     if (const char* e = std::getenv("GSC_SCAN_MAX_PASSES")) max_passes = std::max(1, std::min(kMaxScanIters, std::atoi(e)));
     std::vector<int32_t> flags(2 * static_cast<size_t>(nf));
     static_assert(offsetof(ReduceFrame, generic) == offsetof(ReduceFrame, done) + sizeof(int32_t), "adjacent flags");
     for (int round = 0; round < max_passes; ++round) {
         if (batched) {
-            const int opts = (std::getenv("GSC_SCAN_FULL_A1") ? 1 : 0) | (std::getenv("GSC_SCAN_NO_PRUNE") ? 2 : 0) |
-                             ((std::getenv("GSC_SCAN_KB") ? (std::atoi(std::getenv("GSC_SCAN_KB")) & 255) : 0) << 8);
-            hipError_t e =
-                gsc_launch_scan_batch(D, logk, dfr, nf, X, C, is, rate, tol, max_passes, opts, tails.p, nullptr);
+            hipError_t e;
+            if (sf) {
+                std::lock_guard<std::mutex> lk(sf->mu);
+                e = gsc_launch_scan_batch(D, logk, dfr, nf, X, C, is, rate, tol, max_passes, opts, tails.p, kinds, nullptr,
+                                          sf->side, sf->fork, sf->join);
+            } else {
+                e = gsc_launch_scan_batch(D, logk, dfr, nf, X, C, is, rate, tol, max_passes, opts, tails.p, kinds, nullptr,
+                                          nullptr, nullptr, nullptr);
+            }
             if (e != hipSuccess) return e;
             e = hipMemcpy2D(flags.data(), 2 * sizeof(int32_t), &dfr[0].done, sizeof(ReduceFrame), 2 * sizeof(int32_t),
                             size_t(nf), hipMemcpyDeviceToHost);
@@ -354,8 +414,10 @@
         for (int i = 0; i < nf; ++i)
             if (fr[i].t_done) t0 = std::min<uint64_t>(t0, fr[i].t_done);
         for (int i = 0; i < nf; ++i)
-            std::fprintf(stderr, "frame %d: N %d passes %d slow %d restarts %d done +%.1f ms\n", i, fr[i].N, fr[i].iters,
-                         fr[i].slow, fr[i].restarts, fr[i].t_done ? double(fr[i].t_done - t0) / 1e5 : -1.0);
+            std::fprintf(stderr, "frame %d: N %d passes %d slow %d restarts %d done +%.1f ms kind %s plain_passes %d\n", i,
+                         fr[i].N, fr[i].iters, fr[i].slow, fr[i].restarts,
+                         fr[i].t_done ? double(fr[i].t_done - t0) / 1e5 : -1.0, fr[i].plain ? "plain" : "general",
+                         fr[i].plain_passes);
     }
     if (std::getenv("GSC_HOST_TIMING") && nf > 0 && fr[0].ystamps[6] + fr[0].ystamps[1] + fr[0].ystamps[2] != 0) {
         double m[16] = {};
@@ -1834,8 +1896,10 @@
     if (fr[0].loop_iters < 0) return fail("KNNScanReduce: batched pipeline made no progress (guard tripped)");
     if (std::getenv("GSC_SCAN_DEBUG"))
     {
-        std::fprintf(stderr, "scan: passes %d slow %d restarts %d loop_iters(last pass) %d err %.9g tree_exact %d\n",
-                     fr[0].iters, fr[0].slow, fr[0].restarts, fr[0].loop_iters, fr[0].err, fr[0].tree_exact);
+        std::fprintf(stderr, "scan: passes %d slow %d restarts %d loop_iters(last pass) %d err %.9g tree_exact %d"
+                             " kind %s plain_passes %d\n",
+                     fr[0].iters, fr[0].slow, fr[0].restarts, fr[0].loop_iters, fr[0].err, fr[0].tree_exact,
+                     fr[0].plain ? "plain" : "general", fr[0].plain_passes);
         std::fprintf(stderr, "stamps [prep A1 A2 B2 part3 part4 B1 vcheck won setup soloA soloDFS a2win a2far a2box a2out]");
         for (int w = 0; w < 8; ++w) {
             std::fprintf(stderr, "\n  w%d:", w);
@@ -1872,6 +1936,72 @@
     return 0;
 }
 
+extern "C" int gsc_scan_reduce_frames(int nf, int d0, const int* ns, const float* x, const int* ks, float* centroids,
+                                      int* clusters, int precision, int* iters, int* plain, int* plain_passes,
+                                      double* err) {
+    if (ensure_device() != 0) return -1;
+    if (nf <= 0 || !ns || !ks || !x || !centroids || !clusters) return fail("gsc_scan_reduce_frames: invalid argument");
+    if (d0 <= 0 || d0 > 32) return fail("KNNScanReduce kernels support 1 <= d <= 32 features");
+    const int d = feature_stride((d0 + 1) / 2);
+    int kmax = 0, nmax = 0;
+    int64_t nsum = 0, ksum = 0;
+    for (int i = 0; i < nf; ++i) {
+        if (ns[i] <= 0 || ks[i] < 2 || ks[i] > kMaxK) return fail("gsc_scan_reduce_frames: invalid frame shape");
+        kmax = std::max(kmax, ks[i]);
+        nmax = std::max(nmax, ns[i]);
+        nsum += ns[i];
+        ksum += ks[i];
+    }
+    const int Kp = padded_k(kmax);
+    const std::vector<float> xp = pad_rows(x, int(nsum), d0, d);
+    std::vector<float> cp = pad_rows(centroids, int(ksum), d0, d);
+    std::vector<ReduceFrame> fr(static_cast<size_t>(nf));
+    int64_t no = 0, ko = 0;
+    for (int i = 0; i < nf; ++i) {
+        fr[i] = ReduceFrame{};
+        fr[i].x_off = no * d;
+        fr[i].c_off = ko * d;
+        fr[i].n_off = no;
+        fr[i].k_off = nsum + ko;
+        fr[i].ka_off = nsum + ksum + int64_t(i) * Kp;
+        fr[i].t_off = tail_offset(i);
+        fr[i].N = ns[i];
+        fr[i].K = ks[i];
+        fr[i].dcol = d0;
+        no += ns[i];
+        ko += ks[i];
+    }
+    DevBuf<float> dX, dC, dRate, dF;
+    DevBuf<int> dI;
+    DevBuf<ReduceFrame> dFr;
+    HIP_TRY(dF.alloc(size_t(nsum) * 4));
+    HIP_TRY(dX.alloc(xp.size()));
+    HIP_TRY(dC.alloc(cp.size()));
+    HIP_TRY(dI.alloc(size_t(nsum) + size_t(ksum) + size_t(nf) * size_t(Kp)));
+    HIP_TRY(dFr.alloc(size_t(nf)));
+    const std::vector<float> rt = rate_table(nmax);
+    HIP_TRY(dRate.alloc(rt.size()));
+    HIP_TRY(hipMemcpy(dX.p, xp.data(), sizeof(float) * xp.size(), hipMemcpyHostToDevice));
+    HIP_TRY(hipMemcpy(dC.p, cp.data(), sizeof(float) * cp.size(), hipMemcpyHostToDevice));
+    HIP_TRY(hipMemcpy(dRate.p, rt.data(), sizeof(float) * rt.size(), hipMemcpyHostToDevice));
+    HIP_TRY(hipMemcpy(dFr.p, fr.data(), sizeof(ReduceFrame) * size_t(nf), hipMemcpyHostToDevice));
+    HIP_TRY(launch_scan_passes(d, dFr.p, nf, kmax, dX.p, dC.p, dI.p, dF.p, dRate.p, precision));
+    HIP_TRY(hipDeviceSynchronize());
+    HIP_TRY(hipMemcpy(cp.data(), dC.p, sizeof(float) * cp.size(), hipMemcpyDeviceToHost));
+    compact_rows(&cp, int(ksum), d, d0);
+    std::memcpy(centroids, cp.data(), sizeof(float) * size_t(ksum) * d0);
+    HIP_TRY(hipMemcpy(clusters, dI.p, sizeof(int) * size_t(nsum), hipMemcpyDeviceToHost));
+    HIP_TRY(hipMemcpy(fr.data(), dFr.p, sizeof(ReduceFrame) * size_t(nf), hipMemcpyDeviceToHost));
+    for (int i = 0; i < nf; ++i) {
+        if (fr[i].loop_iters < 0) return fail("KNNScanReduce: batched pipeline made no progress (guard tripped)");
+        if (iters) iters[i] = fr[i].iters;
+        if (plain) plain[i] = fr[i].plain;
+        if (plain_passes) plain_passes[i] = fr[i].plain_passes;
+        if (err) err[i] = fr[i].err;
+    }
+    return 0;
+}
+
 int gsc_birch_labels(int n, int d, const float* x, int k, int* labels) {
     if (!x || !labels || n <= 0 || d <= 0 || k <= 0) return fail("gsc_birch_labels: invalid argument");
     if (ensure_device() != 0) return -1;
diff --git a/soundchunks_amd/csrc/gsc_scan.hip b/soundchunks_amd/csrc/gsc_scan.hip
--- a/soundchunks_amd/csrc/gsc_scan.hip
+++ b/soundchunks_amd/csrc/gsc_scan.hip
@@ -84,10 +84,14 @@
     return kInfBits;
 }
 
+#if !defined(GSC_SCAN_EXPERIMENTS) && (defined(GSC_BOX_SHRINK) || defined(GSC_MAX_IMP))
+#error "GSC_BOX_SHRINK and GSC_MAX_IMP are experiment switches: add -DGSC_SCAN_EXPERIMENTS"
+#endif
 #ifndef GSC_MAX_IMP
 #define GSC_MAX_IMP 8
 #endif
 constexpr int kMaxImp = GSC_MAX_IMP;
+static_assert(kMaxImp >= 1 && kMaxImp <= 16, "QRecT::B holds the improvement distances: 16 entries");
 
 template <int D>
 struct QRecT {
@@ -467,7 +471,8 @@
 template <class C, bool APPROX>
 __device__ __forceinline__ void a2_group(Scan2Shared<C>& sh, int j0, int nq, const float (*qrows)[C::QD],
                                          QRecT<C::D>* recs, int wcol0, const int* jlist, int lane,
-                                         bool half = false, float twh = 0.0f, float te = 0.0f, bool nanpass = false
+                                         bool half = false, float twh = 0.0f, float te = 0.0f, bool nanpass = false,
+                                         bool nans = true
 #ifdef GSC_STAMPS
                                          , uint64_t* acc = nullptr, uint64_t* tl = nullptr, uint64_t* xc = nullptr
 #endif
@@ -671,7 +676,7 @@
             R.m2 = m2lo;
             R.rate = sh.rate[cs];
             R.farmask = farmask;
-            R.pad_ = nanf >= 0 ? 1 : 0;
+            if (nans) R.pad_ = nanf >= 0 ? 1 : 0;
         }
     }
     ASTAMP(15)
@@ -685,9 +690,9 @@
 
 template <class C>
 __device__ __forceinline__ void vp_begin(Scan2Shared<C>& sh, int qb, int off, int pn, int a1, int lane, int& lg_pos,
-                                         int lg_tag, VPState& st) {
+                                         int lg_tag, VPState& st, bool nans) {
     if (lg_pos >= 0 && lg_tag < a1) lg_pos = -1;
-    st.cs = lane < pn ? (sh.qrec[qb][off + lane].pad_ ? -100 - lane : sh.qrec[qb][off + lane].cstar) : -2;
+    st.cs = lane < pn ? (nans && sh.qrec[qb][off + lane].pad_ ? -100 - lane : sh.qrec[qb][off + lane].cstar) : -2;
     sh.vmeta[lane].x = lg_pos;
     sh.vmeta[lane].y = 0;
     if (lane < C::KB) sh.vcs[lane] = st.cs;
@@ -715,7 +720,7 @@
 
 template <class C>
 __device__ __forceinline__ void vp_end(Scan2Shared<C>& sh, int qb, int off, int pn, int lane, int lg_pos,
-                                       const VPState& st, bool half, int par) {
+                                       const VPState& st, bool half, int par, bool nans) {
     constexpr int D = C::D, KB = C::KB;
     const int j = lane;
     const bool act = j < pn;
@@ -741,7 +746,7 @@
             float oc[D];
 #pragma unroll
             for (int d = 0; d < D; ++d) oc[d] = o[d];
-            const bool nanq = R.pad_ != 0;
+            const bool nanq = nans && R.pad_ != 0;
             const float gpj = nanq ? __builtin_nanf("") : seqdist<D>(qv, oc);
             const bool okc = nanq || (R.valid != 0 && (pred < 0 || gpj < R.m2));
             const float rate = R.rate;
@@ -780,7 +785,8 @@
 }
 
 template <class C>
-__device__ __forceinline__ void v_check_grab(Scan2Shared<C>& sh, int qb, int off, int pn, int lane, int par) {
+__device__ __forceinline__ void v_check_grab(Scan2Shared<C>& sh, int qb, int off, int pn, int lane, int par,
+                                             bool nans) {
     constexpr int D = C::D, KB = C::KB, QPL = 64 / KB, LOGK = C::LOGK;
     constexpr int VPT = 2 * QPL;
     constexpr int NTRIP = (C::KVER + VPT - 1) / VPT;
@@ -791,7 +797,7 @@
     const int j = lane % KB, grp = lane / KB;
     const int jr = j < pn ? j : 0;
     const QRecT<D>& R = sh.qrec[qb][off + jr];
-    const bool act = j < pn && R.pad_ == 0;
+    const bool act = j < pn && !(nans && R.pad_ != 0);
     const bool dfsa = R.valid == 2;
     const int cs = R.cstar;
     const uint32_t fm = R.farmask;
@@ -1150,14 +1156,14 @@
 template <class C>
 __device__ __forceinline__ void fold_commits(Scan2Shared<C>& sh, float (&creg)[C::SL][C::DR], float (&cn)[C::SL],
                                              float& cnmax, int vwave, int lane, int qb, int off, int kc, int par,
-                                             float* __restrict__ trow = nullptr) {
+                                             bool nans, float* __restrict__ trow = nullptr) {
     constexpr int SL = C::SL, LS = C::LS, D = C::D, DR = C::DR;
     int pp = 0;
     bool mine = false;
     if (lane < kc) {
         const QRecT<D>& R = sh.qrec[qb][off + lane];
         pp = R.cstar;
-        mine = sh.nxt[par][lane] >= kc && R.pad_ == 0 && (pp >> (6 + LS)) == vwave;
+        mine = sh.nxt[par][lane] >= kc && !(nans && R.pad_ != 0) && (pp >> (6 + LS)) == vwave;
     }
     uint64_t m = __ballot(mine);
     if (!m) return;
@@ -1257,20 +1263,29 @@
     }
 }
 
-template <class C>
+template <class C, bool PLAIN>
 __global__ __launch_bounds__(C::NT) void scan_batch_kernel(ReduceFrame* __restrict__ frames, int nframes,
                                                            const float* __restrict__ Xall, float* __restrict__ Call,
                                                            int* __restrict__ i_scratch,
                                                            const float* __restrict__ rate_tab, double tol,
-                                                           int max_passes, int opts,
+                                                           int max_passes,
+#ifdef GSC_SCAN_EXPERIMENTS
+                                                           int opts,
+#endif
                                                            float* __restrict__ Tall) {
     constexpr int D = C::D, K = C::K, SL = C::SL, LS = C::LS, NWL = C::NWL, KB = C::KB;
     constexpr int kErrWave = NWL > 1 ? 1 : 0;
     constexpr bool PRUNE = true;
+    constexpr bool NANS = !PLAIN;
     constexpr bool kInBatchDfs = D <= GSC_INBATCH_DFS_D;
+#ifdef GSC_SCAN_EXPERIMENTS
     const bool no_half = (opts & 1) != 0;
     const bool no_prune = (opts & 2) != 0;
     const int kbe = ((opts >> 8) & 255) > 0 && ((opts >> 8) & 255) < KB ? ((opts >> 8) & 255) : KB;
+#else
+    constexpr bool no_half = false, no_prune = false;
+    constexpr int kbe = KB;
+#endif
     extern __shared__ __attribute__((aligned(16))) unsigned char smem[];
     Scan2Shared<C>& sh = *reinterpret_cast<Scan2Shared<C>*>(smem);
     const int tid = threadIdx.x, lane = tid & 63, wave = tid >> 6;
@@ -1279,12 +1294,12 @@
     const int fi0 = blockIdx.x, fstep = nframes;
     for (int fi = fi0; fi < nframes; fi += fstep) {
     ReduceFrame* frp = frames + fi;
-    if (uniform_int(frp->done) || uniform_int(frp->generic)) continue;
+    if (uniform_int(frp->done) || uniform_int(frp->generic) || (uniform_int(frp->plain) != 0) != PLAIN) continue;
     const int N = uniform_int(frp->N);
-    const int dcol_i = uniform_int(frp->dcol) > 0 ? uniform_int(frp->dcol) : D;
-    auto per_col = [dcol_i](float v) { return dcol_i == D ? v / (float)D : v / (float)dcol_i; };
-    const int Kr = uniform_int(frp->K);
-    const bool padded = Kr != K;
+    const int dcol_i = PLAIN ? D : (uniform_int(frp->dcol) > 0 ? uniform_int(frp->dcol) : D);
+    auto per_col = [=](float v) { return (PLAIN || dcol_i == D) ? v / (float)D : v / (float)dcol_i; };
+    const int Kr = PLAIN ? K : uniform_int(frp->K);
+    const bool padded = !PLAIN && Kr != K;
     const float* __restrict__ X = Xall + uniform_i64(frp->x_off);
     float* C_ = Call + uniform_i64(frp->c_off);
     int* clusters = i_scratch + uniform_i64(frp->n_off);
@@ -1320,27 +1335,35 @@
     if (pass == 0)
         for (int k = tid; k < Kr; k += nthreads) prev_cnt[k] = 1;
     if (tid == 0) sh.any_nan = 0;
-    for (int w = tid; w < kMaxK / 32; w += nthreads) sh.nanid[w] = 0u;
-    __syncthreads();
     int nan_rows = 0;
-    for (int k = tid; k < Kr; k += nthreads) {
-        bool nn = false;
-#pragma unroll
-        for (int d = 0; d < D; ++d) nn |= C_[(int64_t)k * D + d] != C_[(int64_t)k * D + d];
-        if (nn) {
-            atomicOr(&sh.nanid[k >> 5], 1u << (k & 31));
-            nan_rows = 1;
-        }
-    }
-    nan_rows = __syncthreads_or(nan_rows);
+    if constexpr (!PLAIN) {
+        for (int w = tid; w < kMaxK / 32; w += nthreads) sh.nanid[w] = 0u;
+        __syncthreads();
+        for (int k = tid; k < Kr; k += nthreads) {
+            bool nn = false;
+#pragma unroll
+            for (int d = 0; d < D; ++d) nn |= C_[(int64_t)k * D + d] != C_[(int64_t)k * D + d];
+            if (nn) {
+                atomicOr(&sh.nanid[k >> 5], 1u << (k & 31));
+                nan_rows = 1;
+            }
+        }
+        nan_rows = __syncthreads_or(nan_rows);
+    } else {
+        __syncthreads();
+    }
     if (padded) {
-        build_tree<D>(sh.t, sh.dist, C_, Kr);
-        pad_tree<C::LOGK>(sh.t, reinterpret_cast<int*>(sh.dist), Kr, tid, nthreads);
+        if constexpr (!PLAIN) {
+            build_tree<D>(sh.t, sh.dist, C_, Kr);
+            pad_tree<C::LOGK>(sh.t, reinterpret_cast<int*>(sh.dist), Kr, tid, nthreads);
+        }
     } else if (nan_rows) {
-        if constexpr (K / nthreads >= 4)
-            build_tree_nan<D, C::LOGK, nthreads>(sh.t, sh.dist, sh.dfs_inc, C_);
-        else
-            build_tree<D>(sh.t, sh.dist, C_, K);
+        if constexpr (!PLAIN) {
+            if constexpr (K / nthreads >= 4)
+                build_tree_nan<D, C::LOGK, nthreads>(sh.t, sh.dist, sh.dfs_inc, C_);
+            else
+                build_tree<D>(sh.t, sh.dist, C_, K);
+        }
     } else if constexpr (K / nthreads < 4) {
         build_tree<D>(sh.t, sh.dist, C_, K);
     } else if (!build_tree_fast<D, C::LOGK, nthreads>(sh.t, sh.dist, sh.dfs_inc, C_, &sh.slow_pos)) {
@@ -1365,15 +1388,22 @@
         const int p = p0 + s;
         const int id = p < K ? (int)sh.t.pidx[p] : 0xFFFF;
         bool dead = false;
-        if (nan_rows && p < K) {
+        if constexpr (!PLAIN) {
+            if (nan_rows && p < K) {
 #pragma unroll 1
-            for (int l = 0, h = 0; l < C::LOGK; ++l) {
-                const int bit = (p >> (C::LOGK - 1 - l)) & 1;
-                dead |= bit == 0 && sh.t.cv[h] != sh.t.cv[h];
-                h = 2 * h + 1 + bit;
-            }
-        }
-        if (id != 0xFFFF && !dead && !((sh.nanid[id >> 5] >> (id & 31)) & 1u)) {
+                for (int l = 0, h = 0; l < C::LOGK; ++l) {
+                    const int bit = (p >> (C::LOGK - 1 - l)) & 1;
+                    dead |= bit == 0 && sh.t.cv[h] != sh.t.cv[h];
+                    h = 2 * h + 1 + bit;
+                }
+            }
+        }
+        bool live = true;
+        if constexpr (!PLAIN)
+            live = id != 0xFFFF && !dead && !((sh.nanid[id >> 5] >> (id & 31)) & 1u);
+        else if constexpr (!C::FULL)
+            live = id != 0xFFFF;
+        if (live) {
 #pragma unroll
             for (int d = 0; d < C::DR; ++d) {
                 creg[s][d] = C_[(int64_t)id * D + d];
@@ -1554,11 +1584,11 @@
 #ifdef GSC_STAMPS_PREP
         STAMP(14)
 #endif
-        if (wave == 0 && has_p) vp_begin<C>(sh, P_buf, P_off, P_n, vq_a10, ln, lg_pos, lg_tag, vst);
+        if (wave == 0 && has_p) vp_begin<C>(sh, P_buf, P_off, P_n, vq_a10, ln, lg_pos, lg_tag, vst, NANS);
         constexpr bool kVpEarly = D <= GSC_VP_EARLY_D;
         if constexpr (kVpEarly) {
             if (wave == 0 && has_p) {
-                vp_end<C>(sh, P_buf, P_off, P_n, ln, lg_pos, vst, half, it & 1);
+                vp_end<C>(sh, P_buf, P_off, P_n, ln, lg_pos, vst, half, it & 1, NANS);
                 wave_lds_sync();
                 if (ln == 0) __hip_atomic_store(&sh.vp_ready, it + 1, __ATOMIC_RELEASE, __HIP_MEMORY_SCOPE_WORKGROUP);
             }
@@ -1641,7 +1671,7 @@
             a1_mask(curm);
         }
         if constexpr (!kVpEarly) {
-            if (wave == 0 && has_p) vp_end<C>(sh, P_buf, P_off, P_n, ln, lg_pos, vst, half, it & 1);
+            if (wave == 0 && has_p) vp_end<C>(sh, P_buf, P_off, P_n, ln, lg_pos, vst, half, it & 1, NANS);
         }
         {
             STAMP(7)
@@ -1656,7 +1686,7 @@
                     while (__hip_atomic_load(&sh.vp_ready, __ATOMIC_ACQUIRE, __HIP_MEMORY_SCOPE_WORKGROUP) != it + 1)
                         __builtin_amdgcn_s_sleep(1);
                 }
-                v_check_grab<C>(sh, P_buf, P_off, P_n, ln, it & 1);
+                v_check_grab<C>(sh, P_buf, P_off, P_n, ln, it & 1, NANS);
             }
         }
 #ifdef GSC_STAMPS
@@ -1743,7 +1773,7 @@
 #pragma unroll 1
             for (int j0 = wave * 4; j0 < A_n; j0 += 4 * NWL)
                 a2_group<C, true>(sh, j0, A_n, sh.q[A_buf], sh.qrec[A_buf], 0, nullptr, ln, half, twh, te,
-                                  nan_rows != 0
+                                  NANS && nan_rows != 0, NANS
 #ifdef GSC_STAMPS
                                   , acc, &tlast, xc
 #endif
@@ -1778,7 +1808,7 @@
                 write_cstar<C>(sh, creg, sh.qrec[A_buf], fx, 0, wave, ln, trow);
 #pragma unroll 1
                 for (int j0 = wave * 4; j0 < nfx; j0 += 4 * NWL)
-                    a2_group<C, false>(sh, j0, nfx, sh.q[A_buf], sh.qrec[A_buf], 0, sh.fxl, ln);
+                    a2_group<C, false>(sh, j0, nfx, sh.q[A_buf], sh.qrec[A_buf], 0, sh.fxl, ln, false, 0.0f, 0.0f, false, NANS);
                 lds_barrier();
                 if (kInBatchDfs && 3 * ib_fail <= ib_try + 8) {
                     uint64_t ux = __ballot(((fx >> ln) & 1ull) && sh.qrec[A_buf][ln].valid == 0);
@@ -1793,7 +1823,7 @@
                         lds_barrier();
                         int bpos;
                         float key;
-                        if (nan_rows)
+                        if (NANS && nan_rows)
                             dfs_parallel_nan<C>(sh, sh.q[A_buf][jj], tid, ln, wave, bpos, key, &R);
                         else
                             dfs_parallel_call<C>(sh, sh.q[A_buf][jj], tid, ln, wave, bpos, key, &R);
@@ -1823,7 +1853,7 @@
                 }
             }
         }
-        if (kc > 0) fold_commits<C>(sh, creg, cn, cnmax, vwave, ln, P_buf, P_off, kc, it & 1, trow);
+        if (kc > 0) fold_commits<C>(sh, creg, cn, cnmax, vwave, ln, P_buf, P_off, kc, it & 1, NANS, trow);
 #ifdef GSC_BOX_SHRINK
         if constexpr (!C::SPLIT) {
             if ((it % GSC_BOX_SHRINK) == GSC_BOX_SHRINK - 1) wave_box_init<C>(sh, creg, vwave, ln, p0, dmask);
@@ -1849,7 +1879,7 @@
             const int j = ln;
             const bool cj = j < kc;
             const QRecT<D>& R = sh.qrec[P_buf][P_off + (cj ? j : 0)];
-            const bool lastc = cj && sh.nxt[it & 1][j] >= kc && R.pad_ == 0;
+            const bool lastc = cj && sh.nxt[it & 1][j] >= kc && !(NANS && R.pad_ != 0);
             int tgt = lastc ? sh.ient[j] : -1;
             const uint64_t need = __ballot(lastc && tgt < 0);
             const uint64_t freem = __ballot(lg_pos < 0);
@@ -1879,7 +1909,7 @@
                 lds_barrier();
                 if (wave == 0)
                     a2_group<C, false>(sh, 0, 1, reinterpret_cast<const float(*)[C::QD]>(sh.qslow), &sh.qsolo, KB,
-                                       nullptr, ln);
+                                       nullptr, ln, false, 0.0f, 0.0f, false, NANS);
                 lds_barrier();
             }
             int bpos;
@@ -1891,7 +1921,7 @@
             } else {
                 exact_dists(sh.qslow);
                 lds_barrier();
-                if (nan_rows) {
+                if (NANS && nan_rows) {
                     dfs_parallel_nan<C>(sh, sh.qslow, tid, ln, wave, bpos, key, nullptr);
                 } else if constexpr (D <= GSC_DFS_CALL_D) {
                     dfs_parallel_call<C>(sh, sh.qslow, tid, ln, wave, bpos, key, nullptr);
@@ -2015,6 +2045,7 @@
     prev_err = err;
     if (tid == 0) {
         frp->iters = pass + 1;
+        if constexpr (PLAIN) frp->plain_passes += 1;
         frp->slow += slow_total;
         frp->restarts += restarts;
         frp->err = err;
@@ -2038,37 +2069,99 @@
     }
 }
 
+__global__ __launch_bounds__(256) void scan_classify_kernel(ReduceFrame* __restrict__ frames, int nframes,
+                                                            const float* __restrict__ Call, int D, int K2) {
+    const int fi = blockIdx.x;
+    if (fi >= nframes) return;
+    ReduceFrame* frp = frames + fi;
+    if (uniform_int(frp->done)) return;
+    const int Kr = uniform_int(frp->K), dcol = uniform_int(frp->dcol);
+    const float* __restrict__ C_ = Call + uniform_i64(frp->c_off);
+    int nan = 0;
+    if (Kr == K2 && (dcol == 0 || dcol == D)) {
+        const int64_t n = (int64_t)Kr * D;
+        for (int64_t i = threadIdx.x; i < n; i += blockDim.x) nan |= C_[i] != C_[i] ? 1 : 0;
+    } else {
+        nan = 1;
+    }
+    nan = __syncthreads_or(nan);
+    if (threadIdx.x == 0) frp->plain = nan ? 0 : 1;
+}
+
 }
 
 using namespace gsc;
 
 template <class C>
 static hipError_t launch_scan(ReduceFrame* frames, int nframes, const float* X, float* Cc, int* is,
-                              const float* rate_tab, double tol, int max_passes, int opts, float* tails,
-                              hipStream_t st) {
+                              const float* rate_tab, double tol, int max_passes, int opts, float* tails, int kinds,
+                              hipStream_t st, hipStream_t st_general, hipEvent_t fork, hipEvent_t join) {
     const size_t shm = sizeof(Scan2Shared<C>);
     static_assert(sizeof(Scan2Shared<C>) <= 160 * 1024, "LDS budget (160 KB per CU)");
-    hipError_t e = hipFuncSetAttribute((const void*)scan_batch_kernel<C>, hipFuncAttributeMaxDynamicSharedMemorySize,
-                                       (int)shm);
-    if (e != hipSuccess) return e;
-    hipLaunchKernelGGL(scan_batch_kernel<C>, dim3(nframes), dim3(C::NT), shm, st, frames, nframes, X, Cc, is, rate_tab,
-                       tol, max_passes, opts, tails);
+    hipError_t e;
+    if (C::SPLIT) kinds = 2;
+    const bool both = (kinds & 3) == 3 && st_general != nullptr;
+    auto launch = [&](auto kernel, hipStream_t s) -> hipError_t {
+        hipError_t le = hipFuncSetAttribute((const void*)kernel, hipFuncAttributeMaxDynamicSharedMemorySize, (int)shm);
+        if (le != hipSuccess) return le;
+#ifdef GSC_SCAN_EXPERIMENTS
+        hipLaunchKernelGGL(kernel, dim3(nframes), dim3(C::NT), shm, s, frames, nframes, X, Cc, is, rate_tab, tol,
+                           max_passes, opts, tails);
+#else
+        (void)opts;
+        hipLaunchKernelGGL(kernel, dim3(nframes), dim3(C::NT), shm, s, frames, nframes, X, Cc, is, rate_tab, tol,
+                           max_passes, tails);
+#endif
+        return hipGetLastError();
+    };
+    if (kinds & 2) {
+        if (both) {
+            if ((e = hipEventRecord(fork, st)) != hipSuccess) return e;
+            if ((e = hipStreamWaitEvent(st_general, fork, 0)) != hipSuccess) return e;
+        }
+        if ((e = launch(scan_batch_kernel<C, false>, both ? st_general : st)) != hipSuccess) return e;
+        if (both && (e = hipEventRecord(join, st_general)) != hipSuccess) return e;
+    }
+    if constexpr (!C::SPLIT) {
+        if (kinds & 1) {
+            if ((e = launch(scan_batch_kernel<C, true>, st)) != hipSuccess) return e;
+        }
+    }
+    if ((kinds & 2) && both) return hipStreamWaitEvent(st, join, 0);
+    return hipSuccess;
+}
+
+extern "C" int gsc_scan_has_plain(int D, int logk) { return !(D == 32 && logk == 12); }
+
+extern "C" hipError_t gsc_launch_scan_classify(int D, int logk, ReduceFrame* frames, int nframes, const float* Cc,
+                                               hipStream_t st) {
+    hipLaunchKernelGGL(scan_classify_kernel, dim3(nframes), dim3(256), 0, st, frames, nframes, Cc, D,
+                       gsc_scan_has_plain(D, logk) ? (1 << logk) : -1);
     return hipGetLastError();
+}
+
+extern "C" int gsc_scan_has_experiments(void) {
+#ifdef GSC_SCAN_EXPERIMENTS
+    return 1;
+#else
+    return 0;
+#endif
 }
 
 extern "C" hipError_t gsc_launch_scan_batch(int D, int logk, ReduceFrame* frames, int nframes, const float* X,
                                             float* Cc, int* is, const float* rate_tab, double tol, int max_passes,
-                                            int opts, float* tails, hipStream_t st) {
+                                            int opts, float* tails, int kinds, hipStream_t st, hipStream_t st_general,
+                                            hipEvent_t fork, hipEvent_t join) {
 #define SB(DV, LK, SLV)                                                                                           \
     if (D == DV && logk == LK)                                                                                    \
         return launch_scan<ScanCfg<DV, LK, SLV>>(frames, nframes, X, Cc, is, rate_tab, tol, max_passes, opts, tails, \
-                                                 st);
+                                                 kinds, st, st_general, fork, join);
     SB(8, 8, 1) SB(8, 9, 1) SB(8, 10, 2) SB(8, 11, 4) SB(8, 12, 8)
     SB(16, 8, 1) SB(16, 9, 1) SB(16, 10, 2) SB(16, 11, 4) SB(16, 12, 8)
     SB(32, 8, 1) SB(32, 9, 1) SB(32, 10, 2) SB(32, 11, 4)
     if (D == 32 && logk == 12)
         return launch_scan<ScanCfg<32, 12, 8, 16>>(frames, nframes, X, Cc, is, rate_tab, tol, max_passes, opts, tails,
-                                                   st);
+                                                   kinds, st, st_general, fork, join);
 #undef SB
     return hipErrorInvalidValue;
 }
```

Result: faster. 24.33 Msamples/s, median of 6 (+1.7%).
